# DerEchteKarsten/RayTracer3

Hardware: AMD Instinct MI355X
Metric: Mrays/s (higher is better)
Workload: dtype f32

## Files before the change

include/rt3.h:

```cpp
#ifndef RT3_H
#define RT3_H
#include <stddef.h>
#include <stdint.h>

#ifdef __cplusplus
extern "C" {
#endif

#define RT3_OK 0
#define RT3_E_INVALID (-1)
#define RT3_E_HIP (-2)
#define RT3_E_NO_DEVICE (-3)
#define RT3_E_STATE (-4)
#define RT3_E_UNSUPPORTED (-5)
#define RT3_E_DEPTH (-6)
#define RT3_E_COMM (-7)

#define RT3_INVALID_HANDLE 0xFFFFFFFFu
#define RT3_TAG_BUFFER 0u
#define RT3_TAG_IMAGE 1u
#define RT3_TAG_ACCEL 3u
#define RT3_MISS 0xFFFFFFFFu
#define RT3_BACKGROUND_DEPTH 100000.0f

#define RT3_FORMAT_R32_SFLOAT 100u
#define RT3_FORMAT_R32G32B32A32_SFLOAT 109u
#define RT3_FORMAT_R32G32B32A32_UINT 107u
#define RT3_FORMAT_R8G8B8A8_UNORM 37u
#define RT3_FORMAT_R16_UINT 74u

#define RT3_F_NEE_SKY 1u
#define RT3_F_BLUENOISE 2u
#define RT3_F_SPECULAR 4u
#define RT3_F_FACEFORWARD 8u
#define RT3_F_PROBE_RADIANCE 16u
#define RT3_F_NEE_EMISSIVE 32u
#define RT3_F_NEE_PUNCTUAL 64u

typedef struct rt3_gconst {
    float proj[16];
    float view[16];
    float proj_inverse[16];
    float view_inverse[16];
    float window_size[2];
    uint32_t frame;
    float blendfactor;
    uint32_t bounces;
    uint32_t samples;
    uint32_t proberng;
    float cell_size;
    uint32_t mouse[2];
    uint32_t pad[2];
} rt3_gconst;

typedef struct rt3_geometry_info {
    float base_color[4];
    int32_t base_color_texture_index;
    float metallic_factor;
    uint32_t index_offset;
    uint32_t vertex_offset;
    float emission[4];
    float roughness;
    uint32_t _pad[3];
} rt3_geometry_info;

typedef struct rt3_instance {
    uint32_t geometry_first, geometry_count;
    float transform[16];
} rt3_instance;

typedef struct rt3_stats {
    uint64_t extension_rays;
    uint64_t shadow_rays;
    uint64_t nodes_visited;
    uint64_t tris_tested;
    uint64_t shadow_nodes_visited;
    uint64_t shadow_tris_tested;
    uint64_t extend_launches;
    double extend_ms;
    uint64_t shadow_launches;
    double shadow_ms;
    double shade_ms;
    double other_ms;
    uint64_t trace_launches;
    double trace_ms;
    uint64_t trace_rays[2];
    uint64_t trace_nodes[2];
    uint64_t trace_tris[2];
    double gather_ms;
    uint64_t nodes_visited_lds;
    uint64_t shadow_nodes_visited_lds;
    double accel_build_ms;
    uint64_t accel_bulk_copies;
    uint64_t accel_arena_serial;
} rt3_stats;

typedef struct rt3_ctx rt3_ctx;

int rt3_create(int device, rt3_ctx **out);
void rt3_destroy(rt3_ctx *ctx);
const char *rt3_last_error(rt3_ctx *ctx);
int rt3_device_name(rt3_ctx *ctx, char *buf, size_t buf_size);

#define RT3_OPT_BATCH_SPP 1
#define RT3_OPT_PROFILE 2
#define RT3_OPT_COUNT_TRAVERSAL 3
#define RT3_OPT_EXTEND_VARIANT 4
#define RT3_OPT_LEAF_SIZE 5
#define RT3_OPT_NODE_WIDTH 6
#define RT3_OPT_NODE_QUANT 7
#define RT3_OPT_WIDE_COLLAPSE 8
#define RT3_OPT_POOL_CHUNK 9
#define RT3_OPT_SAH_TOP 11
#define RT3_OPT_TRACE_BLOCKS 12
#define RT3_OPT_INSTANCE_MODE 14
#define RT3_OPT_SHADOW_EXIT_TABLE 15
#define RT3_OPT_DEFER_SKY_LIGHT 16
int rt3_set_option(rt3_ctx *ctx, int option, int64_t value);

int rt3_scene_set_vertices(rt3_ctx *ctx, const float *interleaved_p_n_t, uint32_t n_vertices);
int rt3_scene_set_indices(rt3_ctx *ctx, const uint32_t *indices, uint32_t n_indices);
int rt3_scene_set_geometry(rt3_ctx *ctx, const rt3_geometry_info *infos, const uint32_t *prim_counts, uint32_t n);
int rt3_scene_set_sky(rt3_ctx *ctx, const float *rgb, uint32_t width, uint32_t height);
int rt3_scene_set_bluenoise(rt3_ctx *ctx, const uint8_t *rgba, uint32_t width, uint32_t height);
int rt3_scene_set_texture(rt3_ctx *ctx, uint32_t index, const uint8_t *rgba_srgb, uint32_t width, uint32_t height);
int rt3_scene_set_alpha_cutoffs(rt3_ctx *ctx, const float *cutoffs, uint32_t n);
typedef struct rt3_material_textures {
    int32_t metallic_roughness_texture;
    int32_t normal_texture;
    int32_t emissive_texture;
    float   normal_scale;
} rt3_material_textures;
int rt3_scene_set_material_textures(rt3_ctx *ctx, const rt3_material_textures *m, uint32_t n);
typedef struct rt3_transmission {
    float    transmission;
    float    ior;
    uint32_t thin_walled;
    uint32_t reserved;
} rt3_transmission;
int rt3_scene_set_transmission(rt3_ctx *ctx, const rt3_transmission *t, uint32_t n);
int rt3_scene_set_pane_shadows(rt3_ctx *ctx, int on);
int rt3_scene_get_pane_shadows(rt3_ctx *ctx, int *on);
int rt3_pane_shadow_info(rt3_ctx *ctx, uint32_t *n_panes);

int rt3_scene_set_instances(rt3_ctx *ctx, const rt3_instance *instances, uint32_t n);
int rt3_scene_set_prev_transforms(rt3_ctx *ctx, const float *transforms , uint32_t n);
#define RT3_LIGHT_POINT 0u
#define RT3_LIGHT_SPOT 1u
#define RT3_LIGHT_DIRECTIONAL 2u
typedef struct rt3_punctual_light {
    uint32_t type;
    float range;
    float inner_cone, outer_cone;
    float position[3];
    float _pad0;
    float direction[3];
    float _pad1;
    float intensity[3];
    float _pad2;
} rt3_punctual_light;
int rt3_scene_set_lights(rt3_ctx *ctx, const rt3_punctual_light *lights, uint32_t n);
int rt3_light_masses(rt3_ctx *ctx, uint32_t flags, uint32_t *n_emitters, uint32_t *n_punctual, uint32_t *mass);
int rt3_scene_snapshot_vertices(rt3_ctx *ctx);
int rt3_scene_forget_prev_vertices(rt3_ctx *ctx);
int rt3_scene_deformed_geometries(rt3_ctx *ctx, uint8_t *flags, uint32_t n);

int rt3_accel_build(rt3_ctx *ctx, uint32_t *out_handle);
int rt3_accel_info(rt3_ctx *ctx, uint32_t *n_nodes, uint32_t *n_tris, uint32_t *max_depth, uint32_t *node_bytes);
int rt3_accel_download(rt3_ctx *ctx, void *nodes, size_t nodes_bytes, void *tris, size_t tris_bytes);
int rt3_accel_levels(rt3_ctx *ctx, uint32_t *n_meshes, uint32_t *n_meshes_built, uint32_t *n_top_nodes, uint64_t *accel_bytes);
int rt3_accel_exit_table_info(rt3_ctx *ctx, uint32_t *cells, uint64_t *tried, uint64_t *occluded, uint32_t *in_use);
int rt3_accel_import(rt3_ctx *ctx, const void *nodes, size_t nodes_bytes, const void *tris, size_t tris_bytes);
int rt3_scene_update_vertices(rt3_ctx *ctx, const float *interleaved_p_n_t, uint32_t first, uint32_t n);
int rt3_accel_refit(rt3_ctx *ctx, uint32_t *out_handle);
int rt3_light_info(rt3_ctx *ctx, uint32_t *n_emitters, uint64_t *cdf_total);
int rt3_light_download(rt3_ctx *ctx, uint32_t *prim, float *area, uint32_t *mass );
int rt3_sky_download(rt3_ctx *ctx, uint32_t *alias, uint32_t *texels_rgb9e5, float *cdf_marg, float *pdf_uv);

int rt3_buffer_create(rt3_ctx *ctx, size_t bytes, uint32_t *out_handle);
int rt3_image_create(rt3_ctx *ctx, uint32_t width, uint32_t height, uint32_t format, uint32_t *out_handle);
int rt3_image_import(rt3_ctx *ctx, void *device_ptr, uint32_t width, uint32_t height, uint32_t format, uint32_t *out_handle);
int rt3_resource_upload(rt3_ctx *ctx, uint32_t handle, const void *src, size_t bytes);
int rt3_resource_download(rt3_ctx *ctx, uint32_t handle, void *dst, size_t bytes);
int rt3_resource_device_ptr(rt3_ctx *ctx, uint32_t handle, void **out_ptr, size_t *out_bytes);

int rt3_set_tile_partition(rt3_ctx *ctx, uint32_t width, uint32_t height, uint32_t rank, uint32_t n_ranks);
int rt3_tile_pixel_count(rt3_ctx *ctx, uint32_t rank, uint32_t n_ranks, uint32_t *out_count);
int rt3_image_pack_tiles(rt3_ctx *ctx, uint32_t image, uint32_t rank, uint32_t n_ranks, void *dst_device);
int rt3_image_unpack_tiles(rt3_ctx *ctx, uint32_t image, uint32_t rank, uint32_t n_ranks, const void *src_device);

#define RT3_COMM_ID_BYTES 128
int rt3_comm_version(int *out);
int rt3_comm_unique_id(void *id_out );
int rt3_comm_init(rt3_ctx *ctx, const void *id , uint32_t rank, uint32_t n_ranks);
int rt3_comm_destroy(rt3_ctx *ctx);
int rt3_gather_tiles(rt3_ctx *ctx, uint32_t image, uint32_t root);
int rt3_gather_layout(rt3_ctx *ctx, uint32_t image, uint32_t root, uint32_t n_ranks, uint64_t *offsets );
int rt3_gather_unpack(rt3_ctx *ctx, uint32_t image, uint32_t root, uint32_t n_ranks, const void *recv_device);

int rt3_pass_launch(rt3_ctx *ctx, const char *pass_name, const char *entry, uint32_t x, uint32_t y, uint32_t z,
                    const void *constants, size_t constants_size, const uint32_t *bindings, uint32_t n_bindings);
#define RT3_DENOISE_NO_DEMODULATION 1u
typedef struct rt3_denoise_params {
    uint32_t iterations;
    uint32_t normal_squarings;
    float sigma_z;
    float sigma_l;
    uint32_t flags;
} rt3_denoise_params;
int rt3_denoise_set_params(rt3_ctx *ctx, const rt3_denoise_params *params);
int rt3_denoise_set_variance_input(rt3_ctx *ctx, uint32_t moments_image);

#define RT3_TEMPORAL_NO_DEMODULATION 1u
typedef struct rt3_temporal_params {
    float alpha;
    float alpha_moments;
    uint32_t max_history;
    float normal_cos;
    float plane_tolerance;
    uint32_t flags;
} rt3_temporal_params;
int rt3_temporal_set_prev_view(rt3_ctx *ctx, const void *prev_gconst, size_t size);
int rt3_temporal_set_params(rt3_ctx *ctx, const rt3_temporal_params *params);
int rt3_temporal_set_motion_input(rt3_ctx *ctx, uint32_t motion_image);
typedef struct rt3_adaptive_params {
    uint32_t min_samples;
    uint32_t step;
    float threshold;
    float dark;
    uint32_t dilate;
    uint32_t flags;
} rt3_adaptive_params;
int rt3_adaptive_set_params(rt3_ctx *ctx, const rt3_adaptive_params *params);
int rt3_adaptive_info(rt3_ctx *ctx, uint32_t *rounds, uint64_t *paths_traced, uint32_t *pixels_capped);
typedef struct rt3_lens_params {
    float aperture_radius;
    float focus_distance;
    float pixel_jitter;
    uint32_t reserved;
} rt3_lens_params;
int rt3_camera_set_lens(rt3_ctx *ctx, const rt3_lens_params *p);
int rt3_camera_get_lens(rt3_ctx *ctx, rt3_lens_params *out, int *enabled);
typedef struct rt3_roulette_params {
    uint32_t start_bounce;
    float min_survival;
    uint32_t reserved[2];
} rt3_roulette_params;
int rt3_path_set_roulette(rt3_ctx *ctx, const rt3_roulette_params *p);
int rt3_path_get_roulette(rt3_ctx *ctx, rt3_roulette_params *out, int *enabled);
int rt3_path_roulette_info(rt3_ctx *ctx, uint64_t *tested, uint64_t *ended);

int rt3_frame_wait(rt3_ctx *ctx);

int rt3_trace_rays(rt3_ctx *ctx, const float *rays, uint32_t n, int any_hit, float *t, float *u, float *v, uint32_t *prim,
                   uint32_t *n_nodes, uint32_t *n_tris, int repeat, double *kernel_ms);

int rt3_selftest_eval(rt3_ctx *ctx, int op, const void *in, uint32_t n, void *out);

int rt3_stats_reset(rt3_ctx *ctx);
int rt3_stats_get(rt3_ctx *ctx, rt3_stats *out);

void rt3_camera_gconst(const float position[3], const float direction[3], float fov_y_radians, float aspect,
                       float z_near, float z_far, float width, float height, rt3_gconst *out);

#ifdef __cplusplus
}
#endif
#endif
```

raytracer3_amd/_lib.py:

```python
from __future__ import annotations

import ctypes as C
import os
from pathlib import Path

PKG = Path(__file__).resolve().parent
LIB_PATH = Path(os.environ.get("RT3_LIBRARY", PKG / "librt3.so"))

RT3_OK = 0
E_INVALID, E_HIP, E_NO_DEVICE, E_STATE, E_UNSUPPORTED, E_DEPTH, E_COMM = -1, -2, -3, -4, -5, -6, -7
COMM_ID_BYTES = 128
TAG_BUFFER, TAG_IMAGE, TAG_ACCEL = 0, 1, 3
MISS = 0xFFFFFFFF
BACKGROUND_DEPTH = 100000.0
FORMAT_R32_SFLOAT, FORMAT_R32G32B32A32_SFLOAT, FORMAT_R32G32B32A32_UINT, FORMAT_R8G8B8A8_UNORM, FORMAT_R16_UINT = 100, 109, 107, 37, 74
F_NEE_SKY, F_BLUENOISE, F_SPECULAR, F_FACEFORWARD, F_PROBE_RADIANCE = 1, 2, 4, 8, 16
F_NEE_EMISSIVE = 32
F_NEE_PUNCTUAL = 64
LIGHT_POINT, LIGHT_SPOT, LIGHT_DIRECTIONAL = 0, 1, 2
SELFTEST_LIGHT = 30
OPT_BATCH_SPP, OPT_PROFILE, OPT_COUNT_TRAVERSAL, OPT_EXTEND_VARIANT, OPT_LEAF_SIZE, OPT_NODE_WIDTH, OPT_NODE_QUANT = 1, 2, 3, 4, 5, 6, 7
OPT_WIDE_COLLAPSE, OPT_POOL_CHUNK, OPT_SAH_TOP, OPT_TRACE_BLOCKS = 8, 9, 11, 12
OPT_FUSED_TRACE = 10
OPT_INSTANCE_MODE = 14
OPT_SHADOW_EXIT_TABLE = 15
OPT_DEFER_SKY_LIGHT = 16
DENOISE_NO_DEMODULATION = 1
TEMPORAL_NO_DEMODULATION = 1
SELFTEST_EXPN = 28
SELFTEST_HIT_INFO = 29
SELFTEST_LENS = 31
SELFTEST_GLASS = 32
SELFTEST_ROULETTE = 33
SELFTEST_ROULETTE_QUEUE = 34

EXPORTS = [
    "rt3_create", "rt3_destroy", "rt3_last_error", "rt3_device_name", "rt3_set_option",
    "rt3_scene_set_vertices", "rt3_scene_set_indices", "rt3_scene_set_geometry", "rt3_scene_set_sky", "rt3_scene_set_bluenoise", "rt3_scene_set_texture",
    "rt3_scene_set_alpha_cutoffs",
    "rt3_scene_set_material_textures",
    "rt3_scene_set_transmission",
    "rt3_scene_set_pane_shadows", "rt3_scene_get_pane_shadows", "rt3_pane_shadow_info",
    "rt3_scene_set_instances",
    "rt3_accel_build", "rt3_accel_info", "rt3_accel_levels", "rt3_accel_exit_table_info", "rt3_accel_download", "rt3_accel_import", "rt3_sky_download",
    "rt3_scene_update_vertices", "rt3_accel_refit", "rt3_light_info", "rt3_light_download",
    "rt3_buffer_create", "rt3_image_create", "rt3_image_import", "rt3_resource_upload", "rt3_resource_download", "rt3_resource_device_ptr",
    "rt3_set_tile_partition", "rt3_tile_pixel_count", "rt3_image_pack_tiles", "rt3_image_unpack_tiles",
    "rt3_comm_version", "rt3_comm_unique_id", "rt3_comm_init", "rt3_comm_destroy", "rt3_gather_tiles", "rt3_gather_layout", "rt3_gather_unpack",
    "rt3_pass_launch", "rt3_denoise_set_params", "rt3_denoise_set_variance_input", "rt3_temporal_set_prev_view", "rt3_temporal_set_params",
    "rt3_scene_set_prev_transforms", "rt3_temporal_set_motion_input",
    "rt3_adaptive_set_params", "rt3_adaptive_info",
    "rt3_camera_set_lens", "rt3_camera_get_lens",
    "rt3_path_set_roulette", "rt3_path_get_roulette", "rt3_path_roulette_info",
    "rt3_scene_set_lights", "rt3_light_masses",
    "rt3_scene_snapshot_vertices", "rt3_scene_forget_prev_vertices", "rt3_scene_deformed_geometries",
    "rt3_frame_wait", "rt3_trace_rays", "rt3_selftest_eval", "rt3_stats_reset", "rt3_stats_get", "rt3_camera_gconst",
]


class GConst(C.Structure):

    _fields_ = [("proj", C.c_float * 16), ("view", C.c_float * 16), ("proj_inverse", C.c_float * 16), ("view_inverse", C.c_float * 16),
                ("window_size", C.c_float * 2), ("frame", C.c_uint32), ("blendfactor", C.c_float), ("bounces", C.c_uint32),
                ("samples", C.c_uint32), ("proberng", C.c_uint32), ("cell_size", C.c_float), ("mouse", C.c_uint32 * 2), ("pad", C.c_uint32 * 2)]


class Stats(C.Structure):
    _fields_ = [("extension_rays", C.c_uint64), ("shadow_rays", C.c_uint64), ("nodes_visited", C.c_uint64), ("tris_tested", C.c_uint64),
                ("shadow_nodes_visited", C.c_uint64), ("shadow_tris_tested", C.c_uint64),
                ("extend_launches", C.c_uint64), ("extend_ms", C.c_double), ("shadow_launches", C.c_uint64), ("shadow_ms", C.c_double),
                ("shade_ms", C.c_double), ("other_ms", C.c_double),
                ("trace_launches", C.c_uint64), ("trace_ms", C.c_double), ("trace_rays", C.c_uint64 * 2), ("trace_nodes", C.c_uint64 * 2),
                ("trace_tris", C.c_uint64 * 2), ("gather_ms", C.c_double), ("nodes_visited_lds", C.c_uint64), ("shadow_nodes_visited_lds", C.c_uint64), ("accel_build_ms", C.c_double), ("accel_bulk_copies", C.c_uint64),
                ("accel_arena_serial", C.c_uint64)]


class Instance(C.Structure):

    _fields_ = [("geometry_first", C.c_uint32), ("geometry_count", C.c_uint32), ("transform", C.c_float * 16)]


class DenoiseParams(C.Structure):

    _fields_ = [("iterations", C.c_uint32), ("normal_squarings", C.c_uint32), ("sigma_z", C.c_float), ("sigma_l", C.c_float), ("flags", C.c_uint32)]

    def __init__(self, iterations=5, normal_squarings=7, sigma_z=0.05, sigma_l=4.0, flags=0):
        super().__init__(iterations, normal_squarings, sigma_z, sigma_l, flags)


class TemporalParams(C.Structure):

    _fields_ = [("alpha", C.c_float), ("alpha_moments", C.c_float), ("max_history", C.c_uint32), ("normal_cos", C.c_float),
                ("plane_tolerance", C.c_float), ("flags", C.c_uint32)]

    def __init__(self, alpha=0.2, alpha_moments=0.2, max_history=32, normal_cos=0.9, plane_tolerance=0.01, flags=0):
        super().__init__(alpha, alpha_moments, max_history, normal_cos, plane_tolerance, flags)


class AdaptiveParams(C.Structure):

    _fields_ = [("min_samples", C.c_uint32), ("step", C.c_uint32), ("threshold", C.c_float), ("dark", C.c_float), ("dilate", C.c_uint32),
                ("flags", C.c_uint32)]

    def __init__(self, min_samples=16, step=16, threshold=0.05, dark=0.01, dilate=1, flags=0):
        super().__init__(min_samples, step, threshold, dark, dilate, flags)


class LensParams(C.Structure):

    _fields_ = [("aperture_radius", C.c_float), ("focus_distance", C.c_float), ("pixel_jitter", C.c_float), ("reserved", C.c_uint32)]

    def __init__(self, aperture_radius=0.0, focus_distance=1.0, pixel_jitter=1.0, reserved=0):
        super().__init__(aperture_radius, focus_distance, pixel_jitter, reserved)


class RouletteParams(C.Structure):

    _fields_ = [("start_bounce", C.c_uint32), ("min_survival", C.c_float), ("reserved", C.c_uint32 * 2)]

    def __init__(self, start_bounce=2, min_survival=0.0625, reserved=(0, 0)):
        super().__init__(start_bounce, min_survival, (C.c_uint32 * 2)(*reserved))


assert C.sizeof(GConst) == 304


def kernel_source_hash() -> str:
    import hashlib

    h = hashlib.sha256()
    files = sorted((PKG / "csrc").glob("*.hip")) + sorted((PKG / "csrc").glob("*.hpp")) + sorted((PKG / "csrc").glob("*.inc")) + [PKG / "csrc" / "Makefile", PKG.parent / "include" / "rt3.h"]
    for f in files:
        h.update(f.name.encode())
        h.update(f.read_bytes())
    return h.hexdigest()[:16]


class Rt3Error(RuntimeError):
    def __init__(self, code, msg):
        super().__init__(f"rt3 error {code}: {msg}")
        self.code = code


_lib = None


def load():
    global _lib
    if _lib is not None:
        return _lib
    try:
        import torch
    except ImportError:
        pass
    if not LIB_PATH.exists():
        raise ImportError(f"{LIB_PATH} is missing: build it with `make -C {PKG / 'csrc'}` (hipcc, gfx950). There is no CPU fallback.")
    L = C.CDLL(str(LIB_PATH))
    vp, u32, i32, f32, sz = C.c_void_p, C.c_uint32, C.c_int, C.c_float, C.c_size_t
    pu32 = C.POINTER(C.c_uint32)
    sig = {
        "rt3_create": (i32, [i32, C.POINTER(vp)]),
        "rt3_destroy": (None, [vp]),
        "rt3_last_error": (C.c_char_p, [vp]),
        "rt3_device_name": (i32, [vp, C.c_char_p, sz]),
        "rt3_set_option": (i32, [vp, i32, C.c_int64]),
        "rt3_scene_set_vertices": (i32, [vp, vp, u32]),
        "rt3_scene_set_indices": (i32, [vp, vp, u32]),
        "rt3_scene_set_geometry": (i32, [vp, vp, vp, u32]),
        "rt3_scene_set_sky": (i32, [vp, vp, u32, u32]),
        "rt3_scene_set_bluenoise": (i32, [vp, vp, u32, u32]),
        "rt3_scene_set_texture": (i32, [vp, u32, vp, u32, u32]),
        "rt3_scene_set_alpha_cutoffs": (i32, [vp, vp, u32]),
        "rt3_scene_set_material_textures": (i32, [vp, vp, u32]),
        "rt3_scene_set_transmission": (i32, [vp, vp, u32]),
        "rt3_scene_set_pane_shadows": (i32, [vp, i32]),
        "rt3_scene_get_pane_shadows": (i32, [vp, C.POINTER(i32)]),
        "rt3_pane_shadow_info": (i32, [vp, C.POINTER(u32)]),
        "rt3_scene_set_instances": (i32, [vp, vp, u32]),
        "rt3_accel_build": (i32, [vp, pu32]),
# ... 60 lines not shown
```

raytracer3_amd/csrc/rt3_api.hip:

```cpp
#include <hip/hip_runtime.h>

#include <cmath>
#include <cstdio>
#include <cstring>
#include <string>
#include <vector>

#include "rt3_ctx.hpp"
#include "rt3_roulette.hpp"

using namespace rt3;

static_assert(sizeof(rt3_gconst) == 304 && sizeof(GConstDev) == 304, "GConst is 304 bytes (renderer/mod.rs:47-63)");
static_assert(sizeof(rt3_geometry_info) == 64, "geometry info is 64 bytes");
static_assert(RT3_F_NEE_SKY == RT3_FLAG_NEE_SKY && RT3_F_BLUENOISE == RT3_FLAG_BLUENOISE && RT3_F_FACEFORWARD == RT3_FLAG_FACEFORWARD && RT3_F_SPECULAR == RT3_FLAG_SPECULAR && RT3_F_PROBE_RADIANCE == RT3_FLAG_PROBE_RADIANCE && RT3_F_NEE_EMISSIVE == RT3_FLAG_NEE_EMISSIVE && RT3_F_NEE_PUNCTUAL == RT3_FLAG_NEE_PUNCTUAL, "flags");
static_assert(sizeof(rt3_punctual_light) == 64, "rt3_punctual_light is four float4 to the device");

static thread_local std::string g_create_error;

namespace rt3 {

int fail(rt3_ctx* c, int code, const std::string& msg) {
    if (c) c->err = msg;
    else g_create_error = msg;
    return code;
}

Resource* get_res(rt3_ctx* c, uint32_t handle, uint32_t want_tag) {
    uint32_t tag = handle >> 30, idx = handle & 0x3FFFFFFFu;
    if (tag != want_tag || idx >= c->resources.size()) return nullptr;
    Resource* r = &c->resources[idx];
    return r->tag == want_tag && r->ptr ? r : nullptr;
}
size_t format_bytes(uint32_t f) {
    switch (f) {
        case RT3_FORMAT_R32_SFLOAT: return 4;
        case RT3_FORMAT_R32G32B32A32_SFLOAT: return 16;
        case RT3_FORMAT_R32G32B32A32_UINT: return 16;
        case RT3_FORMAT_R8G8B8A8_UNORM: return 4;
        case RT3_FORMAT_R16_UINT: return 2;
        default: return 0;
    }
}

int harvest(rt3_ctx* c) {
    if (!c->work.pending_counters.empty()) {
        std::vector<uint32_t> h(c->work.counters_next);
        HIPC(c, hipMemcpy(h.data(), c->work.d_counters.get(), (size_t)c->work.counters_next * 4, hipMemcpyDeviceToHost));
        for (auto& b : c->work.pending_counters) {
            for (uint32_t k = 0; k < b.n_pairs; k++) {
                uint32_t traced = h[b.first + 2 * k];
                if (b.rr_first && k >= b.rr_lo && k + 1 < b.n_pairs) {
                    const uint32_t emitted = traced;
                    traced = h[b.rr_first + k];
                    if (b.launch == c->work.launch_serial) {
                        c->work.roulette_tested += emitted;
                        c->work.roulette_ended += emitted - traced;
                    }
                }
                c->prof.stats.extension_rays += traced;
                c->prof.stats.shadow_rays += h[b.first + 2 * k + 1];
            }
            for (uint32_t k = 0; k < b.n_emit; k++) c->prof.stats.shadow_rays += h[b.emit_first + k];
        }
        c->work.pending_counters.clear();
    }
    c->work.counters_next = 0;
    c->prof.stats.extension_rays += c->work.primary_rays_pending;
    c->work.primary_rays_pending = 0;
    if (c->opt.count) {
        unsigned long long t[kTotWords] = {};
        HIPC(c, hipMemcpy(t, c->work.d_totals.get(), sizeof(t), hipMemcpyDeviceToHost));
        c->prof.stats.nodes_visited += t[kTotExtendNodes];
        c->prof.stats.tris_tested += t[kTotExtendTris];
        c->prof.stats.shadow_nodes_visited += t[kTotShadowNodes];
        c->prof.stats.shadow_tris_tested += t[kTotShadowTris];
        c->prof.stats.nodes_visited_lds += t[kTotExtendLds];
        c->prof.stats.shadow_nodes_visited_lds += t[kTotShadowLds];
        HIPC(c, hipMemset(c->work.d_totals.get(), 0, sizeof(t)));
    }
    for (auto& t : c->prof.pending_events) {
        float ms = 0.0f;
        HIPC(c, hipEventElapsedTime(&ms, t.a, t.b));
        switch (t.cat) {
            case CAT_EXTEND: c->prof.stats.extend_ms += ms; c->prof.stats.extend_launches++; break;
            case CAT_SHADOW: c->prof.stats.shadow_ms += ms; c->prof.stats.shadow_launches++; break;
            case CAT_SHADE: c->prof.stats.shade_ms += ms; break;
            case CAT_GATHER: c->prof.stats.gather_ms += ms; break;
            default: c->prof.stats.other_ms += ms; break;
        }
        c->prof.free_events.push_back(t);
    }
    c->prof.pending_events.clear();
    return RT3_OK;
}

}

extern "C" {

int rt3_create(int device, rt3_ctx** out) {
    if (!out) return fail(nullptr, RT3_E_INVALID, "out is NULL");
    *out = nullptr;
    int n = 0;
    if (hipGetDeviceCount(&n) != hipSuccess || n <= 0) return fail(nullptr, RT3_E_NO_DEVICE, "no HIP device visible (librt3 has no CPU fallback)");
    if (device < 0 || device >= n) return fail(nullptr, RT3_E_INVALID, "device index out of range");
    hipDeviceProp_t prop;
    if (hipSetDevice(device) != hipSuccess || hipGetDeviceProperties(&prop, device) != hipSuccess) return fail(nullptr, RT3_E_HIP, "hipSetDevice failed");
    if (std::string(prop.gcnArchName).rfind("gfx950", 0) != 0)
        return fail(nullptr, RT3_E_NO_DEVICE, std::string("device is ") + prop.gcnArchName + ", librt3 is built for gfx950 only");
    rt3_ctx* c = new rt3_ctx();
    c->device = device;
    snprintf(c->name, sizeof(c->name), "%s (%s)", prop.name, prop.gcnArchName);
    memset(&c->prof.stats, 0, sizeof(c->prof.stats));
    if (hipStreamCreateWithFlags(&c->stream, hipStreamNonBlocking) != hipSuccess || c->work.d_counters.alloc_bytes((size_t)c->work.counters_cap * 4) != hipSuccess ||
        c->work.d_totals.alloc_bytes(kTotWords * 8) != hipSuccess || hipMemset(c->work.d_totals.get(), 0, kTotWords * 8) != hipSuccess) {
        rt3_destroy(c);
        return fail(nullptr, RT3_E_HIP, "stream / counter allocation failed");
    }
    *out = c;
    return RT3_OK;
}

void rt3_destroy(rt3_ctx* c) {
    if (!c) return;
    (void)hipSetDevice(c->device);
    if (c->stream) (void)hipStreamSynchronize(c->stream);
    comm_release(c);
    for (auto& t : c->prof.pending_events) { (void)hipEventDestroy(t.a); (void)hipEventDestroy(t.b); }
    for (auto& t : c->prof.free_events) { (void)hipEventDestroy(t.a); (void)hipEventDestroy(t.b); }
    hipStream_t stream = c->stream;
    delete c;
    if (stream) (void)hipStreamDestroy(stream);
}

const char* rt3_last_error(rt3_ctx* c) { return c ? c->err.c_str() : g_create_error.c_str(); }

int rt3_device_name(rt3_ctx* c, char* buf, size_t n) {
    if (!c || !buf || !n) return RT3_E_INVALID;
    snprintf(buf, n, "%s", c->name);
    return RT3_OK;
}

int rt3_set_option(rt3_ctx* c, int option, int64_t value) {
    if (!c) return RT3_E_INVALID;
    switch (option) {
        case RT3_OPT_BATCH_SPP: c->opt.batch_spp = value; return RT3_OK;
        case RT3_OPT_PROFILE: c->opt.profile = value != 0; return RT3_OK;
        case RT3_OPT_COUNT_TRAVERSAL: c->opt.count = value != 0; return RT3_OK;
        case RT3_OPT_EXTEND_VARIANT:
            c->opt.variant = (int)value;
            HIPC(c, hipSetDevice(c->device));
            set_refill_lanes((uint32_t)value);
            return RT3_OK;
        case RT3_OPT_LEAF_SIZE:
            if (value < 1 || value > 8) return fail(c, RT3_E_INVALID, "leaf size must be 1..8");
            c->opt.leaf_size = (uint32_t)value;
            invalidate_topology(c);
            return RT3_OK;
        case RT3_OPT_NODE_QUANT:
            if (value < 0 || value > 2) return fail(c, RT3_E_INVALID, "node quantisation must be 0 (fp32), 1 (64 B) or 2 (compact 48 B)");
            c->opt.node_quant = (uint32_t)value;
            invalidate_topology(c);
            return RT3_OK;
        case RT3_OPT_SAH_TOP:
            if (value < 0 || value > 65536) return fail(c, RT3_E_INVALID, "SAH-top cluster size must be 0 (off) .. 65536");
            c->opt.sah_top = (uint32_t)value;
            invalidate_topology(c);
            return RT3_OK;
        case RT3_OPT_POOL_CHUNK:
            if (value < 64 || value > 65536 || (value & 63)) return fail(c, RT3_E_INVALID, "pool chunk must be a multiple of 64 in [64, 65536]");
            HIPC(c, hipSetDevice(c->device));
            set_pool_chunk((uint32_t)value);
            return RT3_OK;
        case RT3_OPT_TRACE_BLOCKS:
            if (value < 1 || value > 65535) return fail(c, RT3_E_INVALID, "trace blocks must be in [1, 65535]");
            set_trace_blocks((uint32_t)value);
            return RT3_OK;
        case RT3_OPT_WIDE_COLLAPSE:
            if (value < 0 || value > 2) return fail(c, RT3_E_INVALID, "wide collapse must be 0 (even depth), 1 (surface area) or 2 (cost-driven)");
            c->opt.collapse = (uint32_t)value;
            invalidate_topology(c);
            return RT3_OK;
        case RT3_OPT_NODE_WIDTH:
            if (value != 2 && value != 4) return fail(c, RT3_E_INVALID, "node width must be 2 or 4");
            c->opt.node_width = (uint32_t)value;
            invalidate_topology(c);
            return RT3_OK;
        case RT3_OPT_INSTANCE_MODE:
            if (value != 0 && value != 1) return fail(c, RT3_E_INVALID, "instance mode must be 0 (flatten) or 1 (two-level)");
            c->opt.instance_mode = (int)value;
            invalidate_accel(c);
            return RT3_OK;
        case RT3_OPT_SHADOW_EXIT_TABLE:
            if (value < 0 || value > 2) return fail(c, RT3_E_INVALID, "shadow exit table must be 0 (off), 1 (on) or 2 (on, scrambled entries)");
            c->opt.exit_table = (int)value;
            return exit_table_update(c);
        case RT3_OPT_DEFER_SKY_LIGHT:
            if (value != 0 && value != 1) return fail(c, RT3_E_INVALID, "defer sky light must be 0 (off) or 1 (on)");
            c->opt.defer_sky_light = value != 0;
            return RT3_OK;
        default: return fail(c, RT3_E_INVALID, "unknown option");
    }
}

int rt3_buffer_create(rt3_ctx* c, size_t bytes, uint32_t* out) {
    if (!c || !out || !bytes) return fail(c, RT3_E_INVALID, "bad buffer size");
    HIPC(c, hipSetDevice(c->device));
    Resource r;
    r.tag = RT3_TAG_BUFFER;
    r.bytes = bytes;
    HIPC(c, r.mem.alloc_bytes(bytes));
    r.ptr = r.mem.get();
    HIPC(c, hipMemset(r.ptr, 0, bytes));
    c->resources.push_back(std::move(r));
    *out = (RT3_TAG_BUFFER << 30) | (uint32_t)(c->resources.size() - 1);
    return RT3_OK;
}
int rt3_image_create(rt3_ctx* c, uint32_t w, uint32_t h, uint32_t format, uint32_t* out) {
    size_t px = format_bytes(format);
    if (!c || !out || !w || !h || !px) return fail(c, RT3_E_INVALID, "bad image size / format");
    HIPC(c, hipSetDevice(c->device));
    Resource r;
    r.tag = RT3_TAG_IMAGE;
    r.w = w; r.h = h; r.format = format;
    r.bytes = (size_t)w * h * px;
    HIPC(c, r.mem.alloc_bytes(r.bytes));
    r.ptr = r.mem.get();
    HIPC(c, hipMemset(r.ptr, 0, r.bytes));
    c->resources.push_back(std::move(r));
    *out = (RT3_TAG_IMAGE << 30) | (uint32_t)(c->resources.size() - 1);
    return RT3_OK;
}
int rt3_image_import(rt3_ctx* c, void* device_ptr, uint32_t w, uint32_t h, uint32_t format, uint32_t* out) {
    size_t px = format_bytes(format);
    if (!c || !out || !device_ptr || !w || !h || !px) return fail(c, RT3_E_INVALID, "bad import");
    Resource r;
    r.tag = RT3_TAG_IMAGE;
    r.w = w; r.h = h; r.format = format;
    r.bytes = (size_t)w * h * px;
    r.ptr = device_ptr;
    c->resources.push_back(std::move(r));
    *out = (RT3_TAG_IMAGE << 30) | (uint32_t)(c->resources.size() - 1);
    return RT3_OK;
}
static Resource* any_res(rt3_ctx* c, uint32_t handle) {
    Resource* r = get_res(c, handle, RT3_TAG_IMAGE);
    return r ? r : get_res(c, handle, RT3_TAG_BUFFER);
}
int rt3_resource_upload(rt3_ctx* c, uint32_t handle, const void* src, size_t bytes) {
    if (!c || !src) return RT3_E_INVALID;
    Resource* r = any_res(c, handle);
    if (!r || bytes != r->bytes) return fail(c, RT3_E_INVALID, "upload: bad handle or size");
    HIPC(c, hipSetDevice(c->device));
    HIPC(c, hipStreamSynchronize(c->stream));
    HIPC(c, hipMemcpy(r->ptr, src, bytes, hipMemcpyHostToDevice));
    return RT3_OK;
}
int rt3_resource_download(rt3_ctx* c, uint32_t handle, void* dst, size_t bytes) {
    if (!c || !dst) return RT3_E_INVALID;
    Resource* r = any_res(c, handle);
    if (!r || bytes != r->bytes) return fail(c, RT3_E_INVALID, "download: bad handle or size");
    HIPC(c, hipSetDevice(c->device));
    HIPC(c, hipStreamSynchronize(c->stream));
    HIPC(c, hipMemcpy(dst, r->ptr, bytes, hipMemcpyDeviceToHost));
    return RT3_OK;
}
int rt3_resource_device_ptr(rt3_ctx* c, uint32_t handle, void** out_ptr, size_t* out_bytes) {
    if (!c || !out_ptr) return RT3_E_INVALID;
    Resource* r = any_res(c, handle);
    if (!r) return fail(c, RT3_E_INVALID, "bad handle");
    *out_ptr = r->ptr;
    if (out_bytes) *out_bytes = r->bytes;
    return RT3_OK;
}

int rt3_frame_wait(rt3_ctx* c) {
    if (!c) return RT3_E_INVALID;
    HIPC(c, hipSetDevice(c->device));
    HIPC(c, hipStreamSynchronize(c->stream));
    return RT3_OK;
}

int rt3_trace_rays(rt3_ctx* c, const float* rays, uint32_t n, int any_hit, float* t, float* u, float* v, uint32_t* prim, uint32_t* n_nodes,
                   uint32_t* n_tris, int repeat, double* kernel_ms) {
    if (!c || !rays || !prim || (!any_hit && (!t || !u || !v))) return fail(c, RT3_E_INVALID, "trace_rays: NULL argument");
    if (int r = check_accel_current(c)) return r;
    if (n == 0) return RT3_OK;
    HIPC(c, hipSetDevice(c->device));
    DevBuf<float> d_rays, d_hits;
    DevBuf<uint32_t> d_cn, d_ct, d_occ, d_cur;
    const bool count = n_nodes || n_tris;
    struct Events {
        hipEvent_t e0 = nullptr, e1 = nullptr;
        ~Events() {
            if (e0) (void)hipEventDestroy(e0);
            if (e1) (void)hipEventDestroy(e1);
        }
    } ev;
    HIPC(c, d_rays.alloc_bytes((size_t)n * 32));
    HIPC(c, d_hits.alloc_bytes((size_t)n * 16));
    HIPC(c, d_occ.alloc_bytes((size_t)n * 4));
    HIPC(c, d_cur.alloc_bytes(4));
    if (count) {
        HIPC(c, d_cn.alloc_bytes((size_t)n * 4));
        HIPC(c, d_ct.alloc_bytes((size_t)n * 4));
    }
    {
        std::vector<float> rec((size_t)n * 8);
        for (uint32_t i = 0; i < n; i++) {
            float* a = &rec[4 * (size_t)i];
            float* b = &rec[4 * ((size_t)n + i)];
            a[0] = rays[i]; a[1] = rays[(size_t)n + i]; a[2] = rays[2 * (size_t)n + i]; a[3] = rays[6 * (size_t)n + i];
            b[0] = rays[3 * (size_t)n + i]; b[1] = rays[4 * (size_t)n + i]; b[2] = rays[5 * (size_t)n + i]; b[3] = rays[7 * (size_t)n + i];
        }
        HIPC(c, hipMemcpy(d_rays.get(), rec.data(), (size_t)n * 32, hipMemcpyHostToDevice));
    }
    HIPC(c, hipEventCreate(&ev.e0));
    HIPC(c, hipEventCreate(&ev.e1));
    if (repeat < 1) repeat = 1;
    TraceLaunch L;
    L.rays = d_rays.get(); L.stride = n; L.n = n; L.work_counter = d_cur.get();
    L.hits = d_hits.get(); L.occluded = d_occ.get();
    L.count = count; L.cnt_nodes = d_cn.get(); L.cnt_tris = d_ct.get();
    if (c->accel.masked) {
        if (int r = sync_textures(c)) return r;
        L.alpha = alpha_dev(c);
    }
    auto launch = [&]() {
        (void)hipMemsetAsync(d_cur.get(), 0, 4, c->stream);
        if (any_hit) launch_shadow(c->stream, c->accel.bvh, L);
        else launch_extend(c->stream, c->accel.bvh, L);
    };
    launch();
    HIPC(c, hipEventRecord(ev.e0, c->stream));
    for (int k = 0; k < repeat; k++) launch();
    HIPC(c, hipEventRecord(ev.e1, c->stream));
    HIPC(c, hipGetLastError());
    HIPC(c, hipStreamSynchronize(c->stream));
    float ms = 0.0f;
    HIPC(c, hipEventElapsedTime(&ms, ev.e0, ev.e1));
    if (kernel_ms) *kernel_ms = (double)ms / repeat;
    if (any_hit) {
        HIPC(c, hipMemcpy(prim, d_occ.get(), (size_t)n * 4, hipMemcpyDeviceToHost));
    } else {
        std::vector<float> rec((size_t)n * 4);
        HIPC(c, hipMemcpy(rec.data(), d_hits.get(), (size_t)n * 16, hipMemcpyDeviceToHost));
        for (uint32_t i = 0; i < n; i++) {
            t[i] = rec[4 * (size_t)i];
            u[i] = rec[4 * (size_t)i + 1];
            v[i] = rec[4 * (size_t)i + 2];
            memcpy(&prim[i], &rec[4 * (size_t)i + 3], 4);
        }
// ... 183 lines not shown
```

raytracer3_amd/csrc/rt3_ctx.hpp:

```cpp
#pragma once
#include <hip/hip_runtime.h>

#include <cstring>
#include <string>
#include <utility>
#include <vector>

#include "../../include/rt3.h"
#include "rt3_internal.hpp"

struct ncclComm;

namespace rt3 {

inline const rt3_denoise_params kDenoiseDefaults = {5u, 7u, 0.05f, 4.0f, 0u};
inline const rt3_temporal_params kTemporalDefaults = {0.2f, 0.2f, 32u, 0.9f, 0.01f, 0u};
inline const rt3_adaptive_params kAdaptiveDefaults = {16u, 16u, 0.05f, 0.01f, 1u, 0u};
inline constexpr float kIdentity[16] = {1, 0, 0, 0, 0, 1, 0, 0, 0, 0, 1, 0, 0, 0, 0, 1};
inline void pack3x4(const float* m16, float* m12) {
    for (int col = 0; col < 4; col++)
        for (int row = 0; row < 3; row++) m12[3 * col + row] = m16[4 * col + row];
}

struct Resource {
    uint32_t tag = 0;
    void* ptr = nullptr;
    DevBuf<char> mem;
    size_t bytes = 0;
    uint32_t w = 0, h = 0, format = 0;
};
struct PixelList {
    uint32_t w, h, rank, n_ranks, count;
    DevBuf<uint32_t> dev;
    DevBuf<uint2> dev_bn;
    uint64_t bn_stamp = ~0ull;
};
struct GatherLayout {
    uint32_t w, h, root, n_ranks;
    std::vector<uint64_t> off;
    DevBuf<uint32_t> dev;
};
enum Cat { CAT_EXTEND = 0, CAT_SHADOW = 1, CAT_SHADE = 2, CAT_OTHER = 3, CAT_GATHER = 4 };
struct Timed {
    hipEvent_t a, b;
    int cat;
};
struct CounterBlock {
    uint32_t first, n_pairs;
    uint32_t emit_first = 0, n_emit = 0;
    uint32_t rr_first = 0, rr_lo = 0;
    uint64_t launch = 0;
};

struct TlMesh {
    uint32_t first, count;
    uint32_t node_off, tri_off;
    uint32_t n_nodes, n_tris, depth;
    double box[6];
};
struct TlInstance {
    double A[3][3], b[3];
    double nA, nM;
    float m[16];
    uint32_t mesh, prim_base;
    bool identity;
};
struct TwoLevelState {
    bool valid = false;
    uint64_t gen = 0;
    uint32_t head = 0;
    uint32_t n_alloc_nodes = 0;
    std::vector<TlMesh> meshes;
    std::vector<TlInstance> inst;
    uint32_t n_placed = 0, top_cap = 0;
    uint32_t n_meshes = 0, n_built = 0, n_top = 0;
    DevBuf<char> scratch;
};
struct MeshTables {
    DevBuf<char> mem;
    FlatGeomDev* geoms = nullptr;
    uint32_t *first_prim = nullptr, *prim_geom = nullptr;
};
struct ShadeRecords {
    DevBuf<uint4> rec;
    DevBuf<float2> uv;
    DevBuf<uint32_t> tan;
    bool has_tan = false;
    uint32_t n = 0;
    std::vector<uint64_t> key;
};
struct Placed {
    uint32_t instance, geom;
    uint32_t first_prim, n_prims;
    bool identity;
};

}

struct rt3_ctx {
    int device = 0;
    hipStream_t stream = nullptr;
    std::string err;
    char name[256] = {0};
    std::vector<rt3::Resource> resources;

    struct Scene {
        rt3::DevBuf<float> d_verts;
        uint32_t n_verts = 0;
        rt3::DevBuf<uint32_t> d_indices;
        uint32_t n_indices = 0;
        uint32_t n_geoms = 0, n_prims = 0;
        std::vector<uint32_t> h_indices;
        std::vector<rt3_geometry_info> h_geoms;
        std::vector<uint32_t> h_prim_counts;
        std::vector<std::pair<uint32_t, uint32_t>> h_geom_span;
        int64_t max_tex_index = -1;
        std::vector<float> h_cutoffs;
        std::vector<rt3_material_textures> h_mat_tex;
        std::vector<rt3_transmission> h_transmission;
        std::vector<rt3_instance> h_instances;
        std::vector<float> prev_transforms;
        std::vector<rt3_punctual_light> lights;
        uint64_t lights_stamp = 1;
        rt3::DevBuf<uint2> d_sky;
        rt3::DevBuf<float> d_cdf_marg;
        rt3::DevBuf<uint32_t> d_sky_alias, d_guide_marg;
        uint32_t sky_w = 0, sky_h = 0, sky_wt = 0;
        float sky_min_pdf = 0.0f;
        rt3::DevBuf<uint8_t> d_bn;
        uint32_t bn_w = 0, bn_h = 0;
        uint64_t bn_stamp = 0;
        std::vector<std::vector<uint8_t>> h_tex;
        std::vector<uint32_t> tex_w, tex_h;
        rt3::DevBuf<uint8_t> d_tex_pixels;
        rt3::DevBuf<uint4> d_tex_table;
        rt3::DevBuf<float> d_srgb_lut;
        bool tex_dirty = false;
        uint64_t topo_gen = 1, content_gen = 1;
    } scene;

    struct Accel {
        rt3::DevBuf<rt3::FlatGeomDev> d_geoms;
        rt3::DevBuf<rt3::ShadeGeomDev> d_shade_geoms;
        rt3::DevBuf<rt3::MatTexDev> d_mat_tex;
        bool has_mat_tex = false, has_normal_tex = false;
        rt3::DevBuf<rt3::GlassDev> d_glass;
        bool has_glass = false;
        rt3::DevBuf<uint32_t> d_prim_geom, d_first_prim;
        uint32_t n_flat_geoms = 0, n_flat_prims = 0;
        std::vector<rt3::Placed> placed;
        uint64_t bulk_copies = 0;
        rt3::DevBuf<uint2> d_geom_mask, d_alpha;
        bool masked = false;
        uint32_t n_panes = 0, pane_first_slot = 0;
        bool marked = false;
        rt3::LbvhResult bvh;
        rt3::ShadeRecords shade;
        rt3::DevBuf<char> build_scratch;
        bool built = false;
        bool stale = false;
        uint64_t topo_gen = 0;
        uint64_t stamp = 0;
        rt3::LightTable lights;
        bool refit_planned = false;
        std::vector<rt3::RefitTree> refit_trees;
        std::vector<rt3::MeshTables> refit_tables;
        rt3::DevBuf<char> refit_scratch;
        rt3::TwoLevelState tl;
        rt3::DevBuf<unsigned long long> exit_counters;
        rt3::DevBuf<char> exit_scratch;
    } accel;

    struct Work {
        size_t cap = 0, cap_pix = 0;
        rt3::DevBuf<float> rays[2], hits, T[2];
        rt3::DevBuf<float> sh_rays, sh_contrib, lacc, radsum;
        rt3::DevBuf<float> sh2_rays, sh2_contrib, sh2_tmax;
        size_t cap_emit = 0;
        rt3::DevBuf<float> pane_dist;
        size_t cap_pane = 0;
        rt3::DevBuf<uint32_t> d_counters;
        uint32_t counters_cap = 1 << 16, counters_next = 0;
        rt3::DevBuf<unsigned long long> d_totals;
        std::vector<rt3::CounterBlock> pending_counters;
        uint64_t primary_rays_pending = 0;
        uint64_t launch_serial = 0, roulette_tested = 0, roulette_ended = 0;
    } work;

    struct Tiles {
        std::vector<rt3::PixelList> pixlists;
        std::vector<rt3::GatherLayout> gather_layouts;
        uint32_t rank = 0, n_ranks = 1, part_w = 0, part_h = 0;
        ncclComm* comm = nullptr;
        uint32_t comm_rank = 0, comm_size = 0;
        rt3::DevBuf<char> gather_buf;
    } tiles;

    struct Denoise {
        rt3_denoise_params params = rt3::kDenoiseDefaults;
        rt3::DevBuf<char> scratch;
        uint32_t variance_image = 0;
    } denoise;
    struct Temporal {
        rt3_temporal_params params = rt3::kTemporalDefaults;
        rt3_gconst prev;
        bool has_prev = false;
        uint32_t motion_image = 0;
    } temporal;
    struct Motion {
        bool dirty = false, any_moved = false, any_deformed = false;
        uint64_t stamp = 0;
        rt3::DevBuf<rt3::MotionPrevDev> d_prev;
        rt3::DevBuf<uint32_t> d_slot;
    } motion;
    struct Adaptive {
        rt3_adaptive_params params = rt3::kAdaptiveDefaults;
        rt3::DevBuf<char> scratch;
        uint32_t rounds = 0, pixels_capped = 0;
        uint64_t paths_traced = 0;
    } adaptive;
    struct Lens {
        rt3_lens_params params = {0.0f, 1.0f, 1.0f, 0u};
        bool on = false;
    } lens;
    struct Roulette {
        rt3_roulette_params params = {2u, 0.0625f, {0u, 0u}};
        bool on = false;
    } roulette;
    bool pane_shadows = false;
    struct Deform {
        rt3::DevBuf<float4> d_prev_pos;
        bool snapshot = false, dirty = false;
        std::vector<std::pair<uint32_t, uint32_t>> ranges;
        std::vector<uint32_t> h_deformed;
        rt3::DevBuf<uint32_t> d_deformed;
        rt3::DevBuf<uint4> d_chunks;
    } deform;

    struct Opt {
        int64_t batch_spp = 0;
        bool profile = false, count = false;
        int variant = 0;
        uint32_t leaf_size = 2, node_width = 4, node_quant = 1, collapse = 2, sah_top = 1;
        int instance_mode = 0;
        int exit_table = 1;
        bool defer_sky_light = true;
    } opt;
    struct Prof {
        rt3_stats stats;
        std::vector<rt3::Timed> pending_events;
        std::vector<rt3::Timed> free_events;
    } prof;
};

namespace rt3 {

int fail(rt3_ctx* c, int code, const std::string& msg);
#define HIPC(ctx, call)                                                                                              \
    do {                                                                                                             \
        hipError_t e_ = (call);                                                                                      \
        if (e_ != hipSuccess) return fail(ctx, RT3_E_HIP, std::string(#call) + ": " + hipGetErrorString(e_));        \
    } while (0)

template <typename T>
int dev_alloc(rt3_ctx* c, DevBuf<T>& b, size_t count) {
    HIPC(c, b.alloc_bytes((count ? count : 1) * sizeof(T)));
    return RT3_OK;
}
struct ScopedTimer {
    rt3_ctx* c;
    Timed t;
    bool on;
    ScopedTimer(rt3_ctx* ctx, int cat) : c(ctx), on(ctx->opt.profile) {
        if (!on) return;
        if (!c->prof.free_events.empty()) {
            t = c->prof.free_events.back();
            c->prof.free_events.pop_back();
        } else if (hipEventCreate(&t.a) != hipSuccess || hipEventCreate(&t.b) != hipSuccess) {
            on = false;
            return;
        }
        t.cat = cat;
        (void)hipEventRecord(t.a, c->stream);
    }
    ~ScopedTimer() {
        if (!on) return;
        (void)hipEventRecord(t.b, c->stream);
        c->prof.pending_events.push_back(t);
    }
};
Resource* get_res(rt3_ctx* c, uint32_t handle, uint32_t want_tag);
size_t format_bytes(uint32_t f);
int harvest(rt3_ctx* c);

void invalidate_topology(rt3_ctx* c);
int sync_textures(rt3_ctx* c);
int revalidate_geometry(rt3_ctx* c);
int deform_flags(rt3_ctx* c);
inline bool any_cutoff(const rt3_ctx* c) { return !c->scene.h_cutoffs.empty(); }
inline bool any_mat_tex(const rt3_ctx* c) { return !c->scene.h_mat_tex.empty(); }
inline bool any_glass(const rt3_ctx* c) { return !c->scene.h_transmission.empty(); }
inline bool pane_geometry(const rt3_ctx* c, uint32_t g) {
    if (!c->pane_shadows || !any_glass(c)) return false;
    const rt3_transmission& t = c->scene.h_transmission[g];
    if (!(t.transmission > 0.0f) || t.thin_walled != 1u) return false;
    return !any_mat_tex(c) || c->scene.h_mat_tex[g].normal_texture < 0;
}

void invalidate_accel(rt3_ctx* c);
void mark_accel_stale(rt3_ctx* c);
int check_accel_current(rt3_ctx* c, const char* unbuilt = "rt3_accel_build has not been called for the current scene");
std::pair<const rt3_instance*, size_t> placements(const rt3_ctx* c, rt3_instance& whole);
SceneDev scene_dev(const rt3_ctx* c);
GeomTables world_tables(const rt3_ctx* c);
AlphaDev alpha_dev(const rt3_ctx* c);
PaneDev pane_dev(const rt3_ctx* c);
int ensure_lights(rt3_ctx* c, uint32_t combo = RT3_F_NEE_EMISSIVE);
int exit_table_update(rt3_ctx* c);
void exit_counters_reset(rt3_ctx* c);

void motion_tables_stale(rt3_ctx* c);

int get_pixlist(rt3_ctx* c, uint32_t w, uint32_t h, uint32_t rank, uint32_t n_ranks, PixelList** out);
int pixlist_bluenoise(rt3_ctx* c, PixelList* pl);
void comm_release(rt3_ctx* c);

}
```

raytracer3_amd/csrc/rt3_internal.hpp:

```cpp
#pragma once
#include <hip/hip_runtime.h>
#include <stddef.h>
#include <stdint.h>

#include <utility>
#include <vector>

#include "rt3_camera.hpp"
#include "rt3_glass.hpp"
#include "rt3_math.hpp"
#include "rt3_surface.hpp"

#define RT3_FLAG_NEE_SKY 1u
#define RT3_FLAG_BLUENOISE 2u
#define RT3_FLAG_SPECULAR 4u
#define RT3_FLAG_FACEFORWARD 8u
#define RT3_FLAG_PROBE_RADIANCE 16u
#define RT3_FLAG_NEE_EMISSIVE 32u
#define RT3_FLAG_NEE_PUNCTUAL 64u

namespace rt3 {

constexpr int kExtendBlock = 256;
constexpr unsigned kExtendMaxBlocks = 2048;
constexpr int kLayoutBinary64 = 0;
constexpr int kLayoutWide128 = 1;
constexpr int kLayoutWide48Q = 3;
constexpr int kC48Stride = 3;
constexpr int kLayoutWide64Q = 2;
constexpr int kLayoutTwoLevel = 4;
constexpr uint32_t kMaxStack = 64;
constexpr uint32_t kTopCacheNodes = 128;
enum TotalsWord : int {
    kTotExtendNodes = 0,
    kTotExtendTris = 1,
    kTotShadowNodes = 2,
    kTotShadowTris = 3,
    kTotExtendLds = 4,
    kTotShadowLds = 5,
    kTotWords = 6
};

struct ShadeLaunch {
    GConstDev g;
    SceneDev sc;
    const uint32_t* pixels;
    const uint2* pixbn;
    uint32_t npix, width;
    FastDiv npix_div;
    uint32_t s0;
    uint32_t bounce;
    union {
        const uint4* gbuffer;
        const GlassDev* glass;
    };
    const float* depth;
    const float* in_rays;
    const float* in_hits;
    const float* in_T;
    const uint32_t* in_count;
    uint32_t n_first;
    float* out_rays;
    float* out_T;
    uint32_t* out_count;
    float* sh_rays;
    float* sh_contrib;
    uint32_t* sh_count;
    float* lacc;
    size_t stride;
    LightsDev lights;
    float* sh2_rays;
    float* sh2_contrib;
    float* sh2_tmax;
    uint32_t* sh2_count;
};
struct GeomTables {
    const float* verts;
    const uint32_t* indices;
    const FlatGeomDev* geoms;
    const uint32_t *prim_geom, *first_prim;
};

inline unsigned grid_for(uint64_t n, unsigned block, unsigned max_blocks) {
    uint64_t b = (n + block - 1) / block;
    if (b < 1) b = 1;
    return (unsigned)(b > max_blocks ? max_blocks : b);
}

void launch_raygen(hipStream_t st, const GConstDev& g, const uint32_t* pixels, uint32_t npix, float* rays, size_t stride);
void launch_gbuffer(hipStream_t st, const SceneDev& sc, const uint32_t* pixels, uint32_t npix, uint32_t width, const float* hits,
                    size_t stride, void* gbuffer, float* depth);
void launch_shade(hipStream_t st, bool first, ShadeLaunch L, bool punct = false, const GlassDev* glass = nullptr, bool defer = false, float* pane_dist = nullptr);
void launch_light(hipStream_t st, bool first, ShadeLaunch L);
void launch_pixbn(hipStream_t st, const uint32_t* pixels, uint32_t npix, const uint8_t* bluenoise, uint32_t bn_w, uint32_t bn_h, uint2* out);
void launch_accumulate(hipStream_t st, const GConstDev& g, const uint32_t* pixels, uint32_t npix, uint32_t width, const float* depth,
                       const float* lacc, size_t stride, uint32_t sb, int first_batch, int last_batch, float* radsum, void* light,
                       const void* prev);
void launch_postprocess(hipStream_t st, const GConstDev& g, const SceneDev& sc, const uint32_t* pixels, uint32_t npix, uint32_t width,
                        const float* depth, const void* in, void* out);
void launch_lens_rays(hipStream_t st, const GConstDev& g, const LensDev& lens, const uint32_t* pixels, uint32_t npix, uint32_t s0, uint32_t n_first,
                      float* rays, float* T, float* lacc, size_t stride, uint32_t* count);
void launch_lens_miss(hipStream_t st, const SceneDev& sc, const float* rays, const float* hits, float* lacc, size_t stride, uint32_t n);
void launch_accumulate_lens(hipStream_t st, const GConstDev& g, const uint32_t* pixels, uint32_t npix, uint32_t width, const float* lacc, uint32_t sb,
                            int first_batch, int last_batch, float* radsum, void* light, const void* prev);
void launch_postprocess_lens(hipStream_t st, const uint32_t* pixels, uint32_t npix, uint32_t width, const void* in, void* out);
constexpr uint32_t kSelftestLensIn = 41, kSelftestLensOut = 10;
void launch_selftest_lens(hipStream_t st, const uint32_t* in, uint32_t n, uint32_t* out);
constexpr uint32_t kSelftestGlassIn = 9, kSelftestGlassOut = 5;
void launch_selftest_glass(hipStream_t st, const uint32_t* in, uint32_t n, uint32_t* out);
struct RouletteLaunch;
void launch_roulette(hipStream_t st, const RouletteLaunch& a, uint32_t n_max, uint32_t groups = 0);
constexpr uint32_t kSelftestRouletteIn = 5, kSelftestRouletteOut = 5;
void launch_selftest_roulette(hipStream_t st, const uint32_t* in, uint32_t n, uint32_t* out);
constexpr uint32_t kSelftestQueueHeader = 7, kSelftestQueueRecord = 11;
void launch_pack_tiles(hipStream_t st, const uint32_t* pixels, uint32_t npix, uint32_t width, const void* img, void* dst);
void launch_unpack_tiles(hipStream_t st, const uint32_t* pixels, uint32_t npix, uint32_t width, const void* src, void* img);

void launch_sis(hipStream_t st, uint32_t W, uint32_t probes_x, uint32_t probes_y, const void* gbuffer, void* out, float* debug);
void launch_probe_raygen(hipStream_t st, const GConstDev& g, uint32_t W, uint32_t probes_x, uint32_t probes_y, const float* depth, const void* directions,
                         void* atlas, float* rays, size_t stride, void* d2);
void launch_probe_store(hipStream_t st, const SceneDev& sc, uint32_t flags, float blend, uint32_t probes_x, uint32_t probes_y, const float* hits,
                        const void* d2, const void* prev, void* atlas);
void launch_sh_conversion(hipStream_t st, uint32_t probes_x, uint32_t probes_y, const void* atlas, void* out);
void launch_interpolate(hipStream_t st, const GConstDev& g, uint32_t W, uint32_t H, const void* gbuffer, const float* depth, const void* sh, void* light);
void launch_selftest_probes(hipStream_t st, int op, const uint32_t* in, uint32_t n, uint32_t* out);

void launch_prim_geom(hipStream_t st, const uint32_t* first_prim, uint32_t n_geoms, uint32_t n, uint32_t* prim_geom);
void set_refill_lanes(uint32_t v);
void set_pool_chunk(uint32_t v);
void set_trace_blocks(uint32_t v);
bool selftest_widths(int op, uint32_t* in_w, uint32_t* out_w);
void launch_selftest(hipStream_t st, int op, const SceneDev& sc, const uint32_t* in, uint32_t n, uint32_t* out);

#define RT3_TRY(x)                           \
    do {                                     \
        const hipError_t e_ = (x);           \
        if (e_ != hipSuccess) return e_;     \
    } while (0)

template <typename T>
class DevBuf {
public:
    DevBuf() = default;
    DevBuf(const DevBuf&) = delete;
    DevBuf& operator=(const DevBuf&) = delete;
    DevBuf(DevBuf&& o) noexcept : p_(o.p_), cap_(o.cap_) {
        o.p_ = nullptr;
        o.cap_ = 0;
    }
    DevBuf& operator=(DevBuf&& o) noexcept {
        if (this != &o) {
            reset();
            p_ = o.p_;
            cap_ = o.cap_;
            o.p_ = nullptr;
            o.cap_ = 0;
        }
        return *this;
    }
    ~DevBuf() { reset(); }
    T* get() const { return p_; }
    size_t capacity_bytes() const { return cap_; }
    explicit operator bool() const { return p_ != nullptr; }
    void reset() {
        if (p_) (void)hipFree(p_);
        p_ = nullptr;
        cap_ = 0;
    }
    hipError_t alloc_bytes(size_t bytes) {
        reset();
        void* p = nullptr;
        const hipError_t e = hipMalloc(&p, bytes);
        if (e == hipSuccess) {
            p_ = static_cast<T*>(p);
            cap_ = bytes;
        }
        return e;
    }
    hipError_t grow_bytes(size_t bytes) { return bytes <= cap_ ? hipSuccess : alloc_bytes(bytes); }

private:
    T* p_ = nullptr;
    size_t cap_ = 0;
};

class BufLayout {
public:
    template <typename T>
    BufLayout& add(T** dst, size_t count) {
        const size_t at = (end_ + 255) & ~(size_t)255;
        pieces_.push_back({dst, at, &set_ptr<T>});
        end_ = at + count * sizeof(T);
        return *this;
    }
    size_t bytes() const { return end_; }
    hipError_t carve(const DevBuf<char>& buf) const {
        if (buf.capacity_bytes() < end_) return hipErrorOutOfMemory;
        for (const Piece& p : pieces_) p.set(p.dst, buf.get() + p.at);
        return hipSuccess;
    }

private:
    struct Piece {
        void* dst;
        size_t at;
        void (*set)(void* dst, char* p);
    };
    template <typename T>
    static void set_ptr(void* dst, char* p) { *static_cast<T**>(dst) = reinterpret_cast<T*>(p); }
    std::vector<Piece> pieces_;
    size_t end_ = 0;
};

template <typename T>
class DevView {
public:
    DevView() = default;
    explicit DevView(T* p) : p_(p) {}
    T* get() const { return p_; }
    explicit operator bool() const { return p_ != nullptr; }

private:
    T* p_ = nullptr;
};

constexpr uint64_t kArenaMaxBytes = (4ull << 30) - 128;
uint64_t next_arena_serial();
constexpr size_t kArenaSlack = 128;

constexpr uint32_t kExitDefaultR = 256, kExitMaxR = 1024;
constexpr size_t kExitTableSlack = 64;
struct ExitHeader {
    float lo[3], hi[3], scale[3];
    uint32_t R, last;
    uint32_t pad[5];
};
static_assert(sizeof(ExitHeader) == 64, "the entries start 64 bytes behind the header");
constexpr uint64_t kExitWarmupTries = 1ull << 16;
struct ExitTable {
    uint32_t off = 0;
    uint32_t R = 0;
    float lo[3] = {0, 0, 0}, hi[3] = {0, 0, 0};
    float scale[3] = {0, 0, 0};
    unsigned long long* counters = nullptr;
    bool on = false;
};

struct LbvhResult {
    DevBuf<float4> arena;
    DevView<float4> nodes;
    uint32_t node_bytes = 128;
    int layout = kLayoutWide128;
    DevView<float4> tris;
    uint32_t tri_off = 0;
    uint64_t arena_need = 0;
    uint64_t arena_serial = 0;
    DevBuf<float4> top;
    uint32_t n_top = 0;
    uint32_t n_nodes = 0, n_tris = 0, max_depth = 0;
    ExitTable exit;

    hipError_t alloc_arena(size_t nodes_bytes, size_t n_records, hipStream_t st, uint32_t exit_R = 0) {
        const uint32_t exit_cells = 6u * exit_R * exit_R;
        free_arena();
        const size_t off = (nodes_bytes + 127) & ~(size_t)127, rec_end = off + n_records * 48;
        const size_t table = exit_cells ? sizeof(ExitHeader) + (size_t)exit_cells * 4 + kExitTableSlack : 0;
        arena_need = rec_end + kArenaSlack + table;
        if (arena_need > kArenaMaxBytes) return hipErrorInvalidValue;
        RT3_TRY(arena.alloc_bytes(rec_end + kArenaSlack + table));
        arena_serial = next_arena_serial();
        tri_off = (uint32_t)off;
        nodes = DevView<float4>(arena.get());
        tris = DevView<float4>(reinterpret_cast<float4*>(reinterpret_cast<char*>(arena.get()) + off));
        RT3_TRY(hipMemsetAsync(reinterpret_cast<char*>(arena.get()) + rec_end, 0, kArenaSlack, st));
        if (!table) return hipSuccess;
        exit.R = exit_R;
        exit.off = (uint32_t)(rec_end + kArenaSlack);
        return hipMemsetAsync(reinterpret_cast<char*>(arena.get()) + exit.off, 0xFF, table, st);
    }
    void free_arena() {
        arena.reset();
        nodes = tris = DevView<float4>();
        tri_off = 0;
        arena_serial = 0;
        exit = ExitTable{};
    }
    void take_arena(LbvhResult& from) {
        arena = std::move(from.arena);
        nodes = from.nodes;
        tris = from.tris;
        tri_off = from.tri_off;
        arena_serial = from.arena_serial;
        exit = from.exit;
        from.exit = ExitTable{};
        from.nodes = from.tris = DevView<float4>();
        from.tri_off = 0;
        from.arena_serial = 0;
    }
};
struct PaneDev {
    SceneDev sc;
    const GlassDev* glass;
    uint32_t first_slot;
};
struct TraceLaunch {
    const float* rays = nullptr;
    size_t stride = 0;
    const uint32_t* count_ptr = nullptr;
    uint32_t n = 0;
    uint32_t* work_counter = nullptr;
    float* hits = nullptr;
    bool payload = false;
    const float* contrib = nullptr;
    float* lacc = nullptr;
    const float* tmax = nullptr;
    uint32_t* occluded = nullptr;
    bool count = false;
    uint32_t *cnt_nodes = nullptr, *cnt_tris = nullptr;
    unsigned long long* totals = nullptr;
    AlphaDev alpha = {};
    const PaneDev* pane = nullptr;
};
void launch_extend(hipStream_t st, const LbvhResult& bvh, const TraceLaunch& L);
void launch_shadow(hipStream_t st, const LbvhResult& bvh, const TraceLaunch& L);
hipError_t lbvh_build(hipStream_t st, GeomTables t, uint32_t n_prims, uint32_t leaf_max, uint32_t node_width, uint32_t node_quant, uint32_t collapse_mode,
                      uint32_t sah_top, DevBuf<char>& scratch, LbvhResult* out, const uint2* geom_mask = nullptr, uint32_t exit_R = 0);

struct ExitScratch {
    float *rays, *hits;
    uint32_t *prim_leaf, *cursor;
};
void exit_table_plan(uint32_t cells, uint32_t n_prims, BufLayout& plan, ExitScratch* s);
hipError_t exit_table_fill(hipStream_t st, const LbvhResult& bvh, uint32_t n_prims, const ExitScratch& s, bool scramble);
struct SahTopScratch {
    uint32_t *top, *ncl, *pool_pos, *cl_pos, *pool, *cl_ref, *cl_cnt, *idx, *tmp, *counters, *tile_left, *tile_woff, *tile_roff;
    float *cl_mn, *cl_mx;
    char *seg_a, *seg_b, *seg_small, *huge, *tiles;
    char* scan_tmp;
    size_t scan_bytes;
};
hipError_t sah_top_plan(hipStream_t st, uint32_t n, BufLayout& plan, SahTopScratch* s);
hipError_t sah_top_relink_gpu(hipStream_t st, uint32_t nn, uint32_t* left, uint32_t* right, uint32_t* rcnt, uint32_t* pint, uint32_t* pleaf,
                              const float* lmin, const float* lmax, float* nbox, uint32_t T, const SahTopScratch& s, bool* relinked);

void launch_tri_shade(hipStream_t st, GeomTables t, uint32_t n, uint4* tri_shade, float2* tri_uv);
void launch_tri_tangent(hipStream_t st, GeomTables t, uint32_t n, uint32_t* tri_tan);

void tlas_rebase_nodes(hipStream_t st, const float4* src, float4* dst, uint32_t n, uint32_t node_from, uint32_t node_to, uint32_t tri_from, uint32_t tri_to);
void tlas_box_tris(hipStream_t st, const float* boxes, uint32_t n, float* verts, uint32_t* indices);
void tlas_emit_top(hipStream_t st, const float4* top_nodes, uint32_t n_nodes, const float4* top_tris, uint32_t rec_base, float4* dst);

struct RefitTree {
    DevBuf<uint32_t> order;
    std::vector<uint32_t> level_count;
};
hipError_t refit_plan(hipStream_t st, const float4* nodes, uint32_t root, uint32_t n_nodes, uint32_t max_depth, RefitTree* plan);
hipError_t refit_tree(hipStream_t st, const RefitTree& plan, GeomTables t, uint32_t n_prims, uint32_t tri_first, uint32_t n_tris, float4* nodes,
                      float4* tris, uint32_t* bounds, float* nbox, float* tbox);

struct LightTable {
    DevBuf<float4> rec;
    DevBuf<uint32_t> cdf, guide, prim, geom_base;
    DevBuf<float> area;
    DevBuf<char> scratch;
    uint32_t n = 0, n_guide = 0, guide_shift = 0, total = 0;
    uint32_t n_emit = 0, n_punct = 0;
    uint64_t stamp = 0;
    uint64_t lights_stamp = 0;
    uint32_t combo = 0;
    LightsDev dev() const {
        LightsDev d;
        d.rec = rec.get(); d.cdf = cdf.get(); d.guide = guide.get(); d.geom_base = geom_base.get();
        d.n = total ? n : 0u; d.guide_shift = guide_shift;
        return d;
    }
};
hipError_t lights_build(hipStream_t st, GeomTables t, const std::vector<uint32_t>& geom_base, const std::vector<uint32_t>& eg_geom,
                        const std::vector<uint32_t>& eg_first, uint32_t n, LightTable* out, const float* punct = nullptr, uint32_t n_punct = 0,
                        uint32_t n_world_prims = 0);
void launch_selftest_light(hipStream_t st, const float4* lights, uint32_t n_lights, const uint32_t* in, uint32_t n, uint32_t* out);

struct DenoiseScratch {
    float4 *gP, *gN;
    float4* sig[2];
};
struct DenoiseLaunch {
    GConstDev g;
    uint32_t W, H, squarings, flags;
    float sigma_z, sigma_l;
    const void* gbuffer;
    const float* depth;
    const void* in;
    void* out;
    const void* moments = nullptr;
    DenoiseScratch s;
};
void denoise_plan(uint32_t W, uint32_t H, BufLayout& plan, DenoiseScratch* s);
void launch_denoise_prepare(hipStream_t st, const DenoiseLaunch& L);
void launch_denoise_variance(hipStream_t st, const DenoiseLaunch& L);
void launch_denoise_atrous(hipStream_t st, const DenoiseLaunch& L, uint32_t iteration);
void launch_denoise_finish(hipStream_t st, const DenoiseLaunch& L, uint32_t iterations);
void launch_selftest_denoise(hipStream_t st, const uint32_t* in, uint32_t n, uint32_t* out);

struct TemporalLaunch {
    GConstDev g, prev;
    uint32_t W, H, flags;
    float alpha, alpha_moments, max_history, normal_cos, plane_tolerance;
    const void *gbuffer, *in, *prev_gbuffer, *prev_history, *prev_moments;
    const float *depth, *prev_depth;
    void *out, *history, *moments;
    const void* motion = nullptr;
};
void launch_temporal(hipStream_t st, const TemporalLaunch& L);

constexpr uint32_t kMotionUnmoved = 0xFFFFFFFFu;
constexpr uint32_t kMotionDeformed = 0x80000000u;
struct MotionPrevDev {
    float m[12];
    uint32_t identity;
    uint32_t pad[3];
};
static_assert(sizeof(MotionPrevDev) == 64, "MotionPrev layout");
struct MotionDev {
    const float* verts;
    const uint32_t *indices, *prim_geom, *first_prim, *geom_slot;
    const FlatGeomDev* geoms;
    const MotionPrevDev* prev;
};
struct MotionLaunch {
    GConstDev g;
    MotionDev m;
    const uint32_t* pixels;
    uint32_t npix, width;
    const float* hits;
    void* out;
    const float4* prev_pos = nullptr;
};
void launch_motion(hipStream_t st, const MotionLaunch& L);
void launch_snapshot_positions(hipStream_t st, const float* verts, uint32_t first, uint32_t n, float4* prev_pos);
constexpr uint32_t kDeformChunk = 1024;
void launch_compare_positions(hipStream_t st, const float* verts, const float4* prev_pos, const uint4* chunks, uint32_t n_chunks, uint32_t* flags);

struct AdaptiveScratch {
    float4* sums;
    float2* mom;
    uint8_t* mask;
    uint32_t* xy[2];
    uint2* bn[2];
    uint32_t* block_count;
    uint32_t* count;
};
void adaptive_plan(uint32_t W, uint32_t H, uint32_t npix, BufLayout& plan, AdaptiveScratch* s);
void launch_adaptive_init(hipStream_t st, const uint32_t* pixels, uint32_t npix, uint32_t width, const float* depth, const AdaptiveScratch& s,
                          void* moments);
void launch_adaptive_accumulate(hipStream_t st, const uint32_t* pixels, uint32_t npix, uint32_t width, const float* lacc, uint32_t sb, bool first,
                                uint32_t n_after, const AdaptiveScratch& s);
void launch_adaptive_test(hipStream_t st, const uint32_t* pixels, uint32_t npix, uint32_t width, float threshold, float dark,
                          const AdaptiveScratch& s);
void launch_adaptive_compact(hipStream_t st, const uint2* in_bn, uint32_t n_in, uint32_t W, uint32_t H, uint32_t dilate, const AdaptiveScratch& s,
                             int out);
void launch_adaptive_finalise(hipStream_t st, const uint32_t* pixels, uint32_t npix, uint32_t width, const float* depth, float blendfactor,
                              uint32_t cap, const AdaptiveScratch& s, void* light, const void* prev, void* moments);

hipError_t lbvh_make_top(hipStream_t st, const float4* nodes, uint32_t n_nodes, DevBuf<float4>& top, uint32_t* n_top);

}
```

raytracer3_amd/csrc/rt3_passes.hip:

```cpp
#include <hip/hip_runtime.h>

#include <cmath>
#include <cstring>
#include <algorithm>
#include <string>
#include <vector>

#include "rt3_ctx.hpp"
#include "rt3_roulette.hpp"

using namespace rt3;

namespace rt3 {

void motion_tables_stale(rt3_ctx* c) { c->motion.dirty = true; }

}

namespace {

uint32_t spread1by1(uint32_t x) {
    x = (x | (x << 8)) & 0x00FF00FFu;
    x = (x | (x << 4)) & 0x0F0F0F0Fu;
    x = (x | (x << 2)) & 0x33333333u;
// ... 34 lines not shown
    }
    if (r) free_work(c);
    return r;
}
int ensure_emit_queue(rt3_ctx* c) {
    if (c->work.cap_emit >= c->work.cap) return RT3_OK;
    c->work.cap_emit = 0;
    int r = dev_alloc(c, c->work.sh2_rays, 8 * c->work.cap);
    if (!r) r = dev_alloc(c, c->work.sh2_contrib, 2 * c->work.cap);
    if (!r) r = dev_alloc(c, c->work.sh2_tmax, c->work.cap);
    if (!r) c->work.cap_emit = c->work.cap;
    else free_work(c);
    return r;
}

int ensure_pane_dist(rt3_ctx* c) {
    if (c->work.cap_pane >= c->work.cap) return RT3_OK;
    c->work.cap_pane = 0;
    int r = dev_alloc(c, c->work.pane_dist, c->work.cap);
    if (!r) c->work.cap_pane = c->work.cap;
    else free_work(c);
    return r;
}

int reserve_counters(rt3_ctx* c, uint32_t n, uint32_t* first) {
    if (c->work.counters_next + n > c->work.counters_cap) {
        HIPC(c, hipStreamSynchronize(c->stream));
        if (int r = harvest(c)) return r;
    }
    if (n > c->work.counters_cap) return fail(c, RT3_E_INVALID, "too many bounces x batches for the counter block");
    *first = c->work.counters_next;
    c->work.counters_next += n;
    HIPC(c, hipMemsetAsync(c->work.d_counters.get() + *first, 0, (size_t)n * 4, c->stream));
    return RT3_OK;
}
TraceLaunch ctx_trace(rt3_ctx* c) {
    TraceLaunch L;
    L.stride = c->work.cap;
    L.count = c->opt.count;
    L.totals = c->opt.count ? c->work.d_totals.get() : nullptr;
    L.alpha = alpha_dev(c);
    return L;
}
int trace_primary(rt3_ctx* c, uint32_t n) {
    uint32_t wc_slot;
    if (int r = reserve_counters(c, 1, &wc_slot)) return r;
    TraceLaunch L = ctx_trace(c);
    L.rays = c->work.rays[0].get(); L.n = n; L.work_counter = c->work.d_counters.get() + wc_slot; L.hits = c->work.hits.get();
    c->work.primary_rays_pending += n;
    ScopedTimer t(c, CAT_EXTEND);
    launch_extend(c->stream, c->accel.bvh, L);
    return RT3_OK;
}

int motion_tables(rt3_ctx* c) {
    rt3_instance whole;
    const auto [inst, n_inst] = placements(c, whole);
    const size_t n = c->scene.prev_transforms.size() / 16;
    if (n != 0 && n != n_inst)
        return fail(c, RT3_E_STATE, "motion: " + std::to_string(n) + " previous transforms (rt3_scene_set_prev_transforms) for a structure of " +
                                        std::to_string(n_inst) + " instance(s)");
    if (int r = deform_flags(c)) return r;
    if (!c->motion.dirty && c->motion.stamp == c->accel.stamp) return RT3_OK;
    const bool deformed_any = std::any_of(c->deform.h_deformed.begin(), c->deform.h_deformed.end(), [](uint32_t f) { return f != 0; });
    std::vector<MotionPrevDev> rec(n || deformed_any ? n_inst : 0);
    std::vector<uint8_t> moved(rec.size());
    std::vector<uint32_t> slot;
    bool any = false, any_deformed = false;
    for (size_t i = 0; i < rec.size(); i++) {
        const float *cm = inst[i].transform, *pm = n ? &c->scene.prev_transforms[16 * i] : cm;
        float cur[12];
        memset(&rec[i], 0, sizeof(rec[i]));
        pack3x4(pm, rec[i].m);
        pack3x4(cm, cur);
        rec[i].identity = memcmp(pm, kIdentity, sizeof(kIdentity)) == 0 ? 1u : 0u;
        moved[i] = memcmp(rec[i].m, cur, sizeof(cur)) != 0;
    }
    if (!rec.empty())
        for (const Placed& p : c->accel.placed) {
            const bool deformed = p.geom < c->deform.h_deformed.size() && c->deform.h_deformed[p.geom];
            slot.push_back(deformed ? (p.instance | kMotionDeformed) : (moved[p.instance] ? p.instance : kMotionUnmoved));
            any = any || moved[p.instance] || deformed;
            any_deformed = any_deformed || deformed;
        }
    if (any) {
        HIPC(c, hipStreamSynchronize(c->stream));
        if (int r = dev_alloc(c, c->motion.d_prev, rec.size())) return r;
        if (int r = dev_alloc(c, c->motion.d_slot, slot.size())) return r;
        HIPC(c, hipMemcpy(c->motion.d_prev.get(), rec.data(), rec.size() * sizeof(MotionPrevDev), hipMemcpyHostToDevice));
        HIPC(c, hipMemcpy(c->motion.d_slot.get(), slot.data(), slot.size() * 4, hipMemcpyHostToDevice));
    }
    c->motion.any_moved = any;
    c->motion.any_deformed = any_deformed;
    c->motion.dirty = false;
    c->motion.stamp = c->accel.stamp;
    return RT3_OK;
}

GConstDev gconst_dev(const rt3_gconst* g) {
    GConstDev gd;
    memcpy(&gd, g, sizeof(gd));
    return gd;
}
int check_window(rt3_ctx* c, const rt3_gconst* g, uint32_t* W, uint32_t* H) {
    float fw = g->window_size[0], fh = g->window_size[1];
    if (!(fw >= 1.0f && fh >= 1.0f && fw <= 65535.0f && fh <= 65535.0f) || fw != std::floor(fw) || fh != std::floor(fh))
        return fail(c, RT3_E_INVALID, "GConst.window_size must hold integral pixel counts in [1, 65535]");
    *W = (uint32_t)fw;
    *H = (uint32_t)fh;
    return RT3_OK;
}
Resource* image_checked(rt3_ctx* c, uint32_t handle, uint32_t W, uint32_t H, uint32_t format, const char* what) {
    Resource* r = get_res(c, handle, RT3_TAG_IMAGE);
    if (!r || r->w != W || r->h != H || r->format != format) {
        c->err = std::string("binding '") + what + "' is not a " + std::to_string(W) + "x" + std::to_string(H) + " image of the expected format";
        return nullptr;
    }
    return r;
}
int buffer_at_least(rt3_ctx* c, const Resource* r, size_t need, const char* what) {
    if (r->bytes >= need) return RT3_OK;
    return fail(c, RT3_E_INVALID, std::string("binding '") + what + "' must be a buffer of at least " + std::to_string(need) + " bytes");
}
int primary_hits(rt3_ctx* c, const GConstDev& gd, uint32_t W, uint32_t H, PixelList** out) {
    if (int r = get_pixlist(c, W, H, c->tiles.rank, c->tiles.n_ranks, out)) return r;
    const PixelList* pl = *out;
    if (pl->count == 0) return RT3_OK;
    if (int r = ensure_work(c, pl->count, pl->count)) return r;
    {
        ScopedTimer t(c, CAT_OTHER);
        launch_raygen(c->stream, gd, pl->dev.get(), pl->count, c->work.rays[0].get(), c->work.cap);
    }
    return trace_primary(c, pl->count);
}

int pass_gbuffer(rt3_ctx* c, const rt3_gconst* g, uint32_t W, uint32_t H, Resource* const* res) {
    PixelList* pl;
    if (int r = primary_hits(c, gconst_dev(g), W, H, &pl)) return r;
    if (pl->count == 0) return RT3_OK;
    {
        ScopedTimer t(c, CAT_OTHER);
        launch_gbuffer(c->stream, scene_dev(c), pl->dev.get(), pl->count, W, c->work.hits.get(), c->work.cap, res[0]->ptr, (float*)res[1]->ptr);
    }
    HIPC(c, hipGetLastError());
    return RT3_OK;
}

struct PathSetup {
    GConstDev gd;
    SceneDev sc;
    LightsDev lights{};
    bool nee = false, nee_e = false, punct = false;
    bool defer = false;
    bool lens_on = false;
    LensDev lens{};
    bool rr = false;
    uint32_t rr_start = 0;
    float rr_min = 1.0f;
    bool panes = false;
    PaneDev pane{};
};
constexpr float kSkyDeferMinPdf = 0x1p-100f;
int path_setup(rt3_ctx* c, const rt3_gconst* g, PathSetup* ps) {
    const uint32_t B = g->bounces;
    ps->gd = gconst_dev(g);
    if (c->scene.lights.empty() || B <= 1) ps->gd.pad[0] &= ~RT3_F_NEE_PUNCTUAL;
    ps->nee = (g->pad[0] & RT3_F_NEE_SKY) && c->scene.d_sky;
    const uint32_t combo = g->pad[0] & (RT3_F_NEE_EMISSIVE | (c->scene.lights.empty() ? 0u : RT3_F_NEE_PUNCTUAL));
    if (combo && B > 1) {
        if (int r = ensure_lights(c, combo)) return r;
        ps->lights = c->accel.lights.dev();
        ps->punct = ps->lights.n != 0u && c->accel.lights.n_punct != 0u;
        if (ps->lights.n)
            if (int r = ensure_emit_queue(c)) return r;
    }
    ps->nee_e = ps->lights.n != 0u;
    ps->sc = scene_dev(c);
    ps->defer = c->opt.defer_sky_light && ps->nee && !c->accel.has_glass && !ps->punct && ps->sc.mat_tex == nullptr && c->scene.sky_min_pdf >= kSkyDeferMinPdf;
    ps->panes = c->accel.n_panes != 0u && c->accel.has_glass;
    if (ps->panes) {
        if (int r = ensure_pane_dist(c)) return r;
        ps->pane = pane_dev(c);
    }
    ps->rr = c->roulette.on && c->roulette.params.start_bounce < B - 1u;
    ps->rr_start = c->roulette.params.start_bounce;
    ps->rr_min = c->roulette.params.min_survival;
    return RT3_OK;
}
LensDev lens_dev(const rt3_ctx* c) {
    const rt3_lens_params& p = c->lens.params;
    return LensDev{p.aperture_radius, p.focus_distance, p.pixel_jitter};
}
int roulette_begin(rt3_ctx* c, const char* pass, uint32_t samples, uint32_t bounces) {
    if (c->roulette.on && (uint64_t)samples * bounces * 8u > (1ull << 30))
        return fail(c, RT3_E_INVALID, std::string(pass) + " with roulette: samples * bounces * 8 may not exceed 2^30 (the roulette draws' RNG indices start behind it)");
    c->work.launch_serial++;
    c->work.roulette_tested = c->work.roulette_ended = 0;
    return RT3_OK;
}
int trace_batch(rt3_ctx* c, const PathSetup& ps, uint32_t W, const Resource* gb, const Resource* dp, const uint32_t* pixels, const uint2* pixbn,
                uint32_t npix, uint32_t s0, uint32_t nsb) {
    const uint32_t B = ps.gd.bounces;
    const size_t S = c->work.cap;
    const bool nee = ps.nee, nee_e = ps.nee_e;
    const uint32_t n_first = nsb * npix;
    const bool lens = ps.lens_on;
    const uint32_t n_words = (nee_e ? 6 : 4) * B;
    uint32_t first;
    const bool rr = ps.rr;
    if (int r = reserve_counters(c, n_words + 1 + (lens ? 2 : 0) + (rr ? B : 0), &first)) return r;
    first += first & 1u;
    uint32_t* pairs = c->work.d_counters.get() + first;
    uint32_t* pool_cur = c->work.d_counters.get() + first + 2 * B;
    uint32_t* emit_cnt = c->work.d_counters.get() + first + 4 * B;
    uint32_t* lens_cnt = c->work.d_counters.get() + first + n_words;
    uint32_t* rr_cnt = lens_cnt + (lens ? 2 : 0);
    c->work.pending_counters.push_back(
        CounterBlock{first, B, first + 4 * B, nee_e ? B : 0u, rr ? first + n_words + (lens ? 2u : 0u) : 0u, ps.rr_start, c->work.launch_serial});
    auto ext_cnt_at = [pairs](uint32_t b) { return pairs + 2 * b; };
    auto sh_cnt_at = [pairs](uint32_t b) { return pairs + 2 * b + 1; };
    int cur = 0;
    const uint32_t* live_cnt = lens ? lens_cnt : nullptr;
    if (lens) {
        {
            ScopedTimer t(c, CAT_OTHER);
            launch_lens_rays(c->stream, ps.gd, ps.lens, pixels, npix, s0, n_first, c->work.rays[0].get(), c->work.T[0].get(), c->work.lacc.get(), S,
                             lens_cnt);
        }
        {
            TraceLaunch tr = ctx_trace(c);
            tr.rays = c->work.rays[0].get(); tr.n = n_first; tr.work_counter = lens_cnt + 1; tr.hits = c->work.hits.get(); tr.payload = true;
            c->work.primary_rays_pending += n_first;
            ScopedTimer t(c, CAT_EXTEND);
            launch_extend(c->stream, c->accel.bvh, tr);
        }
        if (!nee && ps.sc.sky != nullptr) {
            ScopedTimer t(c, CAT_OTHER);
            launch_lens_miss(c->stream, ps.sc, c->work.rays[0].get(), c->work.hits.get(), c->work.lacc.get(), S, n_first);
        }
    }
    if (ps.panes) HIPC(c, hipMemsetAsync(c->work.pane_dist.get(), 0, (size_t)n_first * sizeof(float), c->stream));
    for (uint32_t bn = 0; bn < B; bn++) {
        ShadeLaunch L;
        L.g = ps.gd; L.sc = ps.sc; L.pixels = pixels; L.pixbn = pixbn; L.npix = npix; L.width = W; L.s0 = s0; L.bounce = bn;
        L.gbuffer = (const uint4*)gb->ptr; L.depth = (const float*)dp->ptr;
        L.in_rays = c->work.rays[cur].get(); L.in_hits = c->work.hits.get(); L.in_T = c->work.T[cur].get();
        L.in_count = live_cnt; L.n_first = n_first;
        L.out_rays = c->work.rays[cur ^ 1].get(); L.out_T = c->work.T[cur ^ 1].get(); L.out_count = ext_cnt_at(bn);
        L.sh_rays = c->work.sh_rays.get(); L.sh_contrib = c->work.sh_contrib.get(); L.sh_count = sh_cnt_at(bn);
        L.lacc = c->work.lacc.get(); L.stride = S;
        L.lights = ps.lights;
        L.sh2_rays = c->work.sh2_rays.get(); L.sh2_contrib = c->work.sh2_contrib.get(); L.sh2_tmax = c->work.sh2_tmax.get(); L.sh2_count = emit_cnt + bn;
        {
            ScopedTimer t(c, CAT_SHADE);
            launch_shade(c->stream, bn == 0 && !lens, L, ps.punct, c->accel.has_glass ? c->accel.d_glass.get() : nullptr, ps.defer,
                         ps.panes ? c->work.pane_dist.get() : nullptr);
        }
        cur ^= 1;
        if (nee) {
            TraceLaunch tr = ctx_trace(c);
            tr.rays = c->work.sh_rays.get(); tr.count_ptr = sh_cnt_at(bn); tr.n = n_first; tr.work_counter = pool_cur + B + bn;
            if (ps.defer) {
                tr.occluded = reinterpret_cast<uint32_t*>(c->work.sh_contrib.get()) + S;
            } else {
                tr.contrib = c->work.sh_contrib.get(); tr.lacc = c->work.lacc.get();
                if (ps.panes) tr.pane = &ps.pane;
            }
            ScopedTimer t(c, CAT_SHADOW);
            launch_shadow(c->stream, c->accel.bvh, tr);
        }
        if (ps.defer) {
            ScopedTimer t(c, CAT_SHADE);
            launch_light(c->stream, bn == 0 && !lens, L);
        }
        if (nee_e && bn + 1 < B) {
            TraceLaunch tr = ctx_trace(c);
            tr.rays = c->work.sh2_rays.get(); tr.count_ptr = emit_cnt + bn; tr.n = n_first; tr.work_counter = emit_cnt + B + bn;
            tr.contrib = c->work.sh2_contrib.get(); tr.lacc = c->work.lacc.get(); tr.tmax = c->work.sh2_tmax.get();
            if (ps.panes) tr.pane = &ps.pane;
            ScopedTimer t(c, CAT_SHADOW);
            launch_shadow(c->stream, c->accel.bvh, tr);
        }
        live_cnt = ext_cnt_at(bn);
        if (rr && bn >= ps.rr_start && bn != B - 1) {
            RouletteLaunch R{};
            R.in_rays = c->work.rays[cur].get(); R.in_T = c->work.T[cur].get(); R.in_count = live_cnt;
            R.out_rays = c->work.rays[cur ^ 1].get(); R.out_T = c->work.T[cur ^ 1].get(); R.out_count = rr_cnt + bn;
            R.stride = S; R.pixels = pixels; R.npix = npix; R.s0 = s0; R.bounces = B; R.bounce = bn; R.frame = ps.gd.frame;
            R.min_survival = ps.rr_min;
            ScopedTimer t(c, CAT_OTHER);
            launch_roulette(c->stream, R, n_first);
            cur ^= 1;
            live_cnt = rr_cnt + bn;
        }
        if (bn != B - 1) {
            TraceLaunch tr = ctx_trace(c);
            tr.rays = c->work.rays[cur].get(); tr.count_ptr = live_cnt; tr.n = n_first; tr.work_counter = pool_cur + bn;
            tr.hits = c->work.hits.get(); tr.payload = true;
            ScopedTimer t(c, CAT_EXTEND);
            launch_extend(c->stream, c->accel.bvh, tr);
        }
    }
    return RT3_OK;
}
int batch_spp(rt3_ctx* c, uint32_t npix, uint32_t spp, uint32_t* sb) {
    uint64_t max_paths = 1ull << 28;
    *sb = c->opt.batch_spp > 0 ? (uint32_t)c->opt.batch_spp : (uint32_t)std::max<uint64_t>(1, max_paths / npix);
    if (*sb > spp) *sb = spp;
    if ((uint64_t)*sb * npix > 0xFFFFFF00ull) return fail(c, RT3_E_INVALID, "batch too large");
    return RT3_OK;
}

int pass_reference_mode(rt3_ctx* c, const rt3_gconst* g, uint32_t W, uint32_t H, Resource* const* res) {
    const Resource *gb = res[0], *dp = res[1], *li = res[2], *pv = res[3];
    const uint32_t Sspp = g->samples, B = g->bounces;
    if (Sspp == 0 || B == 0) return RT3_OK;
    if (B > 64) return fail(c, RT3_E_INVALID, "bounces > 64");
    if (c->lens.on && (uint64_t)Sspp * B * 8u > (1ull << 31))
        return fail(c, RT3_E_INVALID, "refrence_mode with a lens: samples * bounces * 8 may not exceed 2^31 (the camera's RNG indices start there)");
    if (c->accel.has_glass) {
        if (!c->lens.on)
            return fail(c, RT3_E_STATE, "refrence_mode: the scene has glass (rt3_scene_set_transmission) and the packed G-buffer has no room for a material "
                                        "class: start every sample from its own camera ray with rt3_camera_set_lens ({0, f, 0} is the per-sample pinhole)");
        if ((uint64_t)Sspp * B * 8u > (1ull << 30))
            return fail(c, RT3_E_INVALID, "refrence_mode with glass: samples * bounces * 8 may not exceed 2^30 (the glass draws' RNG indices start there)");
    }
    if (int r = roulette_begin(c, "refrence_mode", Sspp, B)) return r;
    PixelList* pl;
    if (int r = get_pixlist(c, W, H, c->tiles.rank, c->tiles.n_ranks, &pl)) return r;
    const uint32_t npix = pl->count;
    if (npix == 0) return RT3_OK;
    if (int r = pixlist_bluenoise(c, pl)) return r;
    uint32_t sb;
    if (int r = batch_spp(c, npix, Sspp, &sb)) return r;
    if (int r = ensure_work(c, (size_t)sb * npix, npix)) return r;
    PathSetup ps;
    if (int r = path_setup(c, g, &ps)) return r;
    ps.lens_on = c->lens.on;
    ps.lens = lens_dev(c);
    for (uint32_t s0 = 0; s0 < Sspp; s0 += sb) {
        const uint32_t nsb = std::min(sb, Sspp - s0);
        if (int r = trace_batch(c, ps, W, gb, dp, pl->dev.get(), pl->dev_bn.get(), npix, s0, nsb)) return r;
        {
            ScopedTimer t(c, CAT_OTHER);
            if (ps.lens_on)
                launch_accumulate_lens(c->stream, ps.gd, pl->dev.get(), npix, W, c->work.lacc.get(), nsb, s0 == 0, s0 + nsb >= Sspp, c->work.radsum.get(),
                                       li->ptr, pv->ptr);
            else
                launch_accumulate(c->stream, ps.gd, pl->dev.get(), npix, W, (const float*)dp->ptr, c->work.lacc.get(), c->work.cap, nsb, s0 == 0, s0 + nsb >= Sspp,
                                  c->work.radsum.get(), li->ptr, pv->ptr);
        }
    }
    HIPC(c, hipGetLastError());
    return RT3_OK;
}

int pass_adaptive(rt3_ctx* c, const rt3_gconst* g, uint32_t W, uint32_t H, Resource* const* res) {
    const Resource *gb = res[0], *dp = res[1], *li = res[2], *pv = res[3], *mo = res[4];
    const rt3_adaptive_params& p = c->adaptive.params;
    const uint32_t cap = g->samples, B = g->bounces;
    c->adaptive.rounds = c->adaptive.pixels_capped = 0;
    c->adaptive.paths_traced = 0;
    if (c->lens.on)
        return fail(c, RT3_E_STATE, "adaptive: not with a lens set (rt3_camera_set_lens): the pass selects pixels by G-buffer depth, which knows nothing "
                                    "of partly covered pixels; switch the lens off (NULL) or use refrence_mode");
    if (c->accel.has_glass)
        return fail(c, RT3_E_STATE, "adaptive: not for a scene with glass (rt3_scene_set_transmission): glass needs per-sample camera rays "
                                    "(rt3_camera_set_lens), which this pass does not take; use refrence_mode");
    if (cap == 0 || B == 0) return RT3_OK;
    if (B > 64) return fail(c, RT3_E_INVALID, "bounces > 64");
    if (int r = roulette_begin(c, "adaptive", cap, B)) return r;
    PixelList* pl;
    if (int r = get_pixlist(c, W, H, c->tiles.rank, c->tiles.n_ranks, &pl)) return r;
    if (pl->count == 0) return RT3_OK;
    if (int r = pixlist_bluenoise(c, pl)) return r;
    AdaptiveScratch s;
    BufLayout plan;
    adaptive_plan(W, H, pl->count, plan, &s);
    if (c->adaptive.scratch.capacity_bytes() < plan.bytes()) {
        HIPC(c, hipStreamSynchronize(c->stream));
        HIPC(c, c->adaptive.scratch.grow_bytes(plan.bytes()));
    }
    HIPC(c, plan.carve(c->adaptive.scratch));
    const float* depth = (const float*)dp->ptr;
    auto list_length = [&](uint32_t* n) {
        HIPC(c, hipMemcpyAsync(n, s.count, 4, hipMemcpyDeviceToHost, c->stream));
        HIPC(c, hipStreamSynchronize(c->stream));
        return (int)RT3_OK;
    };
    uint32_t n_act = 0;
    int cur = 0;
    {
        ScopedTimer t(c, CAT_OTHER);
        HIPC(c, hipMemsetAsync(s.mask, 0, (size_t)W * H, c->stream));
        launch_adaptive_init(c->stream, pl->dev.get(), pl->count, W, depth, s, mo->ptr);
        launch_adaptive_compact(c->stream, pl->dev_bn.get(), pl->count, W, H, 0u, s, cur);
    }
    if (int r = list_length(&n_act)) return r;
    const uint32_t n_fg = n_act;
    if (n_fg) {
        const uint32_t most = std::max(std::min(p.min_samples, cap), std::min(p.step, cap));
        uint32_t sb;
        if (int r = batch_spp(c, n_fg, most, &sb)) return r;
        if (int r = ensure_work(c, (size_t)sb * n_fg, 0)) return r;
    }
    PathSetup ps;
    if (n_fg)
        if (int r = path_setup(c, g, &ps)) return r;
    uint32_t n = 0;
    while (n_act) {
        const uint32_t ns = n == 0 ? std::min(p.min_samples, cap) : std::min(p.step, cap - n);
        uint32_t sb;
        if (int r = batch_spp(c, n_act, ns, &sb)) return r;
        sb = (uint32_t)std::min<uint64_t>(sb, c->work.cap / n_act);
        for (uint32_t s0 = 0; s0 < ns; s0 += sb) {
            const uint32_t nsb = std::min(sb, ns - s0);
// ... 425 lines not shown
```

raytracer3_amd/csrc/rt3_shade.hip:

```cpp
#include <hip/hip_fp16.h>
#include <hip/hip_runtime.h>

#include <type_traits>

#include "rt3_bsdf.hpp"
#include "rt3_camera.hpp"
#include "rt3_glass.hpp"
#include "rt3_internal.hpp"
#include "rt3_math.hpp"
#include "rt3_punctual.hpp"
#include "rt3_rng.hpp"
#include "rt3_sky.hpp"
#include "rt3_surface.hpp"

namespace rt3 {

constexpr int kShadeBlock = 512;
struct BlockAppend {
    uint32_t ext, sh;
};
__device__ __forceinline__ BlockAppend block_append2(bool want_ext, bool want_sh, unsigned long long* pair ,
                                                     uint32_t* lds ) {
    constexpr int kWaves = kShadeBlock / 64;
    const uint32_t lane = __lane_id(), wave = threadIdx.x >> 6;
    const unsigned long long m_ext = __ballot(want_ext), m_sh = __ballot(want_sh);
    if (lane == 0) {
        lds[wave] = (uint32_t)__popcll(m_ext);
        lds[kWaves + 1 + wave] = (uint32_t)__popcll(m_sh);
    }
    __syncthreads();
    if (threadIdx.x == 0) {
        uint32_t te = 0, ts = 0;
#pragma unroll
        for (int w = 0; w < kWaves; w++) {
            uint32_t ce = lds[w], cs = lds[kWaves + 1 + w];
            lds[w] = te;
            lds[kWaves + 1 + w] = ts;
            te += ce;
            ts += cs;
        }
        unsigned long long old = 0ull;
        if (te | ts) old = atomicAdd(pair, (unsigned long long)te | ((unsigned long long)ts << 32));
        lds[kWaves] = (uint32_t)old;
        lds[2 * kWaves + 1] = (uint32_t)(old >> 32);
    }
    __syncthreads();
    const unsigned long long below = (1ull << lane) - 1ull;
    BlockAppend r;
    r.ext = lds[kWaves] + lds[wave] + (uint32_t)__popcll(m_ext & below);
    r.sh = lds[2 * kWaves + 1] + lds[kWaves + 1 + wave] + (uint32_t)__popcll(m_sh & below);
    return r;
}
struct BlockAppend3 {
    uint32_t ext, sh, sh2;
};
__device__ __forceinline__ BlockAppend3 block_append3(bool want_ext, bool want_sh, bool want_sh2, unsigned long long* pair, uint32_t* count2,
                                                      uint32_t* lds ) {
    constexpr int kWaves = kShadeBlock / 64, kW1 = kWaves + 1;
    const uint32_t lane = __lane_id(), wave = threadIdx.x >> 6;
    const unsigned long long m_ext = __ballot(want_ext), m_sh = __ballot(want_sh), m_sh2 = __ballot(want_sh2);
    if (lane == 0) {
        lds[wave] = (uint32_t)__popcll(m_ext);
        lds[kW1 + wave] = (uint32_t)__popcll(m_sh);
        lds[2 * kW1 + wave] = (uint32_t)__popcll(m_sh2);
    }
    __syncthreads();
    if (threadIdx.x == 0) {
        uint32_t te = 0, ts = 0, t2 = 0;
#pragma unroll
        for (int w = 0; w < kWaves; w++) {
            const uint32_t ce = lds[w], cs = lds[kW1 + w], c2 = lds[2 * kW1 + w];
            lds[w] = te;
            lds[kW1 + w] = ts;
            lds[2 * kW1 + w] = t2;
            te += ce;
            ts += cs;
            t2 += c2;
        }
        unsigned long long old = 0ull;
        if (te | ts) old = atomicAdd(pair, (unsigned long long)te | ((unsigned long long)ts << 32));
        lds[kWaves] = (uint32_t)old;
        lds[kW1 + kWaves] = (uint32_t)(old >> 32);
        lds[2 * kW1 + kWaves] = t2 ? atomicAdd(count2, t2) : 0u;
    }
    __syncthreads();
    const unsigned long long below = (1ull << lane) - 1ull;
    BlockAppend3 r;
    r.ext = lds[kWaves] + lds[wave] + (uint32_t)__popcll(m_ext & below);
    r.sh = lds[kW1 + kWaves] + lds[kW1 + wave] + (uint32_t)__popcll(m_sh & below);
    r.sh2 = lds[2 * kW1 + kWaves] + lds[2 * kW1 + wave] + (uint32_t)__popcll(m_sh2 & below);
    return r;
}

__device__ __forceinline__ bool light_next(const ShadeLaunch& a, uint32_t it, uint32_t n, uint32_t n_round, uint32_t& held, uint32_t& i, bool& active) {
    constexpr int kWaves = kShadeBlock / 64;
    __shared__ uint32_t packed[2 * kShadeBlock];
    __shared__ uint32_t wave_count[kWaves];
    const uint32_t* src = reinterpret_cast<const uint32_t*>(a.sh_contrib);
    const uint32_t* occluded = src + a.stride;
    bool keep = false;
    uint32_t s = 0;
    if (it < n) {
        keep = occluded[it] == 0u;
        s = src[it];
    }
    const uint32_t lane = __lane_id(), wave = threadIdx.x >> 6;
    const unsigned long long m = __ballot(keep);
    if (lane == 0) wave_count[wave] = (uint32_t)__popcll(m);
    __syncthreads();
    uint32_t before = 0, total = 0;
#pragma unroll
    for (int w = 0; w < kWaves; w++) {
        const uint32_t c = wave_count[w];
        before += (uint32_t)w < wave ? c : 0u;
        total += c;
    }
    if (keep) packed[held + before + (uint32_t)__popcll(m & ((1ull << lane) - 1ull))] = s;
    held += total;
    __syncthreads();
    if (held < (uint32_t)kShadeBlock && !(it >= n_round && held != 0u)) return false;
    const uint32_t take = held < (uint32_t)kShadeBlock ? held : (uint32_t)kShadeBlock;
    active = threadIdx.x < take;
    i = active ? packed[threadIdx.x] : 0u;
    held -= take;
    if (threadIdx.x < held) packed[threadIdx.x] = packed[kShadeBlock + threadIdx.x];
    return true;
}

constexpr int shade_waves(bool mat) { return mat ? 4 : 6; }
template <bool FIRST, bool GLDS, bool EMIT = false, bool MAT = false>
__global__ __launch_bounds__(kShadeBlock) __attribute__((amdgpu_waves_per_eu(shade_waves(MAT), shade_waves(MAT)))) void k_shade(ShadeLaunch a) {
    constexpr bool PUNCT = false, GLASS = false, DEFER = false, LIGHT = false;
    constexpr bool PANE = false;
    float* const pane_dist = nullptr;
#include "rt3_shade_body.inc"
}
template <bool FIRST, bool GLDS, bool MAT>
__global__ __launch_bounds__(kShadeBlock) __attribute__((amdgpu_waves_per_eu(shade_waves(true), shade_waves(true)))) void k_shade_punct(ShadeLaunch a) {
    constexpr bool EMIT = true, PUNCT = true, GLASS = false, DEFER = false, LIGHT = false;
    constexpr bool PANE = false;
    float* const pane_dist = nullptr;
#include "rt3_shade_body.inc"
}
template <bool GLDS, bool EMIT, bool MAT, bool PUNCT>
__global__ __launch_bounds__(kShadeBlock) __attribute__((amdgpu_waves_per_eu(shade_waves(true), shade_waves(true)))) void k_shade_glass(ShadeLaunch a) {
    constexpr bool FIRST = false, GLASS = true, DEFER = false, LIGHT = false;
    constexpr bool PANE = false;
    float* const pane_dist = nullptr;
#include "rt3_shade_body.inc"
}
template <bool GLDS, bool EMIT, bool MAT, bool PUNCT>
__global__ __launch_bounds__(kShadeBlock) __attribute__((amdgpu_waves_per_eu(shade_waves(true), shade_waves(true)))) void k_shade_pane(ShadeLaunch a, float* pane_dist) {
    constexpr bool FIRST = false, GLASS = true, DEFER = false, LIGHT = false, PANE = true;
#include "rt3_shade_body.inc"
}
template <bool FIRST, bool GLDS, bool EMIT>
__global__ __launch_bounds__(kShadeBlock) __attribute__((amdgpu_waves_per_eu(shade_waves(false), shade_waves(false)))) void k_shade_defer(ShadeLaunch a) {
    constexpr bool MAT = false, PUNCT = false, GLASS = false, DEFER = true, LIGHT = false;
    constexpr bool PANE = false;
    float* const pane_dist = nullptr;
#include "rt3_shade_body.inc"
}
template <bool FIRST, bool GLDS>
__global__ __launch_bounds__(kShadeBlock) __attribute__((amdgpu_waves_per_eu(shade_waves(false), shade_waves(false)))) void k_light(ShadeLaunch a) {
    constexpr bool EMIT = false, MAT = false, PUNCT = false, GLASS = false, DEFER = false, LIGHT = true;
    constexpr bool PANE = false;
    float* const pane_dist = nullptr;
#include "rt3_shade_body.inc"
}
__global__ void k_selftest_glass(const uint32_t* __restrict__ in, uint32_t n, uint32_t* __restrict__ out) {
    const uint32_t i = blockIdx.x * blockDim.x + threadIdx.x;
    if (i >= n) return;
    const uint32_t* p = in + kSelftestGlassIn * (size_t)i;
    auto F = [](uint32_t u) { return __uint_as_float(u); };
    const GlassEvent e = glass_sample(F(p[0]), p[1] != 0u, v3(F(p[2]), F(p[3]), F(p[4])), v3(F(p[5]), F(p[6]), F(p[7])), F(p[8]));
    uint32_t* o = out + kSelftestGlassOut * (size_t)i;
    o[0] = e.transmit;
    o[1] = __float_as_uint(e.dir.x); o[2] = __float_as_uint(e.dir.y); o[3] = __float_as_uint(e.dir.z);
    o[4] = __float_as_uint(e.F);
}

__global__ void k_accumulate(GConstDev g, const uint32_t* __restrict__ pixels, uint32_t npix, uint32_t width,
                             const float* __restrict__ depth, const float* __restrict__ lacc, size_t stride, uint32_t sb,
                             int first_batch, int last_batch, float* __restrict__ radsum, float4* __restrict__ light,
                             const float4* __restrict__ prev) {
    for (uint32_t i = blockIdx.x * blockDim.x + threadIdx.x; i < npix; i += gridDim.x * blockDim.x) {
        uint32_t xy = pixels[i];
        size_t pi = (size_t)(xy >> 16) * width + (xy & 0xFFFFu);
        if (depth[pi] == kBackgroundDepth) continue;
        float r = first_batch ? 0.0f : radsum[i], gg = first_batch ? 0.0f : radsum[npix + i], bb = first_batch ? 0.0f : radsum[2 * (size_t)npix + i];
        for (uint32_t s = 0; s < sb; s++) {
            size_t p = (size_t)s * npix + i;
            const float4 lv = reinterpret_cast<const float4*>(lacc)[p];
            r += lv.x;
            gg += lv.y;
            bb += lv.z;
        }
        if (!last_batch) {
            radsum[i] = r;
            radsum[npix + i] = gg;
            radsum[2 * (size_t)npix + i] = bb;
        } else {
            float fs = (float)g.samples;
            r = r / fs;
            gg = gg / fs;
            bb = bb / fs;
            if (g.blendfactor >= 1.0f) {
                light[pi] = make_float4(r, gg, bb, 0.0f);
            } else {
                float4 pv = prev[pi];
                float bf = g.blendfactor;
                light[pi] = make_float4(pv.x + (r - pv.x) * bf, pv.y + (gg - pv.y) * bf, pv.z + (bb - pv.z) * bf, 0.0f);
            }
        }
    }
}

template <typename Launch>
static void dispatch_shade(bool first, bool glds, bool emit, bool mat, bool punct, Launch launch) {
    auto by_emit = [&](auto f, auto g, auto m) {
        if (emit && punct) launch(f, g, std::true_type{}, m, std::true_type{});
        else if (emit) launch(f, g, std::true_type{}, m, std::false_type{});
        else launch(f, g, std::false_type{}, m, std::false_type{});
    };
    auto by_mat = [&](auto g) {
        if (mat) by_emit(std::false_type{}, g, std::true_type{});
        else by_emit(std::false_type{}, g, std::false_type{});
    };
    if (first) by_emit(std::true_type{}, std::false_type{}, std::false_type{});
    else if (glds) by_mat(std::true_type{});
    else by_mat(std::false_type{});
}
void launch_shade(hipStream_t st, bool first, ShadeLaunch a, bool punct, const GlassDev* glass, bool defer, float* pane_dist) {
    a.npix_div = make_fastdiv(a.npix);
    const unsigned grid = grid_for(a.n_first, kShadeBlock, 8192);
    const bool glds = a.sc.shade_geoms != nullptr && a.sc.n_geoms <= kShadeGeomsLds;
    if (defer) {
        dispatch_shade(first, glds, a.lights.n != 0u, false, false, [&](auto f, auto g, auto e, auto, auto) {
            hipLaunchKernelGGL((k_shade_defer<decltype(f)::value, decltype(g)::value, decltype(e)::value>), dim3(grid), dim3(kShadeBlock), 0, st, a);
        });
        return;
    }
    dispatch_shade(first, glds, a.lights.n != 0u, a.sc.mat_tex != nullptr, punct && a.lights.n != 0u, [&](auto f, auto g, auto e, auto m, auto p) {
        if constexpr (!decltype(f)::value) {
            if (glass != nullptr) {
                a.glass = glass;
                if (pane_dist != nullptr) {
                    hipLaunchKernelGGL((k_shade_pane<decltype(g)::value, decltype(e)::value, decltype(m)::value, decltype(p)::value>), dim3(grid), dim3(kShadeBlock), 0, st, a, pane_dist);
                    return;
                }
                hipLaunchKernelGGL((k_shade_glass<decltype(g)::value, decltype(e)::value, decltype(m)::value, decltype(p)::value>), dim3(grid), dim3(kShadeBlock), 0, st, a);
                return;
            }
        }
        if constexpr (decltype(p)::value) hipLaunchKernelGGL((k_shade_punct<decltype(f)::value, decltype(g)::value, decltype(m)::value>), dim3(grid), dim3(kShadeBlock), 0, st, a);
        else hipLaunchKernelGGL((k_shade<decltype(f)::value, decltype(g)::value, decltype(e)::value, decltype(m)::value>), dim3(grid), dim3(kShadeBlock), 0, st, a);
    });
}
void launch_light(hipStream_t st, bool first, ShadeLaunch a) {
    a.npix_div = make_fastdiv(a.npix);
    const unsigned grid = grid_for(a.n_first, kShadeBlock * 8, 8192);
    const bool glds = a.sc.shade_geoms != nullptr && a.sc.n_geoms <= kShadeGeomsLds;
    dispatch_shade(first, glds, false, false, false, [&](auto f, auto g, auto, auto, auto) {
        hipLaunchKernelGGL((k_light<decltype(f)::value, decltype(g)::value>), dim3(grid), dim3(kShadeBlock), 0, st, a);
    });
}
void launch_selftest_glass(hipStream_t st, const uint32_t* in, uint32_t n, uint32_t* out) {
    hipLaunchKernelGGL(k_selftest_glass, dim3((n + 255) / 256), dim3(256), 0, st, in, n, out);
}
void launch_accumulate(hipStream_t st, const GConstDev& g, const uint32_t* pixels, uint32_t npix, uint32_t width, const float* depth,
                       const float* lacc, size_t stride, uint32_t sb, int first_batch, int last_batch, float* radsum, void* light,
                       const void* prev) {
    hipLaunchKernelGGL(k_accumulate, dim3(grid_for(npix, 256, 8192)), dim3(256), 0, st, g, pixels, npix, width, depth, lacc, stride, sb,
                       first_batch, last_batch, radsum, (float4*)light, (const float4*)prev);
}

}
```

raytracer3_amd/csrc/rt3_shade_body.inc:

```
    static_assert(GLASS || !PANE, "a pane is a glass geometry");
    static_assert(!(DEFER && LIGHT) && !((DEFER || LIGHT) && (MAT || PUNCT || GLASS)), "deferral covers the plain opaque instances");
    static_assert(!(FIRST && MAT), "the first vertex is read from the G-buffer");
    static_assert(EMIT || !PUNCT, "punctual lights are records of the emitter table");
    static_assert(!(FIRST && GLASS), "the G-buffer has no room for a material class: glass frames start from camera rays");
    __shared__ uint32_t append_lds[2][(EMIT ? 3 : 2) * (kShadeBlock / 64 + 1)];
    __shared__ ShadeGeomDev s_geoms[GLDS ? kShadeGeomsLds : 1];
    __shared__ MatTexDev s_mats[GLDS && MAT ? kShadeGeomsLds : 1];
    __shared__ GlassDev s_glass[GLDS && GLASS ? kShadeGeomsLds : 1];
    if (GLDS) {
        const uint32_t ng = a.sc.n_geoms < kShadeGeomsLds ? a.sc.n_geoms : kShadeGeomsLds;
        const uint32_t words = ng * (uint32_t)(sizeof(ShadeGeomDev) / 4);
        for (uint32_t k = threadIdx.x; k < words; k += kShadeBlock) reinterpret_cast<uint32_t*>(s_geoms)[k] = reinterpret_cast<const uint32_t*>(a.sc.shade_geoms)[k];
        if constexpr (MAT)
            for (uint32_t k = threadIdx.x; k < ng * 4u; k += kShadeBlock) reinterpret_cast<uint32_t*>(s_mats)[k] = reinterpret_cast<const uint32_t*>(a.sc.mat_tex)[k];
        if constexpr (GLASS)
            for (uint32_t k = threadIdx.x; k < ng * 4u; k += kShadeBlock) reinterpret_cast<uint32_t*>(s_glass)[k] = reinterpret_cast<const uint32_t*>(a.glass)[k];
        __syncthreads();
    }
    uint32_t parity = 0;
    constexpr uint32_t kMargRows = 2048;
    __shared__ uint32_t s_guide_marg[kMargRows];
    __shared__ float s_cdf_marg[kMargRows + 4];
    const bool marg_in_lds = (a.g.pad[0] & RT3_FLAG_NEE_SKY) && a.sc.sky != nullptr && a.sc.sky_h <= kMargRows;
    if (marg_in_lds) {
        for (uint32_t k = threadIdx.x; k < a.sc.sky_h; k += kShadeBlock) s_guide_marg[k] = a.sc.guide_marg[k];
        for (uint32_t k = threadIdx.x; k < a.sc.sky_h + 4u; k += kShadeBlock) s_cdf_marg[k] = a.sc.cdf_marg[k];
        __syncthreads();
    }
    const float* cdf_marg = marg_in_lds ? s_cdf_marg : a.sc.cdf_marg;
    const uint32_t* guide_marg = marg_in_lds ? s_guide_marg : a.sc.guide_marg;
    const GConstDev& g = a.g;
    const uint32_t flags = g.pad[0], B = g.bounces, b = a.bounce;
    const uint32_t dims = flags ? 8u : 2u;
    const bool nee = (flags & RT3_FLAG_NEE_SKY) && a.sc.sky != nullptr;
    const bool bnz = (flags & RT3_FLAG_BLUENOISE) && a.sc.bluenoise != nullptr;
    const bool spec = (flags & RT3_FLAG_SPECULAR) != 0u;
    const size_t S = a.stride;
    const uint32_t n = LIGHT ? *a.sh_count : FIRST ? a.n_first : *a.in_count;
    const uint32_t n_round = (n + (kShadeBlock - 1)) & ~(uint32_t)(kShadeBlock - 1);
    uint32_t light_held = 0;
    for (uint32_t it = blockIdx.x * blockDim.x + threadIdx.x; it < n_round + (LIGHT ? gridDim.x * blockDim.x : 0u); it += gridDim.x * blockDim.x) {
        uint32_t i = it;
        bool active = i < n;
        if constexpr (LIGHT) {
            if (!light_next(a, it, n, n_round, light_held, i, active)) continue;
        }
        uint32_t pid = 0;
        V3 o = v3(0, 0, 0), d = v3(0, 0, 1), T = v3(1, 1, 1);
        float t = 0.0f, pdf_b = 0.0f;
        Surface surf;
        surf.albedo = surf.emissive = v3(0, 0, 0);
        surf.normal = v3(0, 0, 1);
        surf.roughness = 1.0f;
        surf.metalness = 0.0f;
        uint32_t px = 0, py = 0, sample_in_batch = 0, bn = 0;
        HitRecord hrecord;
        hrecord.rec = make_uint4(0u, 0u, 0u, 0u);
        hrecord.prim = 0u;
        float hbu = 0.0f, hbv = 0.0f;
        uint32_t htan = 0u;
        float4 ro = make_float4(0.0f, 0.0f, 0.0f, 0.0f), rd = make_float4(0.0f, 0.0f, 1.0f, 0.0f);
        if (!FIRST && active) {
            ro = reinterpret_cast<const float4*>(a.in_rays)[i];
            rd = reinterpret_cast<const float4*>(a.in_rays)[S + i];
        }
        if (active) {
            pid = FIRST ? i : __float_as_uint(rd.w);
            sample_in_batch = fast_div(a.npix_div, pid);
            const uint2 pb = a.pixbn[pid - sample_in_batch * a.npix];
            px = pb.x & 0xFFFFu;
            py = pb.x >> 16;
            bn = pb.y;
        }
        if (FIRST) {
            if (active) {
                size_t pi = (size_t)py * a.width + px;
                float d0 = a.depth[pi];
                if (!LIGHT && d0 == kBackgroundDepth) {
                    reinterpret_cast<float4*>(a.lacc)[pid] = make_float4(0.0f, 0.0f, 0.0f, 0.0f);
                    active = false;
                } else {
                    surf = gbuffer_unpack(a.gbuffer[pi]);
                    primary_ray(g, px, py, o, d);
                    t = d0;
                }
            }
        } else if (active) {
            o = v3(ro.x, ro.y, ro.z);
            d = v3(rd.x, rd.y, rd.z);
            T = v3(a.in_T[i], a.in_T[S + i], a.in_T[2 * S + i]);
            pdf_b = ro.w;
            const float4 hrec = reinterpret_cast<const float4*>(a.in_hits)[i];
            uint32_t prim = __float_as_uint(hrec.w);
            if (!LIGHT && prim == kMiss) {
                if (nee && pdf_b > 0.0f) {
                    float su, sv;
                    direction_to_equirect_uv(d, su, sv);
                    float pl;
                    V3 rad = sky_eval_and_pdf(a.sc, su, sv, pl);
                    float w = pdf_b / (pdf_b + pl);
                    float4* Lp = reinterpret_cast<float4*>(a.lacc) + pid;
                    float4 lv = *Lp;
                    *Lp = make_float4(lv.x + T.x * (rad.x * w), lv.y + T.y * (rad.y * w), lv.z + T.z * (rad.z * w), 0.0f);
                }
                if constexpr (GLASS) {
                    if (!nee && b != 0u && pdf_b == kFloatMax && a.sc.sky != nullptr) {
                        float su, sv;
                        direction_to_equirect_uv(d, su, sv);
                        const V3 rad = sky_eval(a.sc, su, sv);
                        float4* Lp = reinterpret_cast<float4*>(a.lacc) + pid;
                        float4 lv = *Lp;
                        *Lp = make_float4(lv.x + T.x * rad.x, lv.y + T.y * rad.y, lv.z + T.z * rad.z, 0.0f);
                    }
                }
                active = false;
            } else {
                t = hrec.x;
                hbu = hrec.y;
                hbv = hrec.z;
                hrecord = hit_fetch(a.sc, prim);
                if constexpr (MAT) htan = tan_fetch(a.sc, prim);
            }
        }
        bool emit_shadow = false, emit_ext = false;
        V3 wl = v3(0, 1, 0), contrib = v3(0, 0, 0), nd = v3(0, 0, 1), Tn = T;
        float pdf_n = 0.0f;
        float dist_n = 0.0f;
        bool emit_shadow_e = false;
        V3 wle = v3(0, 1, 0), contrib_e = v3(0, 0, 0);
        float tmax_e = 0.0f;
        if (active) {
            uint32_t seed = rng_seed(px, py, g.frame);
            uint32_t sm = a.s0 + sample_in_batch;
            uint32_t base = (sm * B + b) * dims;
            float u0 = uniform_float(seed, base), u1 = uniform_float(seed, base + 1);
            if (bnz) {
                u0 = bluenoise_shift(u0, bn & 0xFFu);
                u1 = bluenoise_shift(u1, (bn >> 8) & 0xFFu);
            }
            V3 rad = v3(0.0f, 0.0f, 0.0f);
            float pl = 0.0f, cosl = 0.0f;
            SkyPick pick;
            pick.u = pick.v = pick.sin_theta = 0.0f;
            pick.x = pick.y = 0;
            if (nee) {
                float ul0 = uniform_float(seed, base + 3), ul1 = uniform_float(seed, base + 4);
                if (bnz) {
                    ul0 = bluenoise_shift(ul0, (bn >> 16) & 0xFFu);
                    ul1 = bluenoise_shift(ul1, (bn >> 24) & 0xFFu);
                }
                pick = sky_sample_direction(a.sc, cdf_marg, guide_marg, ul0, ul1, wl);
            }
            const bool nee_e = !LIGHT && EMIT && b + 1u < B;
            float4 er0 = make_float4(0.0f, 0.0f, 0.0f, 0.0f), er1 = er0, er2 = er0, er3 = er0;
            float eu6 = 0.0f, eu7 = 0.0f;
            if (nee_e) {
                const uint32_t ke = (uint32_t)(uniform_float(seed, base + 5) * 8388608.0f);
                eu6 = uniform_float(seed, base + 6);
                eu7 = uniform_float(seed, base + 7);
                const float4* R = a.lights.rec + 4 * (size_t)light_find(a.lights, ke);
                er0 = R[0];
                er1 = R[1];
                er2 = R[2];
                er3 = R[3];
            }
            if (!FIRST) {
                if constexpr (MAT) {
                    if (GLDS) surf = hit_finish<true>(a.sc, s_geoms, hrecord, hbu, hbv, s_mats, htan);
                    else surf = hit_finish<true>(a.sc, a.sc.shade_geoms, hrecord, hbu, hbv, a.sc.mat_tex, htan);
                } else if (GLDS) surf = hit_finish(a.sc, s_geoms, hrecord, hbu, hbv);
                else surf = hit_finish(a.sc, a.sc.shade_geoms, hrecord, hbu, hbv);
            }
            bool glass_v = false;
            GlassDev gl = {0.0f, 1.0f, 0u, 0u};
            if constexpr (GLASS) {
                if (GLDS) gl = s_glass[hrecord.rec.w];
                else gl = a.glass[hrecord.rec.w];
                if (gl.transmission > 0.0f) glass_v = gl.transmission >= 1.0f || uniform_float(seed, kGlassRngBase + 2u * (sm * B + b)) < gl.transmission;
            }
            V3 N = surf.normal;
            if ((flags & RT3_FLAG_FACEFORWARD) && dot(N, d) > 0.0f) N = neg(N);
            if (!(GLASS && glass_v) && nee) {
                cosl = dot(N, wl);
                if (!DEFER && cosl > 0.0f) sky_sample_radiance(a.sc, pick, rad, pl);
            }
            V3 b1, b2;
            build_orthonormal_basis(N, b1, b2);
            V3 wi = v3(0.0f, 0.0f, 1.0f), vop = surf.albedo, wo = v3(0.0f, 0.0f, 1.0f);
            float pdf_s = 0.0f;
            bool valid = true;
            Bsdf bs;
            const bool last = LIGHT || b == B - 1;
            if (GLASS && glass_v) {
            } else if (spec) {
                bs = bsdf_setup(surf.albedo, surf.roughness, surf.metalness);
                wo = v3(-(d.x * b1.x + d.y * b1.y + d.z * b1.z), -(d.x * b2.x + d.y * b2.y + d.z * b2.z), -(d.x * N.x + d.y * N.y + d.z * N.z));
                if (!last) {
                    float u2 = uniform_float(seed, base + 2);
                    valid = bsdf_sample(bs, wo, u0, u1, u2, wi, vop, pdf_s);
                }
            } else if (!last) {
                wi = diffuse_sample(u0, u1);
                pdf_s = wi.z * kInvPi;
            }
            o = v3(o.x + t * d.x, o.y + t * d.y, o.z + t * d.z);
            if (LIGHT) {
            } else if (FIRST) {
                reinterpret_cast<float4*>(a.lacc)[pid] = make_float4(T.x * surf.emissive.x, T.y * surf.emissive.y, T.z * surf.emissive.z, 0.0f);
            } else if (surf.emissive.x != 0.0f || surf.emissive.y != 0.0f || surf.emissive.z != 0.0f) {
                V3 le = surf.emissive;
                if (EMIT) {
                    const uint32_t eb = a.lights.geom_base[hrecord.rec.w];
                    if (eb != kMiss) {
                        const float4* R = a.lights.rec + 4 * (size_t)(eb + (hrecord.prim - a.sc.first_prim[hrecord.rec.w]));
                        const float pa = R[0].w;
                        const float4 rn = R[3];
                        const float dl = sqrtf(dot(d, d)), cle = fabsf(rn.x * d.x + rn.y * d.y + rn.z * d.z) / dl;
                        float dist = t * dl;
                        if (PANE) dist = pane_dist[pid] + dist;
                        if (pa > 0.0f && cle > 0.0f) {
                            const float ps = pa * (dist * dist) / cle;
                            le = le * (pdf_b / (pdf_b + ps));
                        }
                    }
                }
                float4* Lp = reinterpret_cast<float4*>(a.lacc) + pid;
                float4 lv = *Lp;
                *Lp = make_float4(lv.x + T.x * le.x, lv.y + T.y * le.y, lv.z + T.z * le.z, 0.0f);
            }
            if constexpr (PUNCT) {
                if (!(GLASS && glass_v) && nee_e && er0.w > 0.0f && is_punctual_record(er3)) {
                    const PunctualSample ls = punctual_sample(er0, er1, er2, er3, o, N, kEmitShadowEnd);
                    if (ls.cs > 0.0f && ls.geo > 0.0f) {
                        V3 fv;
                        float scale = (ls.cs * ls.geo) / er0.w;
                        if (spec) {
                            float pproj;
                            bsdf_eval(bs, wo, v3(dot(ls.wl, b1), dot(ls.wl, b2), ls.cs), fv, pproj);
                        } else {
                            fv = surf.albedo;
                            scale = scale * kInvPi;
                        }
                        wle = ls.wl;
                        contrib_e = v3((T.x * fv.x) * (ls.Ic.x * scale), (T.y * fv.y) * (ls.Ic.y * scale), (T.z * fv.z) * (ls.Ic.z * scale));
                        tmax_e = ls.tmax;
                        emit_shadow_e = contrib_e.x > 0.0f || contrib_e.y > 0.0f || contrib_e.z > 0.0f;
                    }
                    er0.w = 0.0f;
                }
            }
            if (!(GLASS && glass_v) && nee_e && er0.w > 0.0f) {
                const float su = sqrtf(eu6), lb1 = eu7 * su, lb2 = su - lb1;
                const V3 pe = v3(er0.x + er1.x * lb1 + er2.x * lb2, er0.y + er1.y * lb1 + er2.y * lb2, er0.z + er1.z * lb1 + er2.z * lb2);
                const V3 wv = pe - o;
                const float dist2 = dot(wv, wv), dist = sqrtf(dist2);
                if (dist2 > 0.0f) {
                    wle = wv * (1.0f / dist);
                    const float cs = dot(N, wle), cle = fabsf(er3.x * wle.x + er3.y * wle.y + er3.z * wle.z);
                    if (cs > 0.0f && cle > 0.0f) {
                        const float ps = er0.w * dist2 / cle;
                        V3 fv;
                        float scale;
                        if (spec) {
                            float pproj;
                            bsdf_eval(bs, wo, v3(dot(wle, b1), dot(wle, b2), cs), fv, pproj);
                            scale = cs / (ps + pproj * cs);
                        } else {
                            fv = surf.albedo;
                            scale = (cs * kInvPi) / (ps + cs * kInvPi);
                        }
                        contrib_e = v3((T.x * fv.x) * (er1.w * scale), (T.y * fv.y) * (er2.w * scale), (T.z * fv.z) * (er3.w * scale));
                        tmax_e = dist * kEmitShadowEnd;
                        emit_shadow_e = contrib_e.x > 0.0f || contrib_e.y > 0.0f || contrib_e.z > 0.0f;
                    }
                }
            }
            if (nee) {
                if (DEFER) emit_shadow = cosl > 0.0f && pick.sin_theta > 0.0f;
                else if (cosl > 0.0f && pl > 0.0f) {
                    V3 fv;
                    float scale;
                    if (spec) {
                        float pproj;
                        bsdf_eval(bs, wo, v3(dot(wl, b1), dot(wl, b2), cosl), fv, pproj);
                        float pb = pproj * cosl;
                        scale = (b == B - 1) ? cosl / pl : cosl / (pl + pb);
                    } else {
                        float pb = cosl * kInvPi;
                        fv = surf.albedo;
                        scale = (b == B - 1) ? (cosl * kInvPi) / pl : (cosl * kInvPi) / (pl + pb);
                    }
                    contrib = v3((T.x * fv.x) * (rad.x * scale), (T.y * fv.y) * (rad.y * scale), (T.z * fv.z) * (rad.z * scale));
                    emit_shadow = true;
                }
            }
            if (GLASS && glass_v) {
                if constexpr (GLASS) {
                    const GlassEvent ev = glass_sample(gl.ior, gl.thin_walled != 0u, d, surf.normal, uniform_float(seed, kGlassRngBase + 2u * (sm * B + b) + 1u));
                    nd = ev.dir;
                    if (ev.transmit) Tn = T * surf.albedo;
                    const bool pane_on = PANE && (gl.pad & kGlassPaneBit) != 0u && ev.transmit != 0u;
                    if (PANE && pane_on && !last) {
                        pdf_n = pdf_b;
                        dist_n = pane_dist[pid] + t * sqrtf(dot(d, d));
                        emit_ext = true;
                    } else if (PANE && pane_on && nee) {
                        float su, sv, pl_s;
                        direction_to_equirect_uv(nd, su, sv);
                        const V3 srad = sky_eval_and_pdf(a.sc, su, sv, pl_s);
                        const float w = pdf_b > 0.0f ? pdf_b / (pdf_b + pl_s) : 0.0f;
                        wl = nd;
                        contrib = v3(Tn.x * (srad.x * w), Tn.y * (srad.y * w), Tn.z * (srad.z * w));
                        emit_shadow = contrib.x > 0.0f || contrib.y > 0.0f || contrib.z > 0.0f;
                    } else if (!last) {
                        pdf_n = pdf_b == kFloatMax ? kFloatMax : kGlassDeltaPdf;
                        emit_ext = true;
                    } else if (nee) {
                        float su, sv;
                        direction_to_equirect_uv(nd, su, sv);
                        const V3 srad = sky_eval(a.sc, su, sv);
                        wl = nd;
                        contrib = v3(Tn.x * srad.x, Tn.y * srad.y, Tn.z * srad.z);
                        emit_shadow = contrib.x > 0.0f || contrib.y > 0.0f || contrib.z > 0.0f;
                    }
                }
            } else if (valid && !last) {
                nd = basis_apply(b1, b2, N, wi);
                pdf_n = pdf_s;
                Tn = T * vop;
                emit_ext = true;
            }
        }
        if constexpr (LIGHT) {
            if (emit_shadow) {
                float4* Lp = reinterpret_cast<float4*>(a.lacc) + pid;
                float4 v = *Lp;
                *Lp = make_float4(v.x + contrib.x, v.y + contrib.y, v.z + contrib.z, 0.0f);
            }
            continue;
        }
        BlockAppend slot;
        uint32_t slot_e = 0;
        if (EMIT) {
            const BlockAppend3 s3 = block_append3(emit_ext, emit_shadow, emit_shadow_e, reinterpret_cast<unsigned long long*>(a.out_count), a.sh2_count, append_lds[parity]);
            slot.ext = s3.ext;
            slot.sh = s3.sh;
            slot_e = s3.sh2;
        } else {
            slot = block_append2(emit_ext, emit_shadow, reinterpret_cast<unsigned long long*>(a.out_count), append_lds[parity]);
        }
        parity ^= 1u;
        if (EMIT && emit_shadow_e) {
            reinterpret_cast<float4*>(a.sh2_rays)[slot_e] = make_float4(o.x, o.y, o.z, contrib_e.x);
            reinterpret_cast<float4*>(a.sh2_rays)[S + slot_e] = make_float4(wle.x, wle.y, wle.z, contrib_e.y);
            reinterpret_cast<float2*>(a.sh2_contrib)[slot_e] = make_float2(contrib_e.z, __uint_as_float(pid));
            a.sh2_tmax[slot_e] = tmax_e;
        }
        if (DEFER && emit_shadow) {
            const uint32_t j = slot.sh;
            reinterpret_cast<float4*>(a.sh_rays)[j] = make_float4(o.x, o.y, o.z, kRayTMin);
            reinterpret_cast<float4*>(a.sh_rays)[S + j] = make_float4(wl.x, wl.y, wl.z, kBackgroundDepth);
            reinterpret_cast<uint32_t*>(a.sh_contrib)[j] = i;
        } else if (emit_shadow) {
            const uint32_t j = slot.sh;
            reinterpret_cast<float4*>(a.sh_rays)[j] = make_float4(o.x, o.y, o.z, contrib.x);
            reinterpret_cast<float4*>(a.sh_rays)[S + j] = make_float4(wl.x, wl.y, wl.z, contrib.y);
            reinterpret_cast<float2*>(a.sh_contrib)[j] = make_float2(contrib.z, __uint_as_float(pid));
        }
        if (emit_ext) {
            const uint32_t j = slot.ext;
            reinterpret_cast<float4*>(a.out_rays)[j] = make_float4(o.x, o.y, o.z, pdf_n);
            reinterpret_cast<float4*>(a.out_rays)[S + j] = make_float4(nd.x, nd.y, nd.z, __uint_as_float(pid));
            a.out_T[j] = Tn.x;
            a.out_T[S + j] = Tn.y;
            a.out_T[2 * S + j] = Tn.z;
            if (PANE) pane_dist[pid] = dist_n;
        }
    }
```

raytracer3_amd/csrc/rt3_trace.hip:

```cpp
#include <hip/hip_fp16.h>
#include <hip/hip_runtime.h>

#include <type_traits>

#include "rt3_hit.hpp"
#include "rt3_internal.hpp"
#include "rt3_math.hpp"
#include "rt3_surface.hpp"

namespace rt3 {

constexpr int kLdsStack = 12;
constexpr uint32_t kTopFlag = 0x40000000u;
constexpr int kSpill = 64 - kLdsStack;
constexpr uint32_t kMaxSteps = 1u << 20;

constexpr uint32_t kEmptySlot = 0xFFFFFFFFu;
constexpr float kTopPadRel = 2.44140625e-4f;

struct Cand {
    float tn;
    uint32_t ref;
};
__device__ __forceinline__ void cswap(Cand& a, Cand& b) {
    bool sw = b.tn < a.tn;
    float ta = a.tn;
    uint32_t ra = a.ref;
    a.tn = sw ? b.tn : a.tn;
    a.ref = sw ? b.ref : a.ref;
    b.tn = sw ? ta : b.tn;
    b.ref = sw ? ra : b.ref;
}
__device__ __forceinline__ void pin(float4& q) { asm volatile("" : "+v"(q.x), "+v"(q.y), "+v"(q.z), "+v"(q.w)); }
__device__ __forceinline__ V3 cross_exact(V3 a, V3 b) { return V3{(a.y * b.z) - (a.z * b.y), (a.z * b.x) - (a.x * b.z), (a.x * b.y) - (a.y * b.x)}; }
__device__ __forceinline__ bool pane_record(float cutoff, uint32_t slot, uint32_t first_slot) { return cutoff != 0.0f ? slot >= first_slot : slot != 0u; }
__device__ __forceinline__ V3 pane_attenuation(const PaneDev& p, uint32_t prim, float u, float v, V3 d) {
    const HitRecord h = hit_fetch(p.sc, prim);
    const Surface s = hit_finish(p.sc, p.sc.shade_geoms, h, u, v);
    const GlassDev gl = p.glass[h.rec.w];
    const float cos_i = fabsf(dot(s.normal, d)) / sqrtf(dot(d, d));
    return s.albedo * (gl.transmission * pane_pass_fraction(gl.ior, cos_i));
}
template <bool MASK = false, bool PANE = false>
__device__ __forceinline__ void tri_test_nb(float4 q0, float4 q1, float4 q2, V3 o, V3 d, float inv_dd, float tmin, Hit& best, const AlphaDev& alpha = AlphaDev{},
                                            const PaneDev* pane = nullptr, float* pay0 = nullptr, float* pay1 = nullptr, float* pay2 = nullptr) {
    const V3 A = v3(q0.x, q0.y, q0.z) - o, B = v3(q0.w, q1.x, q1.y) - o, C = v3(q1.z, q1.w, q2.x) - o;
    const float U = dot_fma(d, cross_exact(B, C)), V = dot_fma(d, cross_exact(C, A)), W = dot_fma(d, cross_exact(A, B));
    const float det = U + (V + W);
    const float inv = 1.0f / det;
    const float w = U * inv, u = V * inv, v = W * inv;
    const float T = __builtin_fmaf(U, dot_fma(A, d), __builtin_fmaf(V, dot_fma(B, d), W * dot_fma(C, d)));
    const float t = (T * inv) * inv_dd;
    const uint32_t prim = __float_as_uint(q2.y);
    constexpr float kEdgeEps = 9.5367431640625e-07f;
    const bool inside = (w >= -kEdgeEps) & (u >= -kEdgeEps) & (v >= -kEdgeEps);
    bool ok = (det != 0.0f) & inside & (t > tmin) & ((t < best.t) | ((t == best.t) & (prim < best.prim)));
    if (MASK && ok && q2.z != 0.0f) ok = alpha_counts(alpha, __float_as_uint(q2.w), q2.z, prim, u, v);
    if constexpr (PANE) {
        if (ok && pane_record(q2.z, __float_as_uint(q2.w), pane->first_slot)) {
            const V3 att = pane_attenuation(*pane, prim, u, v, d);
            *pay0 *= att.x;
            *pay1 *= att.y;
            *pay2 *= att.z;
            ok = *pay0 == 0.0f && *pay1 == 0.0f && *pay2 == 0.0f;
        }
    }
    best.t = ok ? t : best.t;
    best.u = ok ? u : best.u;
    best.v = ok ? v : best.v;
    best.prim = ok ? prim : best.prim;
}

__constant__ uint32_t g_pool_chunk = 256;
__constant__ uint32_t g_refill_lanes = 12;
__device__ __forceinline__ uint32_t pool_chunk_for(uint32_t n, uint32_t n_waves) {
    return (n < 2u * n_waves * g_pool_chunk && g_pool_chunk >= 128u) ? ((g_pool_chunk >> 1) & ~63u) : g_pool_chunk;
}
void set_refill_lanes(uint32_t v) { (void)hipMemcpyToSymbol(HIP_SYMBOL(g_refill_lanes), &v, 4); }
void set_pool_chunk(uint32_t v) { (void)hipMemcpyToSymbol(HIP_SYMBOL(g_pool_chunk), &v, 4); }
static unsigned g_trace_max_blocks = kExtendMaxBlocks;
void set_trace_blocks(uint32_t v) { g_trace_max_blocks = v; }

constexpr uint32_t kTopNodes = kTopCacheNodes;
__device__ __forceinline__ bool load_top(float4* s_top, const float4* __restrict__ top, uint32_t n_top) {
    if (top == nullptr || n_top == 0u) return false;
    n_top = n_top < kTopNodes ? n_top : kTopNodes;
    for (uint32_t i = threadIdx.x; i < 4u * n_top; i += kExtendBlock) s_top[i] = top[i];
    __syncthreads();
    return true;
}

__device__ __forceinline__ bool slab_test_sorted(uint32_t p, uint32_t q, V3 A, V3 B, float tmin, float tbest, float& tn_out) {
    const float nx = __builtin_fmaf((float)(p & 0xFFu), A.x, B.x), ny = __builtin_fmaf((float)((p >> 8) & 0xFFu), A.y, B.y),
                nz = __builtin_fmaf((float)((p >> 16) & 0xFFu), A.z, B.z), fx = __builtin_fmaf((float)(p >> 24), A.x, B.x),
                fy = __builtin_fmaf((float)(q & 0xFFu), A.y, B.y), fz = __builtin_fmaf((float)((q >> 8) & 0xFFu), A.z, B.z);
    const float tn = __builtin_fmaxf(__builtin_fmaxf(nx, ny), __builtin_fmaxf(nz, tmin));
    const float tf = __builtin_fminf(__builtin_fminf(fx, fy), __builtin_fminf(fz, tbest));
    tn_out = tn;
    return tn <= tf;
}

__device__ __forceinline__ bool slab_test_sorted_pad(uint32_t p, uint32_t q, V3 A, V3 B, V3 pad, float tmin, float tbest, float& tn_out) {
    const float nx = __builtin_fmaf((float)(p & 0xFFu), A.x, B.x) - pad.x, ny = __builtin_fmaf((float)((p >> 8) & 0xFFu), A.y, B.y) - pad.y,
                nz = __builtin_fmaf((float)((p >> 16) & 0xFFu), A.z, B.z) - pad.z, fx = __builtin_fmaf((float)(p >> 24), A.x, B.x) + pad.x,
                fy = __builtin_fmaf((float)(q & 0xFFu), A.y, B.y) + pad.y, fz = __builtin_fmaf((float)((q >> 8) & 0xFFu), A.z, B.z) + pad.z;
    const float tn = __builtin_fmaxf(__builtin_fmaxf(nx, ny), __builtin_fmaxf(nz, tmin));
    const float tf = __builtin_fminf(__builtin_fminf(fx, fy), __builtin_fminf(fz, tbest));
    tn_out = tn;
    return tn <= tf;
}

constexpr uint32_t kExitFlag = 0x20000000u;
struct ExitWalk {
    uint32_t off = 0;
    uint32_t mode = 0;
    uint32_t occluded = 0;
};
__device__ __forceinline__ unsigned long long exit_sampled_rays(uint32_t n, uint32_t chunk) {
    if (n == 0u) return 0ull;
    const uint32_t n_chunks = (n - 1u) / chunk + 1u, m = (n_chunks + 31u) / 32u;
    const unsigned long long last_first = 32ull * (m - 1u) * chunk, rest = n - last_first;
    return (unsigned long long)(m - 1u) * chunk + (rest < chunk ? rest : chunk);
}

struct LaneRay {
    V3 o, d, inv;
    float tmin, inv_dd;
    Hit best;
    uint32_t cur, leaf_k, index, steps, cn, ct, cl;
    int sp;
    float pay0, pay1;
    float pay2, pay3;
    uint32_t sel_p0, sel_q0, sel_p1, sel_q1;
};

template <int MODE, bool COUNT, int LAYOUT, bool TWO = false, bool RANGE = false, bool MASK = false, bool EXIT = false, bool PANE = false, typename Finish>
__device__ __forceinline__ void trace_stream(const float4* __restrict__ nodes, uint32_t tri_off,
                                             const float* __restrict__ rays, size_t stride, uint32_t n, uint32_t* __restrict__ work_counter,
                                             uint32_t* __restrict__ lds, Finish finish, bool any_payload = false, bool ext_payload = false, const float4* top_lds = nullptr, bool use_top = false,
                                             const float2* __restrict__ any_contrib = nullptr, const float* __restrict__ any_tmax = nullptr,
                                             const AlphaDev& alpha = AlphaDev{}, ExitWalk* xw = nullptr, const PaneDev* pane = nullptr) {
    static_assert(!PANE || (MODE == 1 && MASK && !EXIT && LAYOUT == kLayoutWide64Q), "panes: the any-hit walk of the default node layout, never from the exit table");
    static_assert(!EXIT || (MODE == 1 && !COUNT && !TWO && !RANGE && LAYOUT == kLayoutWide64Q), "the exit table serves the plain any-hit walk only");
    constexpr bool ANY = MODE == 1;
    constexpr bool WIDE = LAYOUT == kLayoutWide128;
    constexpr bool WIDEQ = LAYOUT == kLayoutWide64Q || LAYOUT == kLayoutWide48Q;
    constexpr bool C48 = LAYOUT == kLayoutWide48Q;
    uint32_t pool_next = 0, pool_end = 0;
    bool queue_empty = false;
    const uint32_t lane = __lane_id();
    const unsigned long long lanes_below = (1ull << lane) - 1ull;
    const uint32_t n_waves = gridDim.x * (blockDim.x >> 6);
    const uint32_t kRefillLanes = g_refill_lanes,
                   kPoolChunk = pool_chunk_for(n, n_waves);
    const uint32_t wave_id = blockIdx.x * (blockDim.x >> 6) + (uint32_t)__builtin_amdgcn_readfirstlane((int)(threadIdx.x >> 6));
    bool first_chunk = true;
    bool chunk_exit = false;
    uint32_t spill[kSpill];
    LaneRay r;
    r.o = r.d = r.inv = v3(0.0f, 0.0f, 0.0f);
    r.tmin = 0.0f;
    r.inv_dd = 1.0f;
    r.best = Hit{0.0f, 0.0f, 0.0f, kMiss};
    r.cur = r.leaf_k = r.index = r.steps = r.cn = r.ct = r.cl = 0u;
    r.sp = 0;
    r.pay0 = r.pay1 = r.pay2 = r.pay3 = 0.0f;
    r.sel_p0 = r.sel_q0 = r.sel_p1 = r.sel_q1 = 0u;
    bool busy = false;
    V3 tl_o = v3(0.0f, 0.0f, 0.0f), tl_pad = v3(0.0f, 0.0f, 0.0f);
    uint32_t tl_mark = 0u, tl_rec = 0u, tl_base = 0u;
    bool tl_bottom = false;
    auto tl_world = [&]() {
        r.inv = v3(guarded_inverse(r.d.x), guarded_inverse(r.d.y), guarded_inverse(r.d.z));
        tl_o = r.o;
        const float pw = kTopPadRel * __builtin_fmaxf(__builtin_fmaxf(fabsf(r.o.x), fabsf(r.o.y)), fabsf(r.o.z));
        tl_pad = v3(pw * fabsf(r.inv.x), pw * fabsf(r.inv.y), pw * fabsf(r.inv.z));
        tl_bottom = false;
    };
    auto tl_sels = [&]() {
        const uint32_t sx = r.inv.x < 0.0f ? 1u : 0u, sy = r.inv.y < 0.0f ? 1u : 0u, sz = r.inv.z < 0.0f ? 1u : 0u;
        const uint32_t nx = 3u * sx, ny = 1u + 3u * sy, nz = 2u + 3u * sz, fx = 3u - 3u * sx, fy = 4u - 3u * sy, fz = 5u - 3u * sz;
        r.sel_p0 = nx | (ny << 8) | (nz << 16) | (fx << 24);
        r.sel_q0 = fy | (fz << 8);
        r.sel_p1 = r.sel_p0 + 0x02020202u;
        r.sel_q1 = r.sel_q0 + 0x00000202u;
    };
    for (;;) {
        const unsigned long long m_idle = __ballot(!busy);
        if (pool_next >= pool_end && !queue_empty && m_idle != 0ull) {
            uint32_t base = 0;
            if (first_chunk) {
                base = wave_id * kPoolChunk;
                first_chunk = false;
            } else {
                if (lane == 0) base = atomicAdd(work_counter, kPoolChunk);
                base = __builtin_amdgcn_readfirstlane(base);
                const unsigned long long b64 = (unsigned long long)n_waves * kPoolChunk + base;
                base = b64 > 0xFFFFFFFFull ? 0xFFFFFFFFu : (uint32_t)b64;
            }
            queue_empty = base >= n;
            pool_next = base < n ? base : n;
            pool_end = (n - pool_next) > kPoolChunk ? pool_next + kPoolChunk : n;
            if constexpr (EXIT) chunk_exit = xw->mode == 2u || (xw->mode == 1u && ((base / kPoolChunk) & 31u) == 0u);
        }
        if (m_idle != 0ull && pool_next < pool_end && ((uint32_t)__popcll(m_idle) >= kRefillLanes || m_idle == ~0ull)) {
            const uint32_t idx = pool_next + (uint32_t)__popcll(m_idle & lanes_below);
            if (!busy && idx < pool_end) {
                const float4 ro = reinterpret_cast<const float4*>(rays)[idx], rd = reinterpret_cast<const float4*>(rays)[stride + idx];
                r.o = v3(ro.x, ro.y, ro.z);
                r.d = v3(rd.x, rd.y, rd.z);
                const bool payload = ANY ? any_payload : ext_payload;
                r.tmin = payload ? kRayTMin : ro.w;
                r.best = Hit{payload ? kBackgroundDepth : rd.w, 0.0f, 0.0f, kMiss};
                if (RANGE) r.best.t = any_tmax[idx];
                r.pay0 = ro.w;
                r.pay1 = rd.w;
                if (ANY && any_contrib != nullptr) {
                    const float2 c2 = any_contrib[idx];
                    r.pay2 = c2.x;
                    r.pay3 = c2.y;
                }
                r.inv = v3(guarded_inverse(r.d.x), guarded_inverse(r.d.y), guarded_inverse(r.d.z));
                r.inv_dd = 1.0f / dot_fma(r.d, r.d);
                if (LAYOUT == kLayoutWide64Q) {
                    const uint32_t sx = r.inv.x < 0.0f ? 1u : 0u, sy = r.inv.y < 0.0f ? 1u : 0u, sz = r.inv.z < 0.0f ? 1u : 0u;
                    const uint32_t nx = 3u * sx, ny = 1u + 3u * sy, nz = 2u + 3u * sz, fx = 3u - 3u * sx, fy = 4u - 3u * sy, fz = 5u - 3u * sz;
                    r.sel_p0 = nx | (ny << 8) | (nz << 16) | (fx << 24);
                    r.sel_q0 = fy | (fz << 8);
                    r.sel_p1 = r.sel_p0 + 0x02020202u;
                    r.sel_q1 = r.sel_q0 + 0x00000202u;
                }
                r.cur = (LAYOUT == kLayoutWide64Q && use_top) ? kTopFlag : 0u;
                if constexpr (EXIT) {
                    if (chunk_exit) {
                        uint32_t hoff = xw->off;
                        asm volatile("" : "+s"(hoff));
                        const ExitHeader e = *reinterpret_cast<const ExitHeader*>(reinterpret_cast<const char*>(nodes) + hoff);
                        const float tx = ((r.inv.x < 0.0f ? e.lo[0] : e.hi[0]) - r.o.x) * r.inv.x, ty = ((r.inv.y < 0.0f ? e.lo[1] : e.hi[1]) - r.o.y) * r.inv.y,
                                    tz = ((r.inv.z < 0.0f ? e.lo[2] : e.hi[2]) - r.o.z) * r.inv.z;
                        const bool ax0 = (tx <= ty) & (tx <= tz), ax1 = !ax0 & (ty <= tz);
                        const float te = ax0 ? tx : (ax1 ? ty : tz);
                        const float cx = (__builtin_fmaf(te, r.d.x, r.o.x) - e.lo[0]) * e.scale[0], cy = (__builtin_fmaf(te, r.d.y, r.o.y) - e.lo[1]) * e.scale[1],
                                    cz = (__builtin_fmaf(te, r.d.z, r.o.z) - e.lo[2]) * e.scale[2];
                        const float cu = ax0 ? cy : (ax1 ? cz : cx), cv = ax0 ? cz : (ax1 ? cx : cy);
                        const float ia = ax0 ? r.inv.x : (ax1 ? r.inv.y : r.inv.z);
                        const uint32_t face = (ax0 ? 0u : (ax1 ? 2u : 4u)) + (ia < 0.0f ? 0u : 1u);
                        const float top = (float)(e.R - 1u);
                        const uint32_t iu = (uint32_t)__builtin_fminf(__builtin_fmaxf(cu, 0.0f), top), iv = (uint32_t)__builtin_fminf(__builtin_fmaxf(cv, 0.0f), top);
                        uint32_t cell = (face * e.R + iv) * e.R + iu;
                        cell = cell < e.last ? cell : e.last;
                        r.cur = kExitFlag | cell;
                    }
                }
                if (TWO) tl_world();
                r.leaf_k = 0u;
                r.sp = 0;
                r.index = idx;
                r.steps = 0u;
                r.cn = r.ct = r.cl = 0u;
                busy = true;
                const bool finite_ray = fabsf(r.o.x) <= kFloatMax && fabsf(r.o.y) <= kFloatMax && fabsf(r.o.z) <= kFloatMax && fabsf(r.d.x) <= kFloatMax &&
                                        fabsf(r.d.y) <= kFloatMax && fabsf(r.d.z) <= kFloatMax;
                if (nodes == nullptr || !finite_ray) {
                    finish(r.index, r.best, 0u, 0u, 0u, r.pay0, r.pay1, r.pay2, r.pay3);
                    busy = false;
                }
            }
            const uint32_t taken = (uint32_t)__popcll(m_idle);
            pool_next = pool_next + taken < pool_end ? pool_next + taken : pool_end;
        }
        if (__ballot(busy) == 0ull && pool_next >= pool_end && queue_empty) break;
        bool by_entry = false;
        if (busy) {
        const bool is_leaf = (r.cur & 0x80000000u) != 0u;
        const uint32_t first = r.cur & 0x0FFFFFFFu, cnt = ((r.cur >> 28) & 7u) + 1u;
        const bool cached = LAYOUT == kLayoutWide64Q && !is_leaf && (r.cur & kTopFlag) != 0u;
        const bool is_inst = TWO && is_leaf && !tl_bottom;
        const bool is_tri = is_leaf && !is_inst;
        constexpr uint32_t kNodeBytes = 16u * (WIDE ? 8 : (C48 ? kC48Stride : 4));
        uint32_t off_tri = tri_off + 48u * (first + r.leaf_k), off_node = kNodeBytes * (cached ? 0u : (is_inst ? first : r.cur));
        asm volatile("" : "+v"(off_tri), "+v"(off_node));
        uint32_t off = is_tri ? off_tri : off_node;
        bool is_exit = false;
        if constexpr (EXIT) {
            is_exit = !is_leaf && (r.cur & kExitFlag) != 0u;
            uint32_t off_exit = xw->off + (uint32_t)sizeof(ExitHeader) + ((r.cur & 0x00FFFFFCu) << 2);
            asm volatile("" : "+v"(off_exit));
            off = is_exit ? off_exit : off;
        }
        const float4* p = reinterpret_cast<const float4*>(reinterpret_cast<const char*>(nodes) + off);
        float4 q0, q1, q2, q3, q4, q5, q6, q7;
        if (TWO && is_tri) {
            const float4* pm = reinterpret_cast<const float4*>(reinterpret_cast<const char*>(nodes) + 64u * (tl_rec + 1u));
            q4 = pm[0];
            q5 = pm[1];
            q6 = pm[2];
        }
        if (LAYOUT == kLayoutWide64Q && cached) {
            const float4* t = top_lds + 4 * (r.cur & 0xFFFFu);
            q0 = t[0];
            q1 = t[1];
            q2 = t[2];
            q3 = t[3];
        } else {
            q0 = p[0];
            q1 = p[1];
            q2 = p[2];
            q3 = C48 ? make_float4(0.0f, 0.0f, 0.0f, 0.0f) : p[3];
        }
        if (WIDE) {
            q4 = p[4];
            q5 = p[5];
            q6 = p[6];
            q7 = p[7];
        }
        if (TWO && is_tri) { pin(q4); pin(q5); pin(q6); }
        pin(q0); pin(q1); pin(q2);
        if (!C48) pin(q3);
        if (WIDE) { pin(q4); pin(q5); pin(q6); pin(q7); }
        bool pop = false, done = false;
        const V3 o = r.o, d = r.d, inv = r.inv;
        const float tmin = r.tmin;
        if (EXIT && is_exit) {
            const uint32_t k = r.cur & 3u;
            const uint32_t e = __float_as_uint(k == 0u ? q0.x : (k == 1u ? q0.y : (k == 2u ? q0.z : q0.w)));
            const uint32_t root = use_top ? kTopFlag : 0u;
            if (e != kEmptySlot) {
                lds[0] = root;
                r.sp = 1;
            }
            r.cur = e != kEmptySlot ? e : root;
        } else if (TWO && is_inst) {
            if (COUNT) r.cn++;
            const float mi[12] = {q0.x, q0.y, q0.z, q0.w, q1.x, q1.y, q1.z, q1.w, q2.x, q2.y, q2.z, q2.w};
            const V3 oo = transform_point(mi, o), dd = transform_vector(mi, d);
            r.inv = v3(guarded_inverse(dd.x), guarded_inverse(dd.y), guarded_inverse(dd.z));
            tl_sels();
            const float om = __builtin_fmaxf(__builtin_fmaxf(__builtin_fmaxf(fabsf(o.x), fabsf(o.y)), __builtin_fmaxf(fabsf(o.z), fabsf(oo.x))),
                                             __builtin_fmaxf(fabsf(oo.y), fabsf(oo.z)));
            const float pb = __builtin_fmaf(q3.w, om, q3.z);
            tl_pad = v3(pb * fabsf(r.inv.x), pb * fabsf(r.inv.y), pb * fabsf(r.inv.z));
            tl_o = oo;
            tl_mark = (uint32_t)r.sp;
            tl_rec = first;
            tl_base = __float_as_uint(q3.y);
            tl_bottom = true;
            r.cur = __float_as_uint(q3.x);
        } else if (is_leaf) {
            if (COUNT) r.ct++;
            if (TWO) {
                const float fm[12] = {q4.x, q4.y, q4.z, q4.w, q5.x, q5.y, q5.z, q5.w, q6.x, q6.y, q6.z, q6.w};
                V3 a = v3(q0.x, q0.y, q0.z), b = v3(q0.w, q1.x, q1.y), c = v3(q1.z, q1.w, q2.x);
                if ((tl_base >> 31) == 0u) {
                    a = transform_point(fm, a);
                    b = transform_point(fm, b);
                    c = transform_point(fm, c);
                }
                const uint32_t gp = __float_as_uint(q2.y) + (tl_base & 0x7FFFFFFFu);
                tri_test_nb<MASK, PANE>(make_float4(a.x, a.y, a.z, b.x), make_float4(b.y, b.z, c.x, c.y),
                                        make_float4(c.z, __uint_as_float(gp), MASK ? q2.z : 0.0f, MASK ? q2.w : 0.0f), o, d, r.inv_dd, tmin, r.best, alpha, pane,
                                        &r.pay0, &r.pay1, &r.pay2);
            } else {
                tri_test_nb<MASK, PANE>(q0, q1, q2, o, d, r.inv_dd, tmin, r.best, alpha, pane, &r.pay0, &r.pay1, &r.pay2);
            }
            r.leaf_k++;
            if (WIDE) {
                if (r.leaf_k < cnt && !(ANY && r.best.prim != kMiss)) {
                    if (COUNT) r.ct++;
                    tri_test_nb(q3, q4, q5, o, d, r.inv_dd, tmin, r.best);
                    r.leaf_k++;
                }
            }
            if (ANY && r.best.prim != kMiss) done = true;
            if (r.leaf_k >= cnt) {
                r.leaf_k = 0;
                pop = true;
            }
        } else {
            if (COUNT) {
                r.cn++;
                r.cl += cached ? 1u : 0u;
            }
            if (WIDE || WIDEQ) {
                const float kInf = __builtin_huge_valf();
                float t0, t1, t2, t3;
                uint32_t r0, r1, r2, r3;
                bool h0, h1, h2, h3;
                if (WIDEQ) {
                    const uint32_t ex = __float_as_uint(q0.w);
                    const V3 A = C48 ? v3(__uint_as_float((ex & 0xFFu) << 23) * inv.x, __uint_as_float(((ex >> 8) & 0xFFu) << 23) * inv.y,
                                          __uint_as_float(((ex >> 16) & 0xFFu) << 23) * inv.z)
                                     : v3(q0.w * inv.x, q3.z * inv.y, q3.w * inv.z);
                    const V3 ob = TWO ? tl_o : o;
                    const V3 B = v3((q0.x - ob.x) * inv.x, (q0.y - ob.y) * inv.y, (q0.z - ob.z) * inv.z);
                    const uint32_t w0 = __float_as_uint(q1.x), w1 = __float_as_uint(q1.y), w2 = __float_as_uint(q1.z), w3 = __float_as_uint(q1.w),
                                   w4 = __float_as_uint(q2.x), w5 = __float_as_uint(q2.y);
                    if (C48) {
                        const uint32_t wa = __float_as_uint(q2.z), wb = __float_as_uint(q2.w);
                        const uint32_t m0 = (ex >> 24) & 15u, m1 = ex >> 28, m2 = wa >> 28, m3 = wb >> 28;
                        uint32_t nb = wa & 0x0FFFFFFFu, tb = wb & 0x0FFFFFFFu;
#define RT3_REF48(m, out)                                                         \
    {                                                                             \
        const bool in_ = (m) == 0u, lf_ = ((m)&8u) != 0u;                         \
        out = in_ ? nb : (lf_ ? (0x80000000u | (((m)&7u) << 28) | tb) : kEmptySlot); \
// ... 171 lines not shown
                                                         const uint32_t* __restrict__ count_ptr, uint32_t count_imm, AlphaArg<MASK> alpha,
                                                         const float* __restrict__ contrib, float* __restrict__ lacc,
                                                         uint32_t* __restrict__ occluded_out, uint32_t* __restrict__ cnt_nodes,
                                                         uint32_t* __restrict__ cnt_tris, unsigned long long* __restrict__ totals,
                                                         uint32_t* __restrict__ work_counter, unsigned long long* __restrict__ lds_total,
                                                         const float* __restrict__ tmax) {
    __shared__ uint32_t stack[kLdsStack * kExtendBlock];
    __shared__ float4 s_top[4 * kTopNodes];
    const bool use_top = load_top(s_top, top, n_top);
    const uint32_t n = count_ptr ? *count_ptr : count_imm;
    TraceCounts<COUNT> counts{cnt_nodes, cnt_tris};
    trace_stream<1, COUNT, LAYOUT == kLayoutTwoLevel ? kLayoutWide64Q : LAYOUT, LAYOUT == kLayoutTwoLevel, RANGE, MASK>(
        nodes, tri_off, rays, stride, n, work_counter, stack + threadIdx.x,
        [&](uint32_t i, const Hit& h, uint32_t cn, uint32_t ct, uint32_t cl, float c_r, float c_g, float c_b, float c_pid) {
            if (occluded_out) {
                occluded_out[i] = h.prim != kMiss ? 1u : 0u;
            } else if (h.prim == kMiss) {
                float4* L = reinterpret_cast<float4*>(lacc) + __float_as_uint(c_pid);
                float4 v = *L;
                *L = make_float4(v.x + c_r, v.y + c_g, v.z + c_b, 0.0f);
            }
            counts.ray(i, cn, ct, cl);
        },
        occluded_out == nullptr, false, s_top, use_top, occluded_out == nullptr ? reinterpret_cast<const float2*>(contrib) : nullptr, tmax,
        alpha.get());
    counts.add_totals(totals, lds_total);
}

template <bool COUNT, int LAYOUT, bool RANGE>
__global__ __launch_bounds__(kExtendBlock) void k_shadow_pane(const float4* __restrict__ nodes, uint32_t tri_off, const float4* __restrict__ top, uint32_t n_top,
                                                              const float* __restrict__ rays, size_t stride,
                                                              const uint32_t* __restrict__ count_ptr, uint32_t count_imm, AlphaDev alpha, PaneDev pane,
                                                              const float* __restrict__ contrib, float* __restrict__ lacc,
                                                              uint32_t* __restrict__ cnt_nodes, uint32_t* __restrict__ cnt_tris,
                                                              unsigned long long* __restrict__ totals, uint32_t* __restrict__ work_counter,
                                                              unsigned long long* __restrict__ lds_total, const float* __restrict__ tmax) {
    __shared__ uint32_t stack[kLdsStack * kExtendBlock];
    __shared__ float4 s_top[4 * kTopNodes];
    const bool use_top = load_top(s_top, top, n_top);
    const uint32_t n = count_ptr ? *count_ptr : count_imm;
    TraceCounts<COUNT> counts{cnt_nodes, cnt_tris};
    trace_stream<1, COUNT, LAYOUT == kLayoutTwoLevel ? kLayoutWide64Q : LAYOUT, LAYOUT == kLayoutTwoLevel, RANGE, true, false, true>(
        nodes, tri_off, rays, stride, n, work_counter, stack + threadIdx.x,
        [&](uint32_t i, const Hit& h, uint32_t cn, uint32_t ct, uint32_t cl, float c_r, float c_g, float c_b, float c_pid) {
            if (h.prim == kMiss) {
                float4* L = reinterpret_cast<float4*>(lacc) + __float_as_uint(c_pid);
                float4 v = *L;
                *L = make_float4(v.x + c_r, v.y + c_g, v.z + c_b, 0.0f);
            }
            counts.ray(i, cn, ct, cl);
        },
        true, false, s_top, use_top, reinterpret_cast<const float2*>(contrib), tmax, alpha, nullptr, &pane);
    counts.add_totals(totals, lds_total);
}

template <bool MASK>
__global__ __launch_bounds__(kExtendBlock) __attribute__((amdgpu_waves_per_eu(8, 8))) void k_shadow_exit(const float4* __restrict__ nodes, uint32_t tri_off, const float4* __restrict__ top, uint32_t n_top,
                                                              const float* __restrict__ rays, size_t stride,
                                                              const uint32_t* __restrict__ count_ptr, uint32_t count_imm, AlphaArg<MASK> alpha,
                                                              const float* __restrict__ contrib, float* __restrict__ lacc,
                                                              uint32_t* __restrict__ occluded_out, uint32_t* __restrict__ work_counter, uint32_t exit_off,
                                                              unsigned long long* __restrict__ counters) {
    __shared__ uint32_t stack[kLdsStack * kExtendBlock];
    __shared__ float4 s_top[4 * kTopNodes];
    const bool use_top = load_top(s_top, top, n_top);
    const uint32_t n = count_ptr ? *count_ptr : count_imm;
    ExitWalk xw;
    xw.off = exit_off;
    {
        const unsigned long long tried = counters[0], occluded = counters[1];
        xw.mode = (tried < kExitWarmupTries || 4ull * occluded >= tried) ? 2u : 1u;
    }
    trace_stream<1, false, kLayoutWide64Q, false, false, MASK, true>(
        nodes, tri_off, rays, stride, n, work_counter, stack + threadIdx.x,
        [&](uint32_t i, const Hit& h, uint32_t, uint32_t, uint32_t, float c_r, float c_g, float c_b, float c_pid) {
            if (occluded_out) {
                occluded_out[i] = h.prim != kMiss ? 1u : 0u;
            } else if (h.prim == kMiss) {
                float4* L = reinterpret_cast<float4*>(lacc) + __float_as_uint(c_pid);
                float4 v = *L;
                *L = make_float4(v.x + c_r, v.y + c_g, v.z + c_b, 0.0f);
            }
        },
        occluded_out == nullptr, false, s_top, use_top, occluded_out == nullptr ? reinterpret_cast<const float2*>(contrib) : nullptr, nullptr, alpha.get(), &xw);
    {
        __syncthreads();
        if ((threadIdx.x & 63u) == 0u) stack[threadIdx.x >> 6] = xw.occluded;
        __syncthreads();
        if (threadIdx.x == 0u) {
            unsigned long long o = 0;
            for (uint32_t w = 0; w < kExtendBlock / 64u; w++) o += stack[w];
            if (o) atomicAdd(&counters[1], o);
            if (blockIdx.x == 0u) {
                const unsigned long long t = xw.mode == 2u ? n : exit_sampled_rays(n, pool_chunk_for(n, gridDim.x * (kExtendBlock / 64u)));
                if (t) atomicAdd(&counters[0], t);
            }
        }
    }
}

template <typename Launch>
static void dispatch_traversal(bool count, int layout, bool masked, Launch launch) {
    auto by_mask = [&](auto c, auto l) {
        if (masked) launch(c, l, std::true_type{});
        else launch(c, l, std::false_type{});
    };
    auto by_layout = [&](auto c) {
        if (layout == kLayoutTwoLevel) by_mask(c, std::integral_constant<int, kLayoutTwoLevel>{});
        else if (layout == kLayoutWide48Q) launch(c, std::integral_constant<int, kLayoutWide48Q>{}, std::false_type{});
        else if (layout == kLayoutWide64Q) by_mask(c, std::integral_constant<int, kLayoutWide64Q>{});
        else if (layout == kLayoutWide128) launch(c, std::integral_constant<int, kLayoutWide128>{}, std::false_type{});
        else launch(c, std::integral_constant<int, kLayoutBinary64>{}, std::false_type{});
    };
    if (count) by_layout(std::true_type{});
    else by_layout(std::false_type{});
}
template <bool MASK>
static AlphaArg<MASK> alpha_arg(const TraceLaunch& L) {
    if constexpr (MASK) return AlphaArg<true>{L.alpha};
    else return AlphaArg<false>{};
}
void launch_extend(hipStream_t st, const LbvhResult& bvh, const TraceLaunch& L) {
    const unsigned grid = grid_for(L.n, kExtendBlock, g_trace_max_blocks);
    unsigned long long* const tot = L.totals ? L.totals + kTotExtendNodes : nullptr;
    unsigned long long* const lds_tot = L.totals ? L.totals + kTotExtendLds : nullptr;
    dispatch_traversal(L.count, bvh.layout, L.alpha.table != nullptr, [&](auto c, auto l, auto m) {
        hipLaunchKernelGGL((k_extend<decltype(c)::value, decltype(l)::value, decltype(m)::value>), dim3(grid), dim3(kExtendBlock), 0, st, bvh.nodes.get(),
                           bvh.tri_off, bvh.top.get(), bvh.n_top, L.rays, L.stride, L.count_ptr, L.n, L.hits, L.cnt_nodes, L.cnt_tris, tot, L.work_counter,
                           L.payload ? 1 : 0, alpha_arg<decltype(m)::value>(L), lds_tot);
    });
}
static void launch_shadow_pane(hipStream_t st, const LbvhResult& bvh, const TraceLaunch& L, unsigned grid) {
    unsigned long long* const tot = L.totals ? L.totals + kTotShadowNodes : nullptr;
    unsigned long long* const lds_tot = L.totals ? L.totals + kTotShadowLds : nullptr;
    auto launch = [&](auto c, auto l, auto range) {
        hipLaunchKernelGGL((k_shadow_pane<decltype(c)::value, decltype(l)::value, decltype(range)::value>), dim3(grid), dim3(kExtendBlock), 0, st, bvh.nodes.get(),
                           bvh.tri_off, bvh.top.get(), bvh.n_top, L.rays, L.stride, L.count_ptr, L.n, L.alpha, *L.pane, L.contrib, L.lacc, L.cnt_nodes, L.cnt_tris, tot,
                           L.work_counter, lds_tot, L.tmax);
    };
    auto by_range = [&](auto c, auto l) {
        if (L.tmax) launch(c, l, std::true_type{});
        else launch(c, l, std::false_type{});
    };
    auto by_layout = [&](auto c) {
        if (bvh.layout == kLayoutTwoLevel) by_range(c, std::integral_constant<int, kLayoutTwoLevel>{});
        else by_range(c, std::integral_constant<int, kLayoutWide64Q>{});
    };
    if (L.count) by_layout(std::true_type{});
    else by_layout(std::false_type{});
}
void launch_shadow(hipStream_t st, const LbvhResult& bvh, const TraceLaunch& L) {
    const unsigned grid = grid_for(L.n, kExtendBlock, g_trace_max_blocks);
    if (L.pane != nullptr && L.occluded == nullptr && (bvh.layout == kLayoutWide64Q || bvh.layout == kLayoutTwoLevel)) return launch_shadow_pane(st, bvh, L, grid);
    if (bvh.exit.on && bvh.exit.off && bvh.exit.counters && bvh.layout == kLayoutWide64Q && bvh.nodes && !L.count && !L.tmax) {
        auto launch = [&](auto m) {
            hipLaunchKernelGGL((k_shadow_exit<decltype(m)::value>), dim3(grid), dim3(kExtendBlock), 0, st, bvh.nodes.get(), bvh.tri_off, bvh.top.get(), bvh.n_top, L.rays,
                               L.stride, L.count_ptr, L.n, alpha_arg<decltype(m)::value>(L), L.contrib, L.lacc, L.occluded, L.work_counter, bvh.exit.off, bvh.exit.counters);
        };
        if (L.alpha.table != nullptr) launch(std::true_type{});
        else launch(std::false_type{});
        return;
    }
    unsigned long long* const tot = L.totals ? L.totals + kTotShadowNodes : nullptr;
    unsigned long long* const lds_tot = L.totals ? L.totals + kTotShadowLds : nullptr;
    dispatch_traversal(L.count, bvh.layout, L.alpha.table != nullptr, [&](auto c, auto l, auto m) {
        auto launch = [&](auto range) {
            hipLaunchKernelGGL((k_shadow<decltype(c)::value, decltype(l)::value, decltype(range)::value, decltype(m)::value>), dim3(grid), dim3(kExtendBlock), 0,
                               st, bvh.nodes.get(), bvh.tri_off, bvh.top.get(), bvh.n_top, L.rays, L.stride, L.count_ptr, L.n,
                               alpha_arg<decltype(m)::value>(L), L.contrib, L.lacc, L.occluded, L.cnt_nodes, L.cnt_tris, tot, L.work_counter, lds_tot, L.tmax);
        };
        if (L.tmax) launch(std::true_type{});
        else launch(std::false_type{});
    });
}

}
```

Measured before the change: 8153.

## Decide deferred sky shadow rays in shade via exit-table triangle test

Moves the exit-table occlusion shortcut for deferred sky shadow rays into the shade kernel. Each shadow ray is tested against the cached exit-cell triangles there, and rays already found occluded are never emitted. The remaining shadow rays are traced from the root by the plain shadow kernel instead of the exit-table kernel. This cuts the number of emitted and traced shadow rays, at the cost of extra work and register pressure in shade and of losing the exit shortcut for the undecided rays.

```diff
diff --git a/include/rt3.h b/include/rt3.h
--- a/include/rt3.h
+++ b/include/rt3.h
@@ -116,6 +116,7 @@
 #define RT3_OPT_INSTANCE_MODE 14
 #define RT3_OPT_SHADOW_EXIT_TABLE 15
 #define RT3_OPT_DEFER_SKY_LIGHT 16
+#define RT3_OPT_SHADE_EXIT_TEST 17
 int rt3_set_option(rt3_ctx *ctx, int option, int64_t value);
 
 int rt3_scene_set_vertices(rt3_ctx *ctx, const float *interleaved_p_n_t, uint32_t n_vertices);
diff --git a/raytracer3_amd/_lib.py b/raytracer3_amd/_lib.py
--- a/raytracer3_amd/_lib.py
+++ b/raytracer3_amd/_lib.py
@@ -25,6 +25,7 @@
 OPT_INSTANCE_MODE = 14
 OPT_SHADOW_EXIT_TABLE = 15
 OPT_DEFER_SKY_LIGHT = 16
+OPT_SHADE_EXIT_TEST = 17
 DENOISE_NO_DEMODULATION = 1
 TEMPORAL_NO_DEMODULATION = 1
 SELFTEST_EXPN = 28
diff --git a/raytracer3_amd/csrc/rt3_api.hip b/raytracer3_amd/csrc/rt3_api.hip
--- a/raytracer3_amd/csrc/rt3_api.hip
+++ b/raytracer3_amd/csrc/rt3_api.hip
@@ -60,6 +60,7 @@
                 }
                 c->prof.stats.extension_rays += traced;
                 c->prof.stats.shadow_rays += h[b.first + 2 * k + 1];
+                if (b.dec_first) c->prof.stats.shadow_rays += h[b.dec_first + k];
             }
             for (uint32_t k = 0; k < b.n_emit; k++) c->prof.stats.shadow_rays += h[b.emit_first + k];
         }
@@ -199,6 +200,10 @@
         case RT3_OPT_DEFER_SKY_LIGHT:
             if (value != 0 && value != 1) return fail(c, RT3_E_INVALID, "defer sky light must be 0 (off) or 1 (on)");
             c->opt.defer_sky_light = value != 0;
+            return RT3_OK;
+        case RT3_OPT_SHADE_EXIT_TEST:
+            if (value != 0 && value != 1) return fail(c, RT3_E_INVALID, "shade exit test must be 0 (off) or 1 (on)");
+            c->opt.shade_exit_test = value != 0;
             return RT3_OK;
         default: return fail(c, RT3_E_INVALID, "unknown option");
     }
diff --git a/raytracer3_amd/csrc/rt3_ctx.hpp b/raytracer3_amd/csrc/rt3_ctx.hpp
--- a/raytracer3_amd/csrc/rt3_ctx.hpp
+++ b/raytracer3_amd/csrc/rt3_ctx.hpp
@@ -50,6 +50,7 @@
     uint32_t emit_first = 0, n_emit = 0;
     uint32_t rr_first = 0, rr_lo = 0;
     uint64_t launch = 0;
+    uint32_t dec_first = 0;
 };
 
 struct TlMesh {
@@ -245,6 +246,7 @@
         int instance_mode = 0;
         int exit_table = 1;
         bool defer_sky_light = true;
+        bool shade_exit_test = true;
     } opt;
     struct Prof {
         rt3_stats stats;
diff --git a/raytracer3_amd/csrc/rt3_internal.hpp b/raytracer3_amd/csrc/rt3_internal.hpp
--- a/raytracer3_amd/csrc/rt3_internal.hpp
+++ b/raytracer3_amd/csrc/rt3_internal.hpp
@@ -90,7 +90,14 @@
 void launch_raygen(hipStream_t st, const GConstDev& g, const uint32_t* pixels, uint32_t npix, float* rays, size_t stride);
 void launch_gbuffer(hipStream_t st, const SceneDev& sc, const uint32_t* pixels, uint32_t npix, uint32_t width, const float* hits,
                     size_t stride, void* gbuffer, float* depth);
-void launch_shade(hipStream_t st, bool first, ShadeLaunch L, bool punct = false, const GlassDev* glass = nullptr, bool defer = false, float* pane_dist = nullptr);
+struct ShadeExit {
+    const float4* arena = nullptr;
+    uint32_t tri_off = 0, exit_off = 0;
+    unsigned long long* counters = nullptr;
+    uint32_t* decided = nullptr;
+};
+void launch_shade(hipStream_t st, bool first, ShadeLaunch L, bool punct = false, const GlassDev* glass = nullptr, bool defer = false, float* pane_dist = nullptr,
+                  const ShadeExit* exit = nullptr);
 void launch_light(hipStream_t st, bool first, ShadeLaunch L);
 void launch_pixbn(hipStream_t st, const uint32_t* pixels, uint32_t npix, const uint8_t* bluenoise, uint32_t bn_w, uint32_t bn_h, uint2* out);
 void launch_accumulate(hipStream_t st, const GConstDev& g, const uint32_t* pixels, uint32_t npix, uint32_t width, const float* depth,
@@ -320,6 +327,7 @@
     unsigned long long* totals = nullptr;
     AlphaDev alpha = {};
     const PaneDev* pane = nullptr;
+    bool from_root = false;
 };
 void launch_extend(hipStream_t st, const LbvhResult& bvh, const TraceLaunch& L);
 void launch_shadow(hipStream_t st, const LbvhResult& bvh, const TraceLaunch& L);
diff --git a/raytracer3_amd/csrc/rt3_passes.hip b/raytracer3_amd/csrc/rt3_passes.hip
--- a/raytracer3_amd/csrc/rt3_passes.hip
+++ b/raytracer3_amd/csrc/rt3_passes.hip
@@ -210,6 +210,8 @@
     LightsDev lights{};
     bool nee = false, nee_e = false, punct = false;
     bool defer = false;
+    bool shade_exit = false;
+    ShadeExit exit{};
     bool lens_on = false;
     LensDev lens{};
     bool rr = false;
@@ -235,6 +237,17 @@
     ps->nee_e = ps->lights.n != 0u;
     ps->sc = scene_dev(c);
     ps->defer = c->opt.defer_sky_light && ps->nee && !c->accel.has_glass && !ps->punct && ps->sc.mat_tex == nullptr && c->scene.sky_min_pdf >= kSkyDeferMinPdf;
+    {
+        const LbvhResult& bvh = c->accel.bvh;
+        ps->shade_exit = c->opt.shade_exit_test && ps->defer && !ps->nee_e && !c->opt.count && alpha_dev(c).table == nullptr && c->accel.n_panes == 0u &&
+                         bvh.exit.on && bvh.exit.off && bvh.exit.counters && bvh.layout == kLayoutWide64Q && bvh.nodes;
+        if (ps->shade_exit) {
+            ps->exit.arena = bvh.nodes.get();
+            ps->exit.tri_off = bvh.tri_off;
+            ps->exit.exit_off = bvh.exit.off;
+            ps->exit.counters = bvh.exit.counters;
+        }
+    }
     ps->panes = c->accel.n_panes != 0u && c->accel.has_glass;
     if (ps->panes) {
         if (int r = ensure_pane_dist(c)) return r;
@@ -266,15 +279,17 @@
     const uint32_t n_words = (nee_e ? 6 : 4) * B;
     uint32_t first;
     const bool rr = ps.rr;
-    if (int r = reserve_counters(c, n_words + 1 + (lens ? 2 : 0) + (rr ? B : 0), &first)) return r;
+    const bool shade_exit = ps.shade_exit;
+    if (int r = reserve_counters(c, n_words + 1 + (lens ? 2 : 0) + (rr ? B : 0) + (shade_exit ? B : 0), &first)) return r;
     first += first & 1u;
     uint32_t* pairs = c->work.d_counters.get() + first;
     uint32_t* pool_cur = c->work.d_counters.get() + first + 2 * B;
     uint32_t* emit_cnt = c->work.d_counters.get() + first + 4 * B;
     uint32_t* lens_cnt = c->work.d_counters.get() + first + n_words;
     uint32_t* rr_cnt = lens_cnt + (lens ? 2 : 0);
-    c->work.pending_counters.push_back(
-        CounterBlock{first, B, first + 4 * B, nee_e ? B : 0u, rr ? first + n_words + (lens ? 2u : 0u) : 0u, ps.rr_start, c->work.launch_serial});
+    uint32_t* dec_cnt = rr_cnt + (rr ? B : 0);
+    c->work.pending_counters.push_back(CounterBlock{first, B, first + 4 * B, nee_e ? B : 0u, rr ? first + n_words + (lens ? 2u : 0u) : 0u, ps.rr_start,
+                                                    c->work.launch_serial, shade_exit ? (uint32_t)(dec_cnt - c->work.d_counters.get()) : 0u});
     auto ext_cnt_at = [pairs](uint32_t b) { return pairs + 2 * b; };
     auto sh_cnt_at = [pairs](uint32_t b) { return pairs + 2 * b + 1; };
     int cur = 0;
@@ -311,8 +326,10 @@
         L.sh2_rays = c->work.sh2_rays.get(); L.sh2_contrib = c->work.sh2_contrib.get(); L.sh2_tmax = c->work.sh2_tmax.get(); L.sh2_count = emit_cnt + bn;
         {
             ScopedTimer t(c, CAT_SHADE);
+            ShadeExit sx = ps.exit;
+            sx.decided = dec_cnt + bn;
             launch_shade(c->stream, bn == 0 && !lens, L, ps.punct, c->accel.has_glass ? c->accel.d_glass.get() : nullptr, ps.defer,
-                         ps.panes ? c->work.pane_dist.get() : nullptr);
+                         ps.panes ? c->work.pane_dist.get() : nullptr, shade_exit ? &sx : nullptr);
         }
         cur ^= 1;
         if (nee) {
@@ -320,6 +337,7 @@
             tr.rays = c->work.sh_rays.get(); tr.count_ptr = sh_cnt_at(bn); tr.n = n_first; tr.work_counter = pool_cur + B + bn;
             if (ps.defer) {
                 tr.occluded = reinterpret_cast<uint32_t*>(c->work.sh_contrib.get()) + S;
+                tr.from_root = shade_exit;
             } else {
                 tr.contrib = c->work.sh_contrib.get(); tr.lacc = c->work.lacc.get();
                 if (ps.panes) tr.pane = &ps.pane;
diff --git a/raytracer3_amd/csrc/rt3_shade.hip b/raytracer3_amd/csrc/rt3_shade.hip
--- a/raytracer3_amd/csrc/rt3_shade.hip
+++ b/raytracer3_amd/csrc/rt3_shade.hip
@@ -7,6 +7,7 @@
 #include "rt3_camera.hpp"
 #include "rt3_glass.hpp"
 #include "rt3_internal.hpp"
+#include "rt3_leaf_test.hpp"
 #include "rt3_math.hpp"
 #include "rt3_punctual.hpp"
 #include "rt3_rng.hpp"
@@ -131,41 +132,54 @@
 template <bool FIRST, bool GLDS, bool EMIT = false, bool MAT = false>
 __global__ __launch_bounds__(kShadeBlock) __attribute__((amdgpu_waves_per_eu(shade_waves(MAT), shade_waves(MAT)))) void k_shade(ShadeLaunch a) {
     constexpr bool PUNCT = false, GLASS = false, DEFER = false, LIGHT = false;
-    constexpr bool PANE = false;
-    float* const pane_dist = nullptr;
+    constexpr bool PANE = false, EXIT = false;
+    float* const pane_dist = nullptr;
+    const ShadeExit x = {};
 #include "rt3_shade_body.inc"
 }
 template <bool FIRST, bool GLDS, bool MAT>
 __global__ __launch_bounds__(kShadeBlock) __attribute__((amdgpu_waves_per_eu(shade_waves(true), shade_waves(true)))) void k_shade_punct(ShadeLaunch a) {
     constexpr bool EMIT = true, PUNCT = true, GLASS = false, DEFER = false, LIGHT = false;
-    constexpr bool PANE = false;
-    float* const pane_dist = nullptr;
+    constexpr bool PANE = false, EXIT = false;
+    float* const pane_dist = nullptr;
+    const ShadeExit x = {};
 #include "rt3_shade_body.inc"
 }
 template <bool GLDS, bool EMIT, bool MAT, bool PUNCT>
 __global__ __launch_bounds__(kShadeBlock) __attribute__((amdgpu_waves_per_eu(shade_waves(true), shade_waves(true)))) void k_shade_glass(ShadeLaunch a) {
     constexpr bool FIRST = false, GLASS = true, DEFER = false, LIGHT = false;
-    constexpr bool PANE = false;
-    float* const pane_dist = nullptr;
+    constexpr bool PANE = false, EXIT = false;
+    float* const pane_dist = nullptr;
+    const ShadeExit x = {};
 #include "rt3_shade_body.inc"
 }
 template <bool GLDS, bool EMIT, bool MAT, bool PUNCT>
 __global__ __launch_bounds__(kShadeBlock) __attribute__((amdgpu_waves_per_eu(shade_waves(true), shade_waves(true)))) void k_shade_pane(ShadeLaunch a, float* pane_dist) {
-    constexpr bool FIRST = false, GLASS = true, DEFER = false, LIGHT = false, PANE = true;
+    constexpr bool FIRST = false, GLASS = true, DEFER = false, LIGHT = false, PANE = true, EXIT = false;
+    const ShadeExit x = {};
 #include "rt3_shade_body.inc"
 }
 template <bool FIRST, bool GLDS, bool EMIT>
 __global__ __launch_bounds__(kShadeBlock) __attribute__((amdgpu_waves_per_eu(shade_waves(false), shade_waves(false)))) void k_shade_defer(ShadeLaunch a) {
     constexpr bool MAT = false, PUNCT = false, GLASS = false, DEFER = true, LIGHT = false;
-    constexpr bool PANE = false;
+    constexpr bool PANE = false, EXIT = false;
+    float* const pane_dist = nullptr;
+    const ShadeExit x = {};
+#include "rt3_shade_body.inc"
+}
+template <bool FIRST, bool GLDS>
+__global__ __launch_bounds__(kShadeBlock) __attribute__((amdgpu_waves_per_eu(shade_waves(false), shade_waves(false)))) void k_shade_defer_exit(ShadeLaunch a, ShadeExit x) {
+    constexpr bool EMIT = false, MAT = false, PUNCT = false, GLASS = false, DEFER = true, LIGHT = false;
+    constexpr bool PANE = false, EXIT = true;
     float* const pane_dist = nullptr;
 #include "rt3_shade_body.inc"
 }
 template <bool FIRST, bool GLDS>
 __global__ __launch_bounds__(kShadeBlock) __attribute__((amdgpu_waves_per_eu(shade_waves(false), shade_waves(false)))) void k_light(ShadeLaunch a) {
     constexpr bool EMIT = false, MAT = false, PUNCT = false, GLASS = false, DEFER = false, LIGHT = true;
-    constexpr bool PANE = false;
-    float* const pane_dist = nullptr;
+    constexpr bool PANE = false, EXIT = false;
+    float* const pane_dist = nullptr;
+    const ShadeExit x = {};
 #include "rt3_shade_body.inc"
 }
 __global__ void k_selftest_glass(const uint32_t* __restrict__ in, uint32_t n, uint32_t* __restrict__ out) {
@@ -231,10 +245,16 @@
     else if (glds) by_mat(std::true_type{});
     else by_mat(std::false_type{});
 }
-void launch_shade(hipStream_t st, bool first, ShadeLaunch a, bool punct, const GlassDev* glass, bool defer, float* pane_dist) {
+void launch_shade(hipStream_t st, bool first, ShadeLaunch a, bool punct, const GlassDev* glass, bool defer, float* pane_dist, const ShadeExit* exit) {
     a.npix_div = make_fastdiv(a.npix);
     const unsigned grid = grid_for(a.n_first, kShadeBlock, 8192);
     const bool glds = a.sc.shade_geoms != nullptr && a.sc.n_geoms <= kShadeGeomsLds;
+    if (defer && exit != nullptr && a.lights.n == 0u) {
+        dispatch_shade(first, glds, false, false, false, [&](auto f, auto g, auto, auto, auto) {
+            hipLaunchKernelGGL((k_shade_defer_exit<decltype(f)::value, decltype(g)::value>), dim3(grid), dim3(kShadeBlock), 0, st, a, *exit);
+        });
+        return;
+    }
     if (defer) {
         dispatch_shade(first, glds, a.lights.n != 0u, false, false, [&](auto f, auto g, auto e, auto, auto) {
             hipLaunchKernelGGL((k_shade_defer<decltype(f)::value, decltype(g)::value, decltype(e)::value>), dim3(grid), dim3(kShadeBlock), 0, st, a);
diff --git a/raytracer3_amd/csrc/rt3_shade_body.inc b/raytracer3_amd/csrc/rt3_shade_body.inc
--- a/raytracer3_amd/csrc/rt3_shade_body.inc
+++ b/raytracer3_amd/csrc/rt3_shade_body.inc
@@ -3,6 +3,7 @@
     static_assert(!(FIRST && MAT), "the first vertex is read from the G-buffer");
     static_assert(EMIT || !PUNCT, "punctual lights are records of the emitter table");
     static_assert(!(FIRST && GLASS), "the G-buffer has no room for a material class: glass frames start from camera rays");
+    static_assert(!EXIT || (DEFER && !EMIT), "the exit test decides deferred sky shadow rays, in frames without an emitter queue");
     __shared__ uint32_t append_lds[2][(EMIT ? 3 : 2) * (kShadeBlock / 64 + 1)];
     __shared__ ShadeGeomDev s_geoms[GLDS ? kShadeGeomsLds : 1];
     __shared__ MatTexDev s_mats[GLDS && MAT ? kShadeGeomsLds : 1];
@@ -18,6 +19,14 @@
         __syncthreads();
     }
     uint32_t parity = 0;
+    bool exit_every = false;
+    uint32_t exit_tested = 0u, exit_decided = 0u;
+    ExitHeader xh = {};
+    if constexpr (EXIT) {
+        const unsigned long long tried = x.counters[0], occluded = x.counters[1];
+        exit_every = tried < kExitWarmupTries || 4ull * occluded >= tried;
+        xh = *reinterpret_cast<const ExitHeader*>(reinterpret_cast<const char*>(x.arena) + x.exit_off);
+    }
     constexpr uint32_t kMargRows = 2048;
     __shared__ uint32_t s_guide_marg[kMargRows];
     __shared__ float s_cdf_marg[kMargRows + 4];
@@ -42,6 +51,9 @@
     for (uint32_t it = blockIdx.x * blockDim.x + threadIdx.x; it < n_round + (LIGHT ? gridDim.x * blockDim.x : 0u); it += gridDim.x * blockDim.x) {
         uint32_t i = it;
         bool active = i < n;
+        const bool exit_trip = EXIT && (exit_every || ((it / kShadeBlock) & 31u) == 0u);
+        bool x_tested = false, x_decided = false;
+        uint32_t x_entry = kEmptySlot;
         if constexpr (LIGHT) {
             if (!light_next(a, it, n, n_round, light_held, i, active)) continue;
         }
@@ -183,6 +195,18 @@
             if (!(GLASS && glass_v) && nee) {
                 cosl = dot(N, wl);
                 if (!DEFER && cosl > 0.0f) sky_sample_radiance(a.sc, pick, rad, pl);
+                if constexpr (EXIT) {
+                    if (exit_trip && cosl > 0.0f && pick.sin_theta > 0.0f) {
+                        x_tested = true;
+                        const V3 xo = v3(o.x + t * d.x, o.y + t * d.y, o.z + t * d.z);
+                        const bool finite_ray = fabsf(xo.x) <= kFloatMax && fabsf(xo.y) <= kFloatMax && fabsf(xo.z) <= kFloatMax && fabsf(wl.x) <= kFloatMax &&
+                                                fabsf(wl.y) <= kFloatMax && fabsf(wl.z) <= kFloatMax;
+                        if (finite_ray) {
+                            const uint32_t cell = exit_cell(xh, xo, wl, v3(guarded_inverse(wl.x), guarded_inverse(wl.y), guarded_inverse(wl.z)));
+                            x_entry = reinterpret_cast<const uint32_t*>(reinterpret_cast<const char*>(x.arena) + x.exit_off + sizeof(ExitHeader))[cell];
+                        }
+                    }
+                }
             }
             V3 b1, b2;
             build_orthonormal_basis(N, b1, b2);
@@ -277,6 +301,17 @@
             }
             if (nee) {
                 if (DEFER) emit_shadow = cosl > 0.0f && pick.sin_theta > 0.0f;
+                if constexpr (EXIT) {
+                    if (emit_shadow && x_entry != kEmptySlot && (x_entry & 0x80000000u) != 0u) {
+                        const uint32_t cnt = ((x_entry >> 28) & 7u) + 1u;
+                        const float4* rec = reinterpret_cast<const float4*>(reinterpret_cast<const char*>(x.arena) + x.tri_off) + 3 * (size_t)(x_entry & 0x0FFFFFFFu);
+                        const float inv_dd = 1.0f / dot_fma(wl, wl);
+                        Hit best = Hit{kBackgroundDepth, 0.0f, 0.0f, kMiss};
+                        for (uint32_t k = 0; k < cnt && best.prim == kMiss; k++) tri_test_nb(rec[3 * k], rec[3 * k + 1], rec[3 * k + 2], o, wl, inv_dd, kRayTMin, best);
+                        x_decided = best.prim != kMiss;
+                        emit_shadow = !x_decided;
+                    }
+                }
                 else if (cosl > 0.0f && pl > 0.0f) {
                     V3 fv;
                     float scale;
@@ -331,6 +366,10 @@
                 emit_ext = true;
             }
         }
+        if constexpr (EXIT) {
+            exit_tested += (uint32_t)__popcll(__ballot(x_tested));
+            exit_decided += (uint32_t)__popcll(__ballot(x_decided));
+        }
         if constexpr (LIGHT) {
             if (emit_shadow) {
                 float4* Lp = reinterpret_cast<float4*>(a.lacc) + pid;
@@ -377,3 +416,23 @@
             if (PANE) pane_dist[pid] = dist_n;
         }
     }
+    if constexpr (EXIT) {
+        __shared__ uint32_t s_exit[2 * (kShadeBlock / 64)];
+        if (__lane_id() == 0u) {
+            s_exit[threadIdx.x >> 6] = exit_tested;
+            s_exit[kShadeBlock / 64 + (threadIdx.x >> 6)] = exit_decided;
+        }
+        __syncthreads();
+        if (threadIdx.x == 0u) {
+            unsigned long long nt = 0ull, nd = 0ull;
+            for (int w = 0; w < kShadeBlock / 64; w++) {
+                nt += s_exit[w];
+                nd += s_exit[kShadeBlock / 64 + w];
+            }
+            if (nt) atomicAdd(&x.counters[0], nt);
+            if (nd) {
+                atomicAdd(&x.counters[1], nd);
+                atomicAdd(x.decided, (uint32_t)nd);
+            }
+        }
+    }
diff --git a/raytracer3_amd/csrc/rt3_trace.hip b/raytracer3_amd/csrc/rt3_trace.hip
--- a/raytracer3_amd/csrc/rt3_trace.hip
+++ b/raytracer3_amd/csrc/rt3_trace.hip
@@ -5,6 +5,7 @@
 
 #include "rt3_hit.hpp"
 #include "rt3_internal.hpp"
+#include "rt3_leaf_test.hpp"
 #include "rt3_math.hpp"
 #include "rt3_surface.hpp"
 
@@ -15,7 +16,6 @@
 constexpr int kSpill = 64 - kLdsStack;
 constexpr uint32_t kMaxSteps = 1u << 20;
 
-constexpr uint32_t kEmptySlot = 0xFFFFFFFFu;
 constexpr float kTopPadRel = 2.44140625e-4f;
 
 struct Cand {
@@ -32,44 +32,6 @@
     b.ref = sw ? ra : b.ref;
 }
 __device__ __forceinline__ void pin(float4& q) { asm volatile("" : "+v"(q.x), "+v"(q.y), "+v"(q.z), "+v"(q.w)); }
-__device__ __forceinline__ V3 cross_exact(V3 a, V3 b) { return V3{(a.y * b.z) - (a.z * b.y), (a.z * b.x) - (a.x * b.z), (a.x * b.y) - (a.y * b.x)}; }
-__device__ __forceinline__ bool pane_record(float cutoff, uint32_t slot, uint32_t first_slot) { return cutoff != 0.0f ? slot >= first_slot : slot != 0u; }
-__device__ __forceinline__ V3 pane_attenuation(const PaneDev& p, uint32_t prim, float u, float v, V3 d) {
-    const HitRecord h = hit_fetch(p.sc, prim);
-    const Surface s = hit_finish(p.sc, p.sc.shade_geoms, h, u, v);
-    const GlassDev gl = p.glass[h.rec.w];
-    const float cos_i = fabsf(dot(s.normal, d)) / sqrtf(dot(d, d));
-    return s.albedo * (gl.transmission * pane_pass_fraction(gl.ior, cos_i));
-}
-template <bool MASK = false, bool PANE = false>
-__device__ __forceinline__ void tri_test_nb(float4 q0, float4 q1, float4 q2, V3 o, V3 d, float inv_dd, float tmin, Hit& best, const AlphaDev& alpha = AlphaDev{},
-                                            const PaneDev* pane = nullptr, float* pay0 = nullptr, float* pay1 = nullptr, float* pay2 = nullptr) {
-    const V3 A = v3(q0.x, q0.y, q0.z) - o, B = v3(q0.w, q1.x, q1.y) - o, C = v3(q1.z, q1.w, q2.x) - o;
-    const float U = dot_fma(d, cross_exact(B, C)), V = dot_fma(d, cross_exact(C, A)), W = dot_fma(d, cross_exact(A, B));
-    const float det = U + (V + W);
-    const float inv = 1.0f / det;
-    const float w = U * inv, u = V * inv, v = W * inv;
-    const float T = __builtin_fmaf(U, dot_fma(A, d), __builtin_fmaf(V, dot_fma(B, d), W * dot_fma(C, d)));
-    const float t = (T * inv) * inv_dd;
-    const uint32_t prim = __float_as_uint(q2.y);
-    constexpr float kEdgeEps = 9.5367431640625e-07f;
-    const bool inside = (w >= -kEdgeEps) & (u >= -kEdgeEps) & (v >= -kEdgeEps);
-    bool ok = (det != 0.0f) & inside & (t > tmin) & ((t < best.t) | ((t == best.t) & (prim < best.prim)));
-    if (MASK && ok && q2.z != 0.0f) ok = alpha_counts(alpha, __float_as_uint(q2.w), q2.z, prim, u, v);
-    if constexpr (PANE) {
-        if (ok && pane_record(q2.z, __float_as_uint(q2.w), pane->first_slot)) {
-            const V3 att = pane_attenuation(*pane, prim, u, v, d);
-            *pay0 *= att.x;
-            *pay1 *= att.y;
-            *pay2 *= att.z;
-            ok = *pay0 == 0.0f && *pay1 == 0.0f && *pay2 == 0.0f;
-        }
-    }
-    best.t = ok ? t : best.t;
-    best.u = ok ? u : best.u;
-    best.v = ok ? v : best.v;
-    best.prim = ok ? prim : best.prim;
-}
 
 __constant__ uint32_t g_pool_chunk = 256;
 __constant__ uint32_t g_refill_lanes = 12;
@@ -236,20 +198,7 @@
                         uint32_t hoff = xw->off;
                         asm volatile("" : "+s"(hoff));
                         const ExitHeader e = *reinterpret_cast<const ExitHeader*>(reinterpret_cast<const char*>(nodes) + hoff);
-                        const float tx = ((r.inv.x < 0.0f ? e.lo[0] : e.hi[0]) - r.o.x) * r.inv.x, ty = ((r.inv.y < 0.0f ? e.lo[1] : e.hi[1]) - r.o.y) * r.inv.y,
-                                    tz = ((r.inv.z < 0.0f ? e.lo[2] : e.hi[2]) - r.o.z) * r.inv.z;
-                        const bool ax0 = (tx <= ty) & (tx <= tz), ax1 = !ax0 & (ty <= tz);
-                        const float te = ax0 ? tx : (ax1 ? ty : tz);
-                        const float cx = (__builtin_fmaf(te, r.d.x, r.o.x) - e.lo[0]) * e.scale[0], cy = (__builtin_fmaf(te, r.d.y, r.o.y) - e.lo[1]) * e.scale[1],
-                                    cz = (__builtin_fmaf(te, r.d.z, r.o.z) - e.lo[2]) * e.scale[2];
-                        const float cu = ax0 ? cy : (ax1 ? cz : cx), cv = ax0 ? cz : (ax1 ? cx : cy);
-                        const float ia = ax0 ? r.inv.x : (ax1 ? r.inv.y : r.inv.z);
-                        const uint32_t face = (ax0 ? 0u : (ax1 ? 2u : 4u)) + (ia < 0.0f ? 0u : 1u);
-                        const float top = (float)(e.R - 1u);
-                        const uint32_t iu = (uint32_t)__builtin_fminf(__builtin_fmaxf(cu, 0.0f), top), iv = (uint32_t)__builtin_fminf(__builtin_fmaxf(cv, 0.0f), top);
-                        uint32_t cell = (face * e.R + iv) * e.R + iu;
-                        cell = cell < e.last ? cell : e.last;
-                        r.cur = kExitFlag | cell;
+                        r.cur = kExitFlag | exit_cell(e, r.o, r.d, r.inv);
                     }
                 }
                 if (TWO) tl_world();
@@ -727,7 +676,7 @@
 void launch_shadow(hipStream_t st, const LbvhResult& bvh, const TraceLaunch& L) {
     const unsigned grid = grid_for(L.n, kExtendBlock, g_trace_max_blocks);
     if (L.pane != nullptr && L.occluded == nullptr && (bvh.layout == kLayoutWide64Q || bvh.layout == kLayoutTwoLevel)) return launch_shadow_pane(st, bvh, L, grid);
-    if (bvh.exit.on && bvh.exit.off && bvh.exit.counters && bvh.layout == kLayoutWide64Q && bvh.nodes && !L.count && !L.tmax) {
+    if (!L.from_root && bvh.exit.on && bvh.exit.off && bvh.exit.counters && bvh.layout == kLayoutWide64Q && bvh.nodes && !L.count && !L.tmax) {
         auto launch = [&](auto m) {
             hipLaunchKernelGGL((k_shadow_exit<decltype(m)::value>), dim3(grid), dim3(kExtendBlock), 0, st, bvh.nodes.get(), bvh.tri_off, bvh.top.get(), bvh.n_top, L.rays,
                                L.stride, L.count_ptr, L.n, alpha_arg<decltype(m)::value>(L), L.contrib, L.lacc, L.occluded, L.work_counter, bvh.exit.off, bvh.exit.counters);
```

After: 8652, median of 6. 1.06x the previous value.
